# abb128/april-asr

Hardware: AMD Instinct MI355X
Metric: audio_seconds_per_second (concurrent 16 kHz sessions x 1/RTF), aprilv0_en-us-sized streaming RNN-T (higher is better)
Workload: dtype f32

## Files before the change

### april_asr_amd/_ffi.py

```python
import ctypes as C
import os

_HERE = os.path.dirname(os.path.abspath(__file__))
LIB_PATH = os.environ.get("APRIL_ASR_LIB") or os.path.join(_HERE, "libaprilasr.so")


class AprilSpeakerID(C.Structure):
    _fields_ = [("data", C.c_uint8 * 16)]


class AprilToken(C.Structure):
    _fields_ = [("token", C.c_char_p), ("logprob", C.c_float), ("flags", C.c_int),
                ("time_ms", C.c_size_t), ("reserved", C.c_void_p)]


HANDLER = C.CFUNCTYPE(None, C.c_void_p, C.c_int, C.c_size_t, C.POINTER(AprilToken))


class AprilConfig(C.Structure):
    _fields_ = [("speaker", AprilSpeakerID), ("handler", HANDLER), ("userdata", C.c_void_p), ("flags", C.c_int)]


class AprilxDims(C.Structure):
    _fields_ = [(n, C.c_int32) for n in ("n_layers", "d_model", "hidden", "ffn", "joiner", "vocab", "mel", "seg",
                                         "seg_step", "context", "fft_size", "frame_shift", "sample_rate", "blank_id",
                                         "n_devices", "precision", "d_model_file")] + [("param_count", C.c_int64)]


class AprilxStats(C.Structure):
    _fields_ = [(n, C.c_uint64) for n in ("ticks", "steps", "chunks", "rounds", "frames", "max_batch_seen")] + \
               [("kernel_ms", C.c_double * 6), ("kernel_launches", C.c_uint64 * 6), ("host_ms", C.c_double * 8),
                ("flights", C.c_uint64), ("replay_mismatch", C.c_uint64), ("kernels_per_step", C.c_uint64),
                ("lm_steps", C.c_uint64), ("lm_chunks", C.c_uint64),
                ("wave_steps", C.c_uint64), ("wave_chunks", C.c_uint64),
                ("gates_clock_ms", C.c_double), ("gates_clock_launches", C.c_uint64), ("gates_clock_rows", C.c_uint64),
                ("gates_clock_ms_by_n", C.c_double * 4), ("gates_clock_launches_by_n", C.c_uint64 * 4),
                ("resample_ms", C.c_double), ("resample_launches", C.c_uint64), ("confidence_records", C.c_uint64)]


class AprilxTokenInfo(C.Structure):
    _fields_ = [("size", C.c_uint32), ("n_alt", C.c_uint32), ("eval_index", C.c_uint64), ("lse", C.c_float),
                ("token_logprob", C.c_float), ("blank_logprob", C.c_float), ("reserved0", C.c_float),
                ("alt_id", C.c_int32 * 8), ("alt_logit", C.c_float * 8)]


class AprilxSearchOptions(C.Structure):
    _fields_ = [("size", C.c_uint32), ("endpoint_silence_ms", C.c_uint32), ("max_utterance_ms", C.c_uint32), ("blank_penalty", C.c_float)]


class AprilxLoadInfo(C.Structure):
    _fields_ = [("broadcast_ms", C.c_double), ("comm_init_ms", C.c_double), ("broadcast_bytes", C.c_uint64),
                ("ranks", C.c_int32), ("used_rccl", C.c_int32)]


class AprilxInputFormat(C.Structure):
    _fields_ = [("size", C.c_uint32), ("encoding", C.c_uint32), ("channels", C.c_uint32), ("channel", C.c_int32)]


EXPORTED_REFERENCE_SYMBOLS = [
    "aam_api_init", "aam_create_model", "aam_get_name", "aam_get_description", "aam_get_language",
    "aam_get_sample_rate", "aam_free", "aas_create_session", "aas_feed_pcm16", "aas_flush",
    "aas_realtime_get_speedup", "aas_free",
]
EXPORTED_ENGINE_SYMBOLS = [
    "aprilx_model_dims", "aprilx_model_token", "aprilx_model_blob_size", "aprilx_model_export_blob",
    "aprilx_model_from_blob", "aprilx_model_save_blob", "aprilx_model_save_blob_f16", "aprilx_model_load_blob",
    "aprilx_broadcast_get_id", "aprilx_model_broadcast", "aprilx_model_load_info", "aprilx_feed_many", "aprilx_flush_many", "aprilx_session_drain", "aprilx_feed_many_pipelined", "aprilx_drain_many",
    "aprilx_run_encoder", "aprilx_run_decoder", "aprilx_run_joiner", "aprilx_run_fbank", "aprilx_run_decide", "aprilx_plan_gemm", "aprilx_stream_form",
    "aprilx_session_trace_logits", "aprilx_session_chunks", "aprilx_session_read_frames", "aprilx_session_context", "aprilx_model_stats", "aprilx_model_profile", "aprilx_model_feed_latency",
    "aprilx_greedy_create", "aprilx_greedy_step", "aprilx_greedy_finish", "aprilx_greedy_free", "aprilx_probe_file", "aprilx_model_load_host", "aprilx_model_fbank_tables", "aprilx_counting_handler",
    "aprilx_session_set_input_rate", "aprilx_session_input_rate", "aprilx_resampler_taps", "aprilx_resample",
    "aprilx_session_set_confidence", "aprilx_session_confidence", "aprilx_run_confidence",
    "aprilx_bias_create", "aprilx_bias_free", "aprilx_bias_info", "aprilx_bias_edges", "aprilx_session_set_bias", "aprilx_session_bias_state",
    "aprilx_run_decide_biased", "aprilx_greedy_set_bias", "aprilx_greedy_bias_state",
    "aprilx_bias_create_ex", "aprilx_bias_flags", "aprilx_run_confidence_biased",
    "aprilx_session_set_search_options", "aprilx_session_search_options", "aprilx_run_decide_opts", "aprilx_greedy_set_search_options",
    "aprilx_ramp_window", "aprilx_model_ramp_stats",
    "aprilx_session_set_input_format", "aprilx_session_input_format", "aprilx_session_feed_bytes", "aprilx_feed_many_bytes",
    "aprilx_decode_host", "aprilx_decode", "aprilx_model_decode_stats",
]

_lib = None
_inited = False


def lib():
    global _lib
    if _lib is not None:
        return _lib
    if not os.path.exists(LIB_PATH):
        raise ImportError("libaprilasr.so is not built: run `python -c 'import __graft_entry__ as g; g.build()'` "
                          "or `make -C april_asr_amd/csrc` (hipcc, gfx950). There is no CPU fallback.")
    L = C.CDLL(LIB_PATH)
    vp, sz = C.c_void_p, C.c_size_t
    L.aam_api_init.argtypes = [C.c_int]; L.aam_api_init.restype = None
    L.aam_create_model.argtypes = [C.c_char_p]; L.aam_create_model.restype = vp
    for f in ("aam_get_name", "aam_get_description", "aam_get_language"):
        getattr(L, f).argtypes = [vp]; getattr(L, f).restype = C.c_char_p
    L.aam_get_sample_rate.argtypes = [vp]; L.aam_get_sample_rate.restype = sz
    L.aam_free.argtypes = [vp]; L.aam_free.restype = None
    L.aas_create_session.argtypes = [vp, AprilConfig]; L.aas_create_session.restype = vp
    L.aas_feed_pcm16.argtypes = [vp, vp, sz]; L.aas_feed_pcm16.restype = None
    L.aas_flush.argtypes = [vp]; L.aas_flush.restype = None
    L.aas_realtime_get_speedup.argtypes = [vp]; L.aas_realtime_get_speedup.restype = C.c_float
    L.aas_free.argtypes = [vp]; L.aas_free.restype = None
    L.aprilx_model_dims.argtypes = [vp, C.POINTER(AprilxDims)]; L.aprilx_model_dims.restype = C.c_int
    L.aprilx_model_token.argtypes = [vp, C.c_int32]; L.aprilx_model_token.restype = C.c_char_p
    L.aprilx_model_blob_size.argtypes = [vp]; L.aprilx_model_blob_size.restype = sz
    L.aprilx_model_export_blob.argtypes = [vp, vp, sz]; L.aprilx_model_export_blob.restype = C.c_int
    L.aprilx_model_from_blob.argtypes = [vp, sz, C.c_int]; L.aprilx_model_from_blob.restype = vp
    L.aprilx_model_save_blob.argtypes = [vp, C.c_char_p]; L.aprilx_model_save_blob.restype = C.c_int
    L.aprilx_model_save_blob_f16.argtypes = [vp, C.c_char_p]; L.aprilx_model_save_blob_f16.restype = C.c_int
    L.aprilx_model_load_blob.argtypes = [C.c_char_p]; L.aprilx_model_load_blob.restype = vp
    L.aprilx_broadcast_get_id.argtypes = [vp, sz]; L.aprilx_broadcast_get_id.restype = C.c_int
    L.aprilx_model_broadcast.argtypes = [vp, C.c_int, C.c_int, vp]; L.aprilx_model_broadcast.restype = vp
    L.aprilx_model_load_info.argtypes = [vp, C.POINTER(AprilxLoadInfo)]; L.aprilx_model_load_info.restype = C.c_int
    L.aprilx_feed_many.argtypes = [sz, C.POINTER(vp), C.POINTER(vp), C.POINTER(sz)]; L.aprilx_feed_many.restype = None
    L.aprilx_flush_many.argtypes = [sz, C.POINTER(vp)]; L.aprilx_flush_many.restype = None
    L.aprilx_session_drain.argtypes = [vp]; L.aprilx_session_drain.restype = None
    L.aprilx_feed_many_pipelined.argtypes = [sz, C.POINTER(vp), C.POINTER(vp), C.POINTER(sz), C.c_int]; L.aprilx_feed_many_pipelined.restype = None
    L.aprilx_drain_many.argtypes = [sz, C.POINTER(vp)]; L.aprilx_drain_many.restype = None
    L.aprilx_run_encoder.argtypes = [vp, C.c_int] + [vp] * 6; L.aprilx_run_encoder.restype = C.c_int
    L.aprilx_run_decoder.argtypes = [vp, C.c_int, vp, vp]; L.aprilx_run_decoder.restype = C.c_int
    L.aprilx_run_joiner.argtypes = [vp, C.c_int, vp, vp, vp]; L.aprilx_run_joiner.restype = C.c_int
    L.aprilx_run_fbank.argtypes = [vp, C.c_int, vp, vp]; L.aprilx_run_fbank.restype = C.c_int
    L.aprilx_plan_gemm.argtypes = [C.c_int] * 6 + [vp]; L.aprilx_plan_gemm.restype = C.c_int
    L.aprilx_ramp_window.argtypes = [C.c_int] * 3 + [vp, C.c_int]; L.aprilx_ramp_window.restype = C.c_int
    L.aprilx_model_ramp_stats.argtypes = [vp, C.c_int, C.POINTER(C.c_uint64), C.POINTER(C.c_uint64)]; L.aprilx_model_ramp_stats.restype = C.c_int
    L.aprilx_stream_form.argtypes = [C.c_int] * 6; L.aprilx_stream_form.restype = C.c_int
    L.aprilx_run_decide.argtypes = [vp, C.c_int, C.c_int, vp, C.c_float, vp, C.c_int, vp, vp]; L.aprilx_run_decide.restype = C.c_int
    L.aprilx_session_trace_logits.argtypes = [vp, vp, sz, C.POINTER(sz)]; L.aprilx_session_trace_logits.restype = None
    L.aprilx_session_chunks.argtypes = [vp]; L.aprilx_session_chunks.restype = C.c_uint64
    L.aprilx_session_read_frames.argtypes = [vp, C.c_uint64, C.c_int, C.c_void_p]; L.aprilx_session_read_frames.restype = C.c_uint64
    L.aprilx_session_context.argtypes = [vp, vp, vp]; L.aprilx_session_context.restype = None
    L.aprilx_model_stats.argtypes = [vp, C.c_int, C.POINTER(AprilxStats)]; L.aprilx_model_stats.restype = None
    L.aprilx_model_feed_latency.argtypes = [vp, C.c_int, vp, C.c_int, C.c_int]; L.aprilx_model_feed_latency.restype = C.c_int
    L.aprilx_model_profile.argtypes = [vp, C.c_int]; L.aprilx_model_profile.restype = None
    L.aprilx_greedy_create.argtypes = [vp, HANDLER, vp]; L.aprilx_greedy_create.restype = vp
    L.aprilx_greedy_step.argtypes = [vp, C.c_int32, C.c_float, C.c_float, C.c_float, sz, C.POINTER(C.c_int32)]
    L.aprilx_greedy_step.restype = C.c_int
    L.aprilx_greedy_finish.argtypes = [vp]; L.aprilx_greedy_finish.restype = None
    L.aprilx_greedy_free.argtypes = [vp]; L.aprilx_greedy_free.restype = None
    L.aprilx_model_load_host.argtypes = [C.c_char_p]; L.aprilx_model_load_host.restype = vp
    L.aprilx_model_fbank_tables.argtypes = [vp, vp, vp]; L.aprilx_model_fbank_tables.restype = C.c_int
    L.aprilx_probe_file.argtypes = [C.c_char_p, C.c_char_p, sz]; L.aprilx_probe_file.restype = C.c_int
    L.aprilx_session_set_input_rate.argtypes = [vp, C.c_uint32]; L.aprilx_session_set_input_rate.restype = C.c_int
    L.aprilx_session_input_rate.argtypes = [vp]; L.aprilx_session_input_rate.restype = C.c_uint32
    L.aprilx_resampler_taps.argtypes = [C.c_uint32, C.c_uint32, vp, vp, sz]; L.aprilx_resampler_taps.restype = C.c_int
    L.aprilx_resample.argtypes = [vp, C.c_uint32, vp, sz, vp, sz]; L.aprilx_resample.restype = C.c_int64
    L.aprilx_session_set_confidence.argtypes = [vp, C.c_int]; L.aprilx_session_set_confidence.restype = C.c_int
    L.aprilx_session_confidence.argtypes = [vp]; L.aprilx_session_confidence.restype = C.c_int
    L.aprilx_run_confidence.argtypes = [vp, C.c_int, vp, C.c_int, vp]; L.aprilx_run_confidence.restype = C.c_int
    L.aprilx_bias_create.argtypes = [vp, sz, C.POINTER(C.c_char_p), C.POINTER(C.c_float), C.c_char_p, sz]; L.aprilx_bias_create.restype = vp
    L.aprilx_bias_create_ex.argtypes = [vp, sz, C.POINTER(C.c_char_p), C.POINTER(C.c_float), C.c_uint32, C.c_char_p, sz]; L.aprilx_bias_create_ex.restype = vp
    L.aprilx_bias_flags.argtypes = [vp]; L.aprilx_bias_flags.restype = C.c_int
    L.aprilx_run_confidence_biased.argtypes = [vp, C.c_int, vp, C.c_int, vp, vp, vp]; L.aprilx_run_confidence_biased.restype = C.c_int
    L.aprilx_bias_free.argtypes = [vp]; L.aprilx_bias_free.restype = None
    L.aprilx_bias_info.argtypes = [vp, C.POINTER(C.c_int32), C.POINTER(C.c_int64)]; L.aprilx_bias_info.restype = C.c_int
    L.aprilx_bias_edges.argtypes = [vp, C.c_int32, vp, vp, vp, sz]; L.aprilx_bias_edges.restype = C.c_int
    L.aprilx_session_set_bias.argtypes = [vp, vp]; L.aprilx_session_set_bias.restype = C.c_int
    L.aprilx_session_bias_state.argtypes = [vp, C.POINTER(C.c_int32), C.POINTER(C.c_int32)]; L.aprilx_session_bias_state.restype = C.c_int
    L.aprilx_run_decide_biased.argtypes = [vp, C.c_int, C.c_int, vp, C.c_float, vp, C.c_int, vp, vp, vp, vp]; L.aprilx_run_decide_biased.restype = C.c_int
    L.aprilx_greedy_set_bias.argtypes = [vp, vp]; L.aprilx_greedy_set_bias.restype = C.c_int
    L.aprilx_greedy_bias_state.argtypes = [vp]; L.aprilx_greedy_bias_state.restype = C.c_int
    L.aprilx_session_set_search_options.argtypes = [vp, C.POINTER(AprilxSearchOptions)]; L.aprilx_session_set_search_options.restype = C.c_int
    L.aprilx_session_search_options.argtypes = [vp, C.POINTER(AprilxSearchOptions)]; L.aprilx_session_search_options.restype = C.c_int
    L.aprilx_run_decide_opts.argtypes = [vp, C.c_int, C.c_int, vp, C.c_float, vp, C.c_int, vp, vp, vp, vp, vp]; L.aprilx_run_decide_opts.restype = C.c_int
    L.aprilx_greedy_set_search_options.argtypes = [vp, C.POINTER(AprilxSearchOptions)]; L.aprilx_greedy_set_search_options.restype = C.c_int
    L.aprilx_session_set_input_format.argtypes = [vp, C.POINTER(AprilxInputFormat)]; L.aprilx_session_set_input_format.restype = C.c_int
    L.aprilx_session_input_format.argtypes = [vp, C.POINTER(AprilxInputFormat)]; L.aprilx_session_input_format.restype = C.c_int
    L.aprilx_session_feed_bytes.argtypes = [vp, vp, sz]; L.aprilx_session_feed_bytes.restype = C.c_int
    L.aprilx_feed_many_bytes.argtypes = [sz, C.POINTER(vp), C.POINTER(vp), C.POINTER(sz), C.c_int]; L.aprilx_feed_many_bytes.restype = C.c_int
    L.aprilx_decode_host.argtypes = [C.POINTER(AprilxInputFormat), vp, sz, vp, sz]; L.aprilx_decode_host.restype = C.c_int64
    L.aprilx_decode.argtypes = [vp, C.POINTER(AprilxInputFormat), vp, sz, vp, sz]; L.aprilx_decode.restype = C.c_int64
    L.aprilx_model_decode_stats.argtypes = [vp, C.c_int, C.POINTER(C.c_uint64), C.POINTER(C.c_uint64), C.POINTER(C.c_double)]; L.aprilx_model_decode_stats.restype = C.c_int
    _lib = L
    return L


def init():
    global _inited
    L = lib()
    if not _inited:
        L.aam_api_init(1)
        _inited = True
    return L
```

### april_asr_amd/csrc/engine.cc

```cpp
#include "engine.h"
#include <array>
#include <algorithm>
#include <cmath>
#include <chrono>
#include <cstdlib>
#include <cstring>
#include "common.h"
#include "env.h"

namespace aprilx {

static size_t align64(size_t x) { return (x + 63) & ~(size_t)63; }

void plan_layout(const NetDims &d, bool has_dec_conv_b, PackedLayout &L)
{
    L.dims = d;
    L.has_dec_conv_b = has_dec_conv_b;
    L.vocab_pad = (d.vocab + 31) & ~31;
    size_t off = 0;
    auto take = [&](size_t n) { size_t o = off; off = align64(off + n); return o; };
    L.k3 = (d.conv_ch[1] * 9 + 63) & ~63;
    L.conv_w[0] = take((size_t)d.conv_ch[0] * 9); L.conv_b[0] = take((size_t)d.conv_ch[0]);
    L.conv_w[1] = take((size_t)d.conv_ch[1] * d.conv_ch[0] * 9); L.conv_b[1] = take((size_t)d.conv_ch[1]);
    L.conv_w[2] = take((size_t)L.k3 * d.conv_ch[2]); L.conv_b[2] = take((size_t)d.conv_ch[2]);
// ... 49 lines not shown
    const NetDims &d = L.dims;
    blob.assign(L.total, 0.0f);
    float *B = blob.data();
    for (int i = 0; i < 3; ++i) {
        if (i < 2) memcpy(B + L.conv_w[i], m.conv_w[i].data(), m.conv_w[i].size() * 4);
        memcpy(B + L.conv_b[i], m.conv_b[i].data(), m.conv_b[i].size() * 4);
    }
    {
        const int kreal = d.conv_ch[1] * 9, c2 = d.conv_ch[2];
        std::vector<float> w3((size_t)L.k3 * c2, 0.0f);
        for (int o = 0; o < c2; ++o) for (int k = 0; k < kreal; ++k) w3[(size_t)k * c2 + o] = m.conv_w[2][(size_t)o * kreal + k];
        pack_mfma(w3.data(), L.k3, c2, c2, nullptr, B + L.conv_w[2]);
    }
    {
        const int c2 = d.conv_ch[2], F = d.f_out;
        std::vector<float> we((size_t)d.embed_in * d.d_model);
        for (int c = 0; c < c2; ++c) for (int f = 0; f < F; ++f)
            memcpy(&we[((size_t)f * c2 + c) * d.d_model], &m.w_embed[((size_t)c * F + f) * d.d_model], (size_t)d.d_model * 4);
        pack_mfma(we.data(), d.embed_in, d.d_model, d.d_model, nullptr, B + L.w_embed);
    }
    memcpy(B + L.b_embed, m.b_embed.data(), (size_t)d.d_model * 4);
    L.embed_eps = m.embed_norm_eps;
    L.norm_eps.resize((size_t)d.n_layers);
    std::vector<int> gmap((size_t)4 * d.hidden);
    for (int u = 0; u < d.hidden; ++u) for (int g = 0; g < 4; ++g) gmap[(size_t)u * 4 + g] = g * d.hidden + u;
    for (int l = 0; l < d.n_layers; ++l) {
        const LayerWeights &lw = m.layers[(size_t)l];
        const PackedLayout::Layer &o = L.layers[(size_t)l];
        pack_mfma(lw.w_gates.data(), 2 * d.d_model, 4 * d.hidden, 4 * d.hidden, &gmap, B + o.wg);
        for (int n = 0; n < 4 * d.hidden; ++n) B[o.bg + n] = lw.b_gates[(size_t)gmap[(size_t)n]];
        pack_mfma(lw.w_hr.data(), d.hidden, d.d_model, d.d_model, nullptr, B + o.whr);
        pack_mfma(lw.w_ff1.data(), d.d_model, d.ffn, d.ffn, nullptr, B + o.wff1);
        memcpy(B + o.bff1, lw.b_ff1.data(), (size_t)d.ffn * 4);
        pack_mfma(lw.w_ff2.data(), d.ffn, d.d_model, d.d_model, nullptr, B + o.wff2);
        memcpy(B + o.bff2, lw.b_ff2.data(), (size_t)d.d_model * 4);
        L.norm_eps[(size_t)l] = lw.norm_eps;
    }
    pack_mfma(m.w_encproj.data(), d.d_model, d.joiner, d.joiner, nullptr, B + L.w_encproj);
    memcpy(B + L.b_encproj, m.b_encproj.data(), (size_t)d.joiner * 4);
    memcpy(B + L.emb, m.emb.data(), m.emb.size() * 4);
    memcpy(B + L.dec_conv, m.dec_conv.data(), m.dec_conv.size() * 4);
    if (!m.dec_conv_b.empty()) memcpy(B + L.dec_conv_b, m.dec_conv_b.data(), m.dec_conv_b.size() * 4);
    pack_mfma(m.w_decproj.data(), d.d_model, d.joiner, d.joiner, nullptr, B + L.w_decproj);
    memcpy(B + L.b_decproj, m.b_decproj.data(), (size_t)d.joiner * 4);
    pack_mfma(m.w_out.data(), d.joiner, d.vocab, L.vocab_pad, nullptr, B + L.w_out);
    memcpy(B + L.b_out, m.b_out.data(), (size_t)d.vocab * 4);
}

template <typename T> static T *dmalloc(size_t n) { HipLegacyLock legacy; T *p = nullptr; HIP_CHECK(hipMalloc((void **)&p, std::max<size_t>(n, 1) * sizeof(T))); return p; }
template <typename T> static T *hmalloc(size_t n) { HipLegacyLock legacy; T *p = nullptr; HIP_CHECK(hipHostMalloc((void **)&p, std::max<size_t>(n, 1) * sizeof(T), hipHostMallocDefault)); return p; }

std::recursive_mutex &hip_legacy_mutex() { static std::recursive_mutex m; return m; }

static int pick_kz(int K, int N, int kblk = 16)
{
    int kz = 256 / std::max(1, N / 16);
    kz = std::max(1, std::min(kz, 8));
    while (kz > 1 && ((K / kblk) / kz < 4 || (K / kblk) % (4 * kz) != 0)) kz >>= 1;
    return kz;
}

Engine::Engine(const EngineConfig &cfg, const PackedLayout &layout, const float *blob_host, const float *blob_device,
               const ModelParams &params, const FbankHostTables &ft, const std::vector<uint8_t> &tok_class)
    : cfg_(cfg), L_(layout), P_(params)
{
    HipLegacyLock legacy;
    HIP_CHECK(hipSetDevice(cfg_.device));
    HIP_CHECK(hipStreamCreateWithFlags(&stream_, hipStreamNonBlocking));
    HIP_CHECK(hipStreamCreateWithFlags(&f_stream_, hipStreamNonBlocking));
    HIP_CHECK(hipStreamCreateWithFlags(&s_stream_, hipStreamNonBlocking));
    search_stream_ = stream_;
    for (int i = 0; i < 32; ++i) { hipEvent_t e; HIP_CHECK(hipEventCreateWithFlags(&e, hipEventDisableTiming)); join_ev_.push_back(e); }
    split_streams_ = std::max(0, std::min(2, env_int("APRIL_SPLIT_STREAMS", 2)));
    const NetDims &d = L_.dims;
    w_ = dmalloc<float>(L_.total);
    if (blob_device) HIP_CHECK(hipMemcpy(w_, blob_device, L_.total * 4, hipMemcpyDeviceToDevice));
    else if (blob_host) HIP_CHECK(hipMemcpy(w_, blob_host, L_.total * 4, hipMemcpyHostToDevice));

    const size_t S = (size_t)cfg_.max_slots, MB = (size_t)cfg_.max_batch;
    ring_frames_ = std::max(P_.segment_size * 32, env_int("APRIL_RING_FRAMES", 8192));
    h_ = dmalloc<float>((size_t)d.n_layers * S * d.d_model);
    c_ = dmalloc<float>((size_t)d.n_layers * S * d.hidden);
    if (!env_str("APRIL_RING_FRAMES")) {
        size_t free_b = 0, total_b = 0;
        if (hipMemGetInfo(&free_b, &total_b) == hipSuccess && free_b > 0) {
            const size_t per_frame = S * (size_t)d.mel * sizeof(float);
            const size_t fit = (free_b / 4) / per_frame;
            if (fit < (size_t)ring_frames_) {
                const int shrunk = std::max(P_.segment_size * 32, (int)std::min<size_t>(fit, 8192) / 64 * 64);
                LOGW("engine: %zu MB of feature rings (%d frames x %zu slots) exceed a quarter of the %zu MB free on device %d: %d frames per session",
                     per_frame * (size_t)ring_frames_ >> 20, ring_frames_, S, free_b >> 20, cfg_.device, shrunk);
                ring_frames_ = shrunk;
            }
        } else (void)hipGetLastError();
        float *p = nullptr;
        if (hipMalloc((void **)&p, S * ring_frames_ * d.mel * sizeof(float)) == hipSuccess) ring_ = p;
        else {
            (void)hipGetLastError();
            const size_t asked = S * (size_t)ring_frames_ * d.mel * sizeof(float);
            ring_frames_ = std::max(P_.segment_size * 32, 2048);
            LOGW("engine: no room for %zu MB of feature rings, falling back to %d frames per session", asked >> 20, ring_frames_);
        }
    }
    if (!ring_) ring_ = dmalloc<float>(S * ring_frames_ * d.mel);
    eout_ = dmalloc<float>(S * d.joiner);
    dout_ = dmalloc<float>(S * d.joiner);
    gstate_ = dmalloc<GreedyState>(S);
    HIP_CHECK(hipMemset(h_, 0, (size_t)d.n_layers * S * d.d_model * 4));
    HIP_CHECK(hipMemset(c_, 0, (size_t)d.n_layers * S * d.hidden * 4));
    HIP_CHECK(hipMemset(ring_, 0, S * ring_frames_ * d.mel * 4));
    HIP_CHECK(hipMemset(eout_, 0, S * d.joiner * 4));
    HIP_CHECK(hipMemset(dout_, 0, S * d.joiner * 4));
    {
        std::vector<GreedyState> init(S);
        for (auto &g : init) { g.ctx0 = P_.blank_id; g.ctx1 = P_.blank_id; g.last_tok = -1; g.last_emit_ms = 0; }
        HIP_CHECK(hipMemcpy(gstate_, init.data(), S * sizeof(GreedyState), hipMemcpyHostToDevice));
    }
    cls_ = dmalloc<uint8_t>((size_t)d.vocab);
    HIP_CHECK(hipMemcpy(cls_, tok_class.data(), (size_t)d.vocab, hipMemcpyHostToDevice));

    kz_embed_ = pick_kz(d.embed_in, d.d_model);
    kz_hr_ = pick_kz(d.hidden, d.d_model);
    kz_ff2_ = pick_kz(d.ffn, d.d_model);
    kz_proj_ = pick_kz(d.d_model, d.joiner);
    kz_out_ = pick_kz(d.joiner, L_.vocab_pad);
    {
        const bool want = cfg_.precision == 1 && env_int("APRIL_F16_TILE", 1) != 0;
        f16_tile_ = want && d.d_model % 128 == 0 && d.hidden % 128 == 0 && d.ffn % 128 == 0 && d.hidden % 16 == 0;
        if (f16_tile_) {
            kzx_hr_ = pick_kz(d.hidden, d.d_model, 32); kzx_ff2_ = pick_kz(d.ffn, d.d_model, 32);
            for (int p = 0; p < 2; ++p) y16_buf_[p] = dmalloc<uint16_t>(MB * d.d_model);
            y16_ = y16_buf_[0];
            for (int p = 0; p < 2; ++p) { xb16_buf_[p] = dmalloc<uint16_t>(MB * d.d_model); u16_buf_[p] = dmalloc<uint16_t>(MB * d.hidden); ff16_buf_[p] = dmalloc<uint16_t>(MB * d.ffn); }
            xb16_ = xb16_buf_[0]; u16_ = u16_buf_[0]; ff16_ = ff16_buf_[0];
            h16_ = dmalloc<uint16_t>((size_t)d.n_layers * S * d.d_model);
            HIP_CHECK(hipMemset(h16_, 0, (size_t)d.n_layers * S * d.d_model * 2));
        }
    }
    ws_mstride_ = cfg_.max_batch;
    const size_t ws_n = (size_t)std::max({kz_embed_ * d.d_model, kz_hr_ * d.d_model, kz_ff2_ * d.d_model, kz_proj_ * d.joiner, kz_out_ * L_.vocab_pad});
    ws_ = dmalloc<float>(ws_n * MB);
    ws_g_ = dmalloc<float>((size_t)std::max(kz_proj_ * d.joiner, kz_out_ * L_.vocab_pad) * MB);
    xin_ = dmalloc<float>(MB * d.embed_in);
    a3_ = dmalloc<float>(MB * d.f_out * L_.k3);
    HIP_CHECK(hipMemset(a3_, 0, MB * d.f_out * L_.k3 * 4));
    for (int p = 0; p < 2; ++p) { y_buf_[p] = dmalloc<float>(MB * d.d_model); ssq_buf_[p] = dmalloc<float>(MB * (d.d_model / SSQ_COLS)); }
    y_ = y_buf_[0]; ssq_ = ssq_buf_[0];
    ws_fe_ = dmalloc<float>((size_t)kz_embed_ * d.d_model * MB);
    ws_sr_ = dmalloc<float>((size_t)std::max(kz_proj_ * d.joiner, d.d_model) * MB);
    for (int p = 0; p < 2; ++p) { xb_buf_[p] = dmalloc<float>(MB * d.d_model); u_buf_[p] = dmalloc<float>(MB * d.hidden); ff_buf_[p] = dmalloc<float>(MB * d.ffn); }
    xb_ = xb_buf_[0]; u_ = u_buf_[0]; ff_ = ff_buf_[0];
    ramp_mode_ = env_int("APRIL_RAMP_MERGE", 1);
    if (ramp_mode_ < 0 || ramp_mode_ > 2) ramp_mode_ = 1;
    ramp_d_ = dmalloc<RampState>(1); HIP_CHECK(hipMemset(ramp_d_, 0, sizeof(RampState)));
    de_ = dmalloc<float>(MB * d.d_model);
    HIP_CHECK(hipMemset(de_, 0, MB * d.d_model * 4));
    logits_ = dmalloc<float>(3 * MB * d.vocab);
    logits_h_ = hmalloc<float>(3 * MB * d.vocab);
    ring_cap_ = std::max<size_t>((size_t)1 << 20, 3 * MB * 8 + 2 * S); ring_h_ = hmalloc<int>(2 * ring_cap_);
    step_cap_ = 1 << 14; step_off_h_ = hmalloc<int>((size_t)2 * step_cap_); rec_off_h_ = hmalloc<int>((size_t)2 * step_cap_);
    rec_cap_ = std::max<size_t>((size_t)1 << 20, 3 * MB * 8); rec_d_ = dmalloc<StepRecord>(2 * rec_cap_); rec_h_ = hmalloc<StepRecord>(2 * rec_cap_);
    for (int i = 0; i < 2; ++i) HIP_CHECK(hipEventCreateWithFlags(&flight_done_[i], hipEventDisableTiming));
    counter_d_ = dmalloc<int>(1);
    for (int p = 0; p < 2; ++p) {
        rec_off_buf_[p] = dmalloc<int>(1); flags_buf_[p] = dmalloc<int>(8); step_buf_[p] = dmalloc<int>(4 * MB);
        HIP_CHECK(hipMemset(rec_off_buf_[p], 0, 4)); HIP_CHECK(hipMemset(flags_buf_[p], 0, 32));
    }
    rec_off_d_ = rec_off_buf_[0]; flags_d_ = flags_buf_[0]; step_d_ = step_buf_[0];
    active_d_ = dmalloc<int>(MB); dirty_d_ = dmalloc<int>(MB);
    dec_slots_d_ = dmalloc<int>(std::max(S, MB));
    HIP_CHECK(hipMemset(counter_d_, 0, 4));

    upload_tables(ft);
    use_graphs_ = env_int("APRIL_NO_GRAPHS", 0) == 0;
    if (const int n = env_int("APRIL_GRAPH_CACHE_CAP", 0))
        step_graphs_.cap = lm_graphs_.cap = lm_search_graphs_.cap = sw_plan_cap_ = (size_t)std::max(n, 2), sw_graphs_.cap = 4 * sw_plan_cap_;
    free_.reserve(S);
    for (int i = cfg_.max_slots - 1; i >= 0; --i) free_.push_back(i);
    LOGI("engine: device %d, %d slots, max batch %d, weights %.1f MB, kz(embed,hr,ff2,proj,out)=%d,%d,%d,%d,%d",
         cfg_.device, cfg_.max_slots, cfg_.max_batch, L_.total * 4.0 / 1e6, kz_embed_, kz_hr_, kz_ff2_, kz_proj_, kz_out_);
}

void Engine::finish_weights()
{
    HipLegacyLock legacy;
    HIP_CHECK(hipSetDevice(cfg_.device));
    if (cfg_.precision == 1 && !wh_) {
        wh_ = dmalloc<uint16_t>(L_.total);
        for (const auto &sec : gemm_sections(L_)) launch_cvt_f16(w_ + sec.first, wh_ + sec.first, sec.second, nullptr);
        if (f16_tile_) {
            const NetDims &d = L_.dims;
            wx_ = dmalloc<uint16_t>(L_.total);
            for (const PackedLayout::Layer &o : L_.layers) {
                launch_repack_x32(w_ + o.wg, wx_ + o.wg, 2 * d.d_model, 4 * d.hidden, nullptr);
                launch_repack_x32(w_ + o.whr, wx_ + o.whr, d.hidden, d.d_model, nullptr);
                launch_repack_x32(w_ + o.wff1, wx_ + o.wff1, d.d_model, d.ffn, nullptr);
                launch_repack_x32(w_ + o.wff2, wx_ + o.wff2, d.ffn, d.d_model, nullptr);
            }
        }
        HIP_CHECK(hipDeviceSynchronize());
    }
    if (!conv_wt_) {
        const NetDims &d = L_.dims;
        conv_wt_ = dmalloc<float>((size_t)9 * d.conv_ch[0] + (size_t)9 * d.conv_ch[0] * d.conv_ch[1]);
        launch_conv_weight_transpose(w_ + L_.conv_w[0], w_ + L_.conv_w[1], d.conv_ch[0], d.conv_ch[1], conv_wt_, conv_wt_ + (size_t)9 * d.conv_ch[0], nullptr);
        HIP_CHECK(hipDeviceSynchronize());
    }
    build_dec_table();
}

void Engine::build_dec_table()
{
    if (dec_table_) return;
    const NetDims &d = L_.dims;
    const size_t limit_mb = (size_t)std::max(0, env_int("APRIL_DEC_TABLE_MB", 2048));
    const size_t rows = (size_t)d.vocab * (size_t)d.vocab;
    if (d.context != 2 || rows * (size_t)d.joiner * 4 > limit_mb * 1024 * 1024 || rows * (size_t)d.joiner * 4 >= ((size_t)1 << 32)) return;
    const int MB = cfg_.max_batch;
    float *table = dmalloc<float>(rows * (size_t)d.joiner);
    std::vector<int> iota((size_t)MB), ctx((size_t)MB * 2);
    for (int i = 0; i < MB; ++i) iota[(size_t)i] = i;
    int *ctx_d = dmalloc<int>((size_t)MB * 2);
    HIP_CHECK(hipMemcpy(dec_slots_d_, iota.data(), (size_t)MB * 4, hipMemcpyHostToDevice));
    for (size_t base = 0; base < rows; base += (size_t)MB) {
        const int n = (int)std::min<size_t>((size_t)MB, rows - base);
        for (int i = 0; i < n; ++i) { const size_t r = base + (size_t)i; ctx[(size_t)2 * i] = (int)(r / (size_t)d.vocab); ctx[(size_t)2 * i + 1] = (int)(r % (size_t)d.vocab); }
        HIP_CHECK(hipMemcpy(ctx_d, ctx.data(), (size_t)n * 8, hipMemcpyHostToDevice));
        DecEmbedArgs a; a.dec = dec_params(); a.ctx = ctx_d; a.M = n; a.out = de_; a.ldo = d.d_model;
        launch_dec_embed(a, stream_);
        run_decproj(n, dec_slots_d_, nullptr, nullptr, 1, table + base * (size_t)d.joiner);
        HIP_CHECK(hipStreamSynchronize(stream_));
    }
    (void)hipFree(ctx_d);
    dec_table_ = table;
    LOGI("engine: decoder table %zu rows x %d (%.0f MB)", rows, d.joiner, rows * (double)d.joiner * 4 / 1e6);
}

Engine::~Engine()
{
    HipLegacyLock legacy;
    (void)hipSetDevice(cfg_.device);
    (void)hipStreamSynchronize(f_stream_); (void)hipStreamSynchronize(stream_); (void)hipStreamSynchronize(s_stream_);
    dump_stream_trace();
    if (ramp_d_ && ramp_eligible_.load() > 0) {
        unsigned h = 0;
        if (hipMemcpy(&h, &ramp_d_->hosted, sizeof h, hipMemcpyDeviceToHost) == hipSuccess) LOGI("engine: ramp merge: %u of %llu hostable split feeds were hosted by their predecessor", h, (unsigned long long)ramp_eligible_.load());
    }
    for (StreamTrace &t : trace_) for (hipEvent_t e : t.ev) if (e) (void)hipEventDestroy(e);
    if (trace_base_) (void)hipEventDestroy(trace_base_);
    for (hipEvent_t e : join_ev_) (void)hipEventDestroy(e);
    for (auto &e : ev_pool_) { (void)hipEventDestroy(e.a); (void)hipEventDestroy(e.b); }
    drop_graphs(); free_sw_plans(); if (gclk_slots_) (void)hipFree(gclk_slots_);
    if (lm_stream_) { (void)hipStreamSynchronize(lm_stream_); (void)hipStreamDestroy(lm_stream_); }
    for (hipEvent_t e : lm_events_) (void)hipEventDestroy(e);
    if (zargs_h_) { (void)hipHostFree(zargs_h_); (void)hipFree(zargs_d_); }
    for (int i = 0; i < 3; ++i) if (zargs_done_[i]) (void)hipEventDestroy(zargs_done_[i]);
    for (void *p : {(void *)lm_now_d_, (void *)lm_rows_d_, (void *)lm_rec_off_d_}) if (p) (void)hipFree(p);
    if (conf_k_d_) (void)hipFree(conf_k_d_);
    if (conf_d_) (void)hipFree(conf_d_);
    if (conf_k_h_) (void)hipHostFree(conf_k_h_);
    if (conf_h_) (void)hipHostFree(conf_h_);
    for (auto &b : bias_sets_) if (b.dev) (void)hipFree(b.dev);
    for (void *p : {(void *)bias_set_d_, (void *)bias_state_d_, (void *)bias_desc_d_}) if (p) (void)hipFree(p);
    for (void *p : {(void *)bias_set_h_, (void *)bias_desc_h_}) if (p) (void)hipHostFree(p);
    if (opt_d_) (void)hipFree(opt_d_);
    if (opt_h_) (void)hipHostFree(opt_h_);
    if (ws_g_) (void)hipFree(ws_g_);
    if (conv_wt_) (void)hipFree(conv_wt_);
    if (dec_table_) (void)hipFree(dec_table_);
    if (p_lm_) (void)hipFree(p_lm_);
    for (int p = 0; p < 2; ++p)
        for (void *q : {(void *)eout_lm_buf_[p], (void *)y16_buf_[p], (void *)y_buf_[p], (void *)ssq_buf_[p], (void *)xb_buf_[p], (void *)u_buf_[p], (void *)ff_buf_[p],
                        (void *)xb16_buf_[p], (void *)u16_buf_[p], (void *)ff16_buf_[p], (void *)rec_off_buf_[p], (void *)flags_buf_[p], (void *)step_buf_[p]}) if (q) (void)hipFree(q);
    if (ws_fe_) (void)hipFree(ws_fe_);
    if (ws_sr_) (void)hipFree(ws_sr_);
    for (void *p : {(void *)wx_, (void *)h16_, (void *)ramp_d_}) if (p) (void)hipFree(p);
    for (void *p : {(void *)w_, (void *)wh_, (void *)h_, (void *)c_, (void *)ring_, (void *)eout_, (void *)dout_, (void *)gstate_, (void *)cls_, (void *)ws_, (void *)xin_,
                    (void *)a3_, (void *)de_, (void *)logits_, (void *)rec_d_, (void *)counter_d_,
                    (void *)active_d_, (void *)dirty_d_, (void *)dec_slots_d_,
                    (void *)ds_desc_[0], (void *)ds_desc_[1], (void *)ds_pcm_[0], (void *)ds_pcm_[1]})
        if (p) (void)hipFree(p);
    for (void *p : {(void *)ring_h_, (void *)step_off_h_, (void *)rec_off_h_, (void *)rec_h_, (void *)logits_h_, (void *)hs_desc_[0], (void *)hs_desc_[1], (void *)hs_pcm_[0], (void *)hs_pcm_[1]})
        if (p) (void)hipHostFree(p);
    for (int b = 0; b < 2; ++b) if (fb_done_[b]) (void)hipEventDestroy(fb_done_[b]);
    for (int b = 0; b < 2; ++b) if (flight_done_[b]) (void)hipEventDestroy(flight_done_[b]);
    for (void *p : table_allocs_) (void)hipFree(p);
    (void)hipStreamDestroy(stream_); (void)hipStreamDestroy(f_stream_); (void)hipStreamDestroy(s_stream_);
}

void Engine::upload_tables(const FbankHostTables &ft)
{
    auto up = [&](const void *src, size_t bytes) {
        void *p = nullptr;
        HIP_CHECK(hipMalloc(&p, std::max<size_t>(bytes, 16)));
        if (bytes) HIP_CHECK(hipMemcpy(p, src, bytes, hipMemcpyHostToDevice));
        table_allocs_.push_back(p);
        return p;
    };
    ft_.window = (const float *)up(ft.window.data(), ft.window.size() * 4);
    ft_.mel = (const float *)up(ft.mel.data(), ft.mel.size() * 4);
    ft_.mel_lo = (const int *)up(ft.mel_lo.data(), ft.mel_lo.size() * 4);
    ft_.mel_hi = (const int *)up(ft.mel_hi.data(), ft.mel_hi.size() * 4);
    ft_.nfct = (int)ft.factors.size();
    for (int k = 0; k < ft_.nfct; ++k) {
        ft_.fct[k] = ft.factors[(size_t)k];
        ft_.tw[k] = (const double *)up(ft.tw[(size_t)k].data(), ft.tw[(size_t)k].size() * 8);
        ft_.tws[k] = ft.tws[(size_t)k].empty() ? nullptr : (const double *)up(ft.tws[(size_t)k].data(), ft.tws[(size_t)k].size() * 8);
    }
    ft_.padded = ft.padded; ft_.nbins = ft.nbins;
    pad_value_ = ft.pad_value;
}

int Engine::alloc_slot()
{
    std::lock_guard<std::mutex> g(slot_mu_);
    if (free_.empty() && !zero_pending_.empty()) zero_pending_slots();
    if (free_.empty()) return -1;
    const int s = free_.back();
    free_.pop_back();
    ++live_;
    return s;
}

void Engine::zero_pending_slots()
{
    if (zero_pending_.empty()) return;
    if (hipSetDevice(cfg_.device) == hipSuccess) {
        std::lock_guard<std::mutex> cg(capture_mu_);
        m_touched();
        const NetDims &d = L_.dims;
        for (size_t o = 0; o < zero_pending_.size(); o += 64) {
            ZeroSlotArgs z;
            z.h = h_; z.c = c_; z.n_layers = d.n_layers; z.slots = (size_t)cfg_.max_slots; z.d_model = d.d_model; z.hidden = d.hidden;
            z.eout = eout_; z.dout = dout_; z.joiner = d.joiner; z.state = gstate_; z.blank = P_.blank_id; z.h16 = h16_;
            z.n_list = (int)std::min<size_t>(64, zero_pending_.size() - o);
            for (int i = 0; i < z.n_list; ++i) z.list[i] = zero_pending_[o + (size_t)i];
            launch_zero_slot(z, stream_);
        }
    }
    for (int s : zero_pending_) free_.push_back(s);
    zero_pending_.clear();
}

void Engine::free_slot(int slot)
{
    if (conf_ever_.load(std::memory_order_relaxed)) set_slot_confidence(slot, 0);
    if (bias_ever_.load(std::memory_order_relaxed)) set_slot_bias(slot, nullptr);
    if (opt_ever_.load(std::memory_order_relaxed)) set_slot_search_options(slot, SearchOpt{0u, 0.0f});
    std::lock_guard<std::mutex> g(slot_mu_);
    zero_pending_.push_back(slot);
    --live_;
    if (zero_pending_.size() >= 256) zero_pending_slots();
}

void Engine::sync_streams()
{
    HIP_CHECK(hipStreamSynchronize(f_stream_)); HIP_CHECK(hipStreamSynchronize(stream_)); HIP_CHECK(hipStreamSynchronize(s_stream_));
}

void Engine::sync()
{
    m_touched();
    sync_streams();
    f_unseen_by_m_ = s_unseen_by_m_ = m_unseen_by_f_ = m_unseen_by_s_ = false;
    if (profiling_) collect_timing();
}

template <typename Chain> static hipGraphExec_t capture_graph(hipStream_t st, Chain &&chain)
{
    hipGraph_t graph = nullptr;
    hipGraphExec_t exec = nullptr;
    HipLegacyLock capture_guard;
    HIP_CHECK(hipStreamBeginCapture(st, hipStreamCaptureModeRelaxed));
    chain();
    HIP_CHECK(hipStreamEndCapture(st, &graph));
    HIP_CHECK(hipGraphInstantiate(&exec, graph, nullptr, nullptr, 0));
    HIP_CHECK(hipGraphDestroy(graph));
    return exec;
}

void GraphCache::clear()
{
    if (!map_.empty()) LOGI("engine: %s graphs emptied (%zu entries)", name, map_.size());
    for (auto &g : map_) (void)hipGraphExecDestroy(g.second);
    map_.clear(); uses_.clear();
}

template <typename Chain> hipGraphExec_t Engine::cached_graph(GraphCache &cache, const GraphCache::Key &key, hipStream_t st, Chain &&chain)
{
    if (!cache.find(key)) cache.insert(key, capture_graph(st, chain));
    return cache.find(key);
}

template <typename Capture> void Engine::capture_both_parities(Capture &&capture)
{
    const int par = flight_parity_;
    m_touched();
    for (int q : {1 - par, par}) { select_parity(q); capture(); }
}

Engine::StreamTrace *Engine::trace_slot()
{
    static const char *path = env_str("APRIL_STREAM_TRACE");
    if (!path) return nullptr;
    if (!trace_base_) { HIP_CHECK(hipEventCreate(&trace_base_)); HIP_CHECK(hipEventRecord(trace_base_, stream_)); }
    if (trace_.size() >= 4096) return nullptr;
    trace_.emplace_back();
    StreamTrace &t = trace_.back();
    for (hipEvent_t &e : t.ev) HIP_CHECK(hipEventCreate(&e));
    return &t;
}

void Engine::dump_stream_trace()
{
    const char *path = env_str("APRIL_STREAM_TRACE");
    if (!path || trace_.empty()) return;
    FILE *f = fopen(path, "w");
    if (!f) return;
    fprintf(f, "# one line per split feed; times in us since the first split feed; FE = index fetch + conv + embed on stream F, LY = layer wavefront on M, SR = encoder_proj + search on S\n");
    fprintf(f, "# feed sessions chunks  FE_start FE_end  LY_start LY_end  SR_start SR_end   overlap: FE inside the previous feed's LY window? SR inside the next feed's LY window?\n");
    std::vector<std::array<float, 6>> ts;
    for (StreamTrace &t : trace_) {
        std::array<float, 6> a{};
        bool ok = t.used;
        for (int i = 0; i < 6 && ok; ++i) ok = hipEventElapsedTime(&a[(size_t)i], trace_base_, t.ev[i]) == hipSuccess;
        if (ok) ts.push_back(a); else (void)hipGetLastError();
    }
    for (size_t i = 0; i < ts.size(); ++i) {
        const auto &a = ts[i];
        const bool fe_in_prev = i > 0 && a[0] * 1e3f < ts[i - 1][3] * 1e3f && a[1] * 1e3f > ts[i - 1][2] * 1e3f;
        const bool sr_in_next = i + 1 < ts.size() && a[5] > ts[i + 1][2] && a[4] < ts[i + 1][3];
        fprintf(f, "%4zu %5d %2d  %10.1f %10.1f  %10.1f %10.1f  %10.1f %10.1f   %s %s\n", i, trace_[i].m, trace_[i].T, a[0] * 1e3, a[1] * 1e3, a[2] * 1e3, a[3] * 1e3, a[4] * 1e3, a[5] * 1e3,
                fe_in_prev ? "FE<prevLY" : "-", sr_in_next ? "SR<nextLY" : "-");
    }
    fclose(f);
}

void Engine::join(hipStream_t waiter, hipStream_t src)
{
    hipEvent_t e = join_ev_[join_pos_++ % join_ev_.size()];
    HIP_CHECK(hipEventRecord(e, src));
    HIP_CHECK(hipStreamWaitEvent(waiter, e, 0));
}

void Engine::general_prologue()
{
    m_touched();
    if (f_unseen_by_m_) { join(stream_, f_stream_); f_unseen_by_m_ = false; }
    if (s_unseen_by_m_) { join(stream_, s_stream_); s_unseen_by_m_ = false; }
    m_unseen_by_f_ = m_unseen_by_s_ = true;
    flight_tail_s_ = false;
}

void Engine::set_profiling(bool on) { std::lock_guard<std::mutex> cg(capture_mu_); sync(); profiling_ = on; }
void Engine::reset_timing() { for (auto &t : timing_) t = KernelTiming(); }
void Engine::set_gates_clock(bool on)
{
    std::lock_guard<std::mutex> cg(capture_mu_);
    HIP_CHECK(hipSetDevice(cfg_.device));
    sync();
    if (on) {
        if (!gclk_slots_) gclk_slots_ = dmalloc<unsigned long long>((size_t)GCLK_SLOTS * STAMP_WORDS);
        HIP_CHECK(hipMemsetAsync(gclk_slots_, 0, (size_t)GCLK_SLOTS * STAMP_WORDS * 8, stream_));
        HIP_CHECK(hipStreamSynchronize(stream_));
        gclk_ms_ = 0; gclk_launches_ = 0; gclk_rows_ = 0;
        for (int i = 0; i < 4; ++i) { gclk_ms_n_[i] = 0; gclk_launches_n_[i] = 0; }
        gclk_ = true;
        return;
    }
    collect_gates_clock(); gclk_ = false;
}
void Engine::collect_gates_clock()
{
    if (!gclk_ || !gclk_slots_) return;
    std::vector<unsigned long long> h((size_t)GCLK_SLOTS * STAMP_WORDS);
    HIP_CHECK(hipMemcpyAsync(h.data(), gclk_slots_, h.size() * 8, hipMemcpyDeviceToHost, stream_)); HIP_CHECK(hipStreamSynchronize(stream_));
    for (auto &kv : sw_plans_)
        for (size_t i = 0; i < kv.second.stamp_slots.size(); ++i) {
            const auto &sl = kv.second.stamp_slots[i];
            const unsigned long long ticks = h[(size_t)sl.first * STAMP_WORDS + 2], n = h[(size_t)sl.first * STAMP_WORDS + 3];
            gclk_ms_ += (double)ticks * 1e-5; gclk_launches_ += (long)n; gclk_rows_ += (long)n * sl.second;
            const int bn = std::min(std::max(kv.second.stamp_n[i], 1), 4) - 1;
            gclk_ms_n_[bn] += (double)ticks * 1e-5; gclk_launches_n_[bn] += (long)n;
        }
}
void Engine::timed_begin(int cls)
{
    ++launch_count_;
    if (!profiling_) return;
    if (ev_used_ == ev_pool_.size()) { Ev e; HIP_CHECK(hipEventCreate(&e.a)); HIP_CHECK(hipEventCreate(&e.b)); e.cls = cls; ev_pool_.push_back(e); }
    ev_pool_[ev_used_].cls = cls;
    if (cls == T_GATES) gemm_profile_next_launch(ev_pool_[ev_used_].a, ev_pool_[ev_used_].b);
    else HIP_CHECK(hipEventRecord(ev_pool_[ev_used_].a, stream_));
}
void Engine::timed_end(int cls)
{
    if (!profiling_) return;
    if (cls == T_GATES) {
        if (gemm_profile_pending()) { gemm_profile_next_launch(nullptr, nullptr); return; }
    } else HIP_CHECK(hipEventRecord(ev_pool_[ev_used_].b, stream_));
    ++ev_used_;
}
void Engine::collect_timing()
{
    for (size_t i = 0; i < ev_used_; ++i) {
        float ms = 0;
        if (hipEventElapsedTime(&ms, ev_pool_[i].a, ev_pool_[i].b) == hipSuccess) { timing_[ev_pool_[i].cls].ms += ms; timing_[ev_pool_[i].cls].launches++; }
    }
    ev_used_ = 0;
}

void Engine::fbank(int n_frames, const FbankFrameDesc *desc, const std::pair<const int16_t *, size_t> *parts, size_t n_parts, size_t n_pcm, HostPool *pool)
{
    const int n_rs = n_frames > 0 ? std::max(rs_n_, 0) : 0;
    ResampleDesc *rs = rs_desc_;
    const std::pair<const int16_t *, size_t> *in_parts = rs_in_parts_;
    const size_t n_in_parts = n_rs ? rs_n_in_parts_ : 0, n_in = n_rs ? rs_n_in_ : 0;
    rs_n_ = 0;
    const int n_dc = n_frames > 0 ? std::max(dc_n_, 0) : 0;
    const DecodeDesc *dc = dc_desc_;
    const std::pair<const uint8_t *, size_t> *raw_parts = dc_raw_parts_;
    const size_t n_raw_parts = n_dc ? dc_n_raw_parts_ : 0, n_raw = n_dc ? dc_n_raw_ : 0;
    const size_t raw_units = n_dc ? (n_raw + 1) / 2 + 8 : 0;
    dc_n_ = 0;
    if (n_frames <= 0) return;
    HIP_CHECK(hipSetDevice(cfg_.device));
    for (int i = 0; i < n_rs; ++i) rs[i].taps = resample_table(rs_specs_[i]);
    if (n_frames > desc_cap_ || n_pcm + n_in + raw_units > pcm_cap_ || (size_t)n_rs > rs_cap_ || (size_t)n_dc > dc_cap_) {
        sync();
        HipLegacyLock regrow_guard;
        for (int b = 0; b < 2; ++b) {
            if (hs_desc_[b]) { (void)hipHostFree(hs_desc_[b]); (void)hipFree(ds_desc_[b]); }
            if (hs_pcm_[b]) { (void)hipHostFree(hs_pcm_[b]); (void)hipFree(ds_pcm_[b]); }
        }
        desc_cap_ = std::max({n_frames * 2, desc_cap_, 1024});
        pcm_cap_ = std::max({(n_pcm + n_in + raw_units) * 2, pcm_cap_, (size_t)1 << 16});
        rs_cap_ = std::max({(size_t)n_rs * 2, rs_cap_, n_rs ? (size_t)256 : (size_t)0});
        dc_cap_ = std::max({(size_t)n_dc * 2, dc_cap_, n_dc ? (size_t)256 : (size_t)0});
        const size_t units = pcm_cap_ + 8 + ((size_t)desc_cap_ * sizeof(FbankFrameDesc) + 1) / 2 + 8 + rs_cap_ * sizeof(ResampleDesc) / 2
                             + 8 + dc_cap_ * sizeof(DecodeDesc) / 2;
        for (int b = 0; b < 2; ++b) {
            hs_pcm_[b] = hmalloc<int16_t>(units); ds_pcm_[b] = dmalloc<int16_t>(units);
            hs_desc_[b] = nullptr; ds_desc_[b] = nullptr;
            if (!fb_done_[b]) HIP_CHECK(hipEventCreateWithFlags(&fb_done_[b], hipEventDisableTiming));
        }
    }
    const int b = fb_flip_;
    fb_flip_ ^= 1;
    HIP_CHECK(hipEventSynchronize(fb_done_[b]));
    const size_t woff = ((n_pcm + n_in) * sizeof(int16_t) + 15) / 16 * 16;
    const size_t doff = (woff + n_raw + 15) / 16 * 16;
    const size_t roff = (doff + (size_t)n_frames * sizeof(FbankFrameDesc) + 15) / 16 * 16;
    const size_t coff = (roff + (size_t)n_rs * sizeof(ResampleDesc) + 15) / 16 * 16;
    const size_t bytes = n_dc ? coff + (size_t)n_dc * sizeof(DecodeDesc)
                              : (n_rs ? roff + (size_t)n_rs * sizeof(ResampleDesc) : doff + (size_t)n_frames * sizeof(FbankFrameDesc));
    char *hs = reinterpret_cast<char *>(hs_pcm_[b]);
    memcpy(hs + doff, desc, (size_t)n_frames * sizeof(FbankFrameDesc));
    ResampleArgs ra;
    if (n_rs) {
        ResampleDesc *hr = reinterpret_cast<ResampleDesc *>(hs + roff);
        int64_t blocks = 0, lds = 0;
        for (int i = 0; i < n_rs; ++i) {
            hr[i] = rs[i];
            hr[i].in_off += (int32_t)n_pcm;
            blocks = std::max<int64_t>(blocks, (rs[i].out_cnt + kResampleBlock - 1) / kResampleBlock);
            lds = std::max<int64_t>(lds, resample_lds_floats(rs[i].L, rs[i].M, rs[i].K));
        }
        ra.n_desc = n_rs; ra.max_blocks = (int)blocks; ra.lds_floats = (int)lds;
    }
    DecodeArgs da;
    if (n_dc) {
        DecodeDesc *hd = reinterpret_cast<DecodeDesc *>(hs + coff);
        int64_t blocks = 0; uint64_t frames = 0;
        for (int i = 0; i < n_dc; ++i) {
            hd[i] = dc[i];
            if (dc[i].dst_in) hd[i].dst += (int32_t)n_pcm;
            blocks = std::max<int64_t>(blocks, (dc[i].out_cnt + kDecodeBlock - 1) / kDecodeBlock);
            frames += (uint64_t)dc[i].n_src;
        }
        da.n_desc = n_dc; da.max_blocks = (int)blocks;
        dc_launches_.fetch_add(1, std::memory_order_relaxed); dc_frames_.fetch_add(frames, std::memory_order_relaxed);
    }
    auto stage = [&](const auto *pp, size_t np, size_t base) {
        const size_t el = sizeof(*pp[0].first);
        char *dst = hs;
        if (pool && np >= 256) {
            part_off_.resize(np);
            size_t off = base;
            for (size_t i = 0; i < np; ++i) { part_off_[i] = off; off += pp[i].second; }
            pool->run(np, 64, [&](size_t i) { if (pp[i].first) memcpy(dst + part_off_[i] * el, pp[i].first, pp[i].second * el); });
        } else {
            size_t off = base;
            for (size_t i = 0; i < np; ++i) { if (pp[i].first) memcpy(dst + off * el, pp[i].first, pp[i].second * el); off += pp[i].second; }
        }
    };
    stage(parts, n_parts, 0);
    if (n_in_parts) stage(in_parts, n_in_parts, n_pcm);
    if (n_raw_parts) stage(raw_parts, n_raw_parts, woff);
    std::lock_guard<std::mutex> cg(capture_mu_);
    if (m_unseen_by_f_) { join(f_stream_, stream_); m_unseen_by_f_ = false; }
    HIP_CHECK(hipMemcpyAsync(ds_pcm_[b], hs_pcm_[b], bytes, hipMemcpyHostToDevice, f_stream_));
    FbankArgs a;
    a.t = ft_; a.pcm = ds_pcm_[b]; a.desc = reinterpret_cast<const FbankFrameDesc *>(reinterpret_cast<const char *>(ds_pcm_[b]) + doff); a.n_frames = n_frames; a.ring = ring_; a.ring_frames = ring_frames_; a.pad_value = pad_value_;
    if (n_rs) { ra.in = ds_pcm_[b]; ra.out = ds_pcm_[b]; ra.desc = reinterpret_cast<const ResampleDesc *>(reinterpret_cast<const char *>(ds_pcm_[b]) + roff); }
    if (n_dc) {
        da.raw = reinterpret_cast<const uint8_t *>(ds_pcm_[b]) + woff; da.out = ds_pcm_[b];
        da.desc = reinterpret_cast<const DecodeDesc *>(reinterpret_cast<const char *>(ds_pcm_[b]) + coff);
    }
    if (profiling_) {
        m_touched();
        join(stream_, f_stream_);
        if (n_dc) { timed_begin(T_DECODE); launch_decode(da, stream_); timed_end(T_DECODE); }
        if (n_rs) { timed_begin(T_RESAMPLE); launch_resample(ra, stream_); timed_end(T_RESAMPLE); }
        timed_begin(T_FBANK); launch_fbank(a, stream_); timed_end(T_FBANK);
        join(f_stream_, stream_);
    } else {
        if (n_dc) launch_decode(da, f_stream_);
        if (n_rs) launch_resample(ra, f_stream_);
        launch_fbank(a, f_stream_);
    }
    HIP_CHECK(hipEventRecord(fb_done_[b], f_stream_));
    f_unseen_by_m_ = true;
}

const float *Engine::resample_table(const ResampleSpec *spec)
{
    std::lock_guard<std::mutex> g(rs_mu_);
    auto it = rs_tables_.find(spec);
    if (it != rs_tables_.end()) return it->second;
    HIP_CHECK(hipSetDevice(cfg_.device));
    float *d = dmalloc<float>(spec->taps.size());
    {
        HipLegacyLock legacy;
        if (!spec->taps.empty()) HIP_CHECK(hipMemcpy(d, spec->taps.data(), spec->taps.size() * sizeof(float), hipMemcpyHostToDevice));
        table_allocs_.push_back(d);
    }
    rs_tables_[spec] = d;
    return d;
}


RowScale Engine::in_scale(int l, size_t r0) const
{
    const NetDims &d = L_.dims;
    const int G = d.d_model / SSQ_COLS;
    RowScale r; r.ssq = ssq_ + r0 * G; r.groups = G; r.inv_n = 1.0f / (float)(d.d_norm ? d.d_norm : d.d_model); r.eps = l == 0 ? L_.embed_eps : L_.norm_eps[(size_t)l - 1];
    return r;
}

GemmArgs Engine::args_gates(int l, size_t r0, int rows, int waves) const
{
    const NetDims &d = L_.dims;
    const size_t S = (size_t)cfg_.max_slots;
    const PackedLayout::Layer &o = L_.layers[(size_t)l];
    GemmArgs g; g.a0 = y_ + r0 * d.d_model; g.lda0 = d.d_model; g.K0 = d.d_model; g.lda1 = d.d_model; g.K1 = d.d_model;
    lin(g, o.wg); g.M = rows; g.N = 4 * d.hidden; g.K = 2 * d.d_model; g.kz = 1; g.wave_mask = waves;
    if (f16_tile_) { g.a0 = reinterpret_cast<const float *>(y16_ + r0 * d.d_model); lin16(g, o.wg); }
    if (waves != GATES_H) g.x_scale = in_scale(l, r0);
    if (waves == GATES_X) {
        g.a1 = g.a0; g.epi = EPI_XPART; g.out = p_lm_ + r0 * 4 * d.hidden; g.ldo = 4 * d.hidden;
        return g;
    }
    g.a1 = h_ + (size_t)l * S * d.d_model; g.aidx1 = step_d_; g.epi = EPI_LSTM;
    g.out = u_ + r0 * d.hidden; g.ldo = d.hidden; g.bias = w_ + o.bg; g.c_state = c_ + (size_t)l * S * d.hidden; g.slot_idx = step_d_; g.hidden = d.hidden;
    if (waves == GATES_H) { g.p_add = p_lm_ + r0 * 4 * d.hidden; g.ldp = 4 * d.hidden; }
    else if (cfg_.precision == 0 && gates_tile_rows(rows)) g.tile_ok = 2;
    if (f16_tile_) {
        g.a1 = reinterpret_cast<const float *>(h16_ + (size_t)l * S * d.d_model); g.out = nullptr; g.out16 = u16_ + r0 * d.hidden;
    }
    return g;
}

constexpr long GATES_TILE_MIN_ROWS = 2048;
bool Engine::gates_tile_rows(long rows) const
{
    static const int mode = env_int("APRIL_GATES_TILE", 2);
    return mode == 1 || (mode == 2 && rows >= GATES_TILE_MIN_ROWS);
}

GemmArgs Engine::args_whr(int l, size_t r0, int rows) const
{
    const NetDims &d = L_.dims;
// ... 205 lines not shown

static int lm_block_steps(int T)
{
    const int b = (int)(0.75 * std::sqrt((double)std::max(1, T)) + 0.5);
    return std::max(6, std::min(32, b));
}
constexpr int LM_WAVEFRONT_MIN_CHUNKS = 10;

static bool lm_wavefront_on()
{
    static const bool on = env_int("APRIL_LM_WAVEFRONT", 1) != 0;
    return on;
}

void Engine::run_lm_chain(int m, int T, bool dump_logits)
{
    const NetDims &d = L_.dims;
    const int MB = cfg_.max_batch;
    const int L = d.n_layers;
    launch_advance(advance_args(m, T), stream_);
    encoder_front(0, m * T, step_d_ + 3 * MB, nullptr, stream_, ws_);
    for (int l = 0; l < L; ++l) lm_stage_layer(l, m, 0, T, stream_);
    lm_stage_proj(m, 0, T, stream_, ws_);
    for (int t = 0; t < T; ++t) run_greedy_rounds(m, dump_logits, t, eout_lm_ + (size_t)t * m * d.joiner);
}

void Engine::run_lm_wavefront(int m, int T, bool dump_logits)
{
    const NetDims &d = L_.dims;
    const int MB = cfg_.max_batch;
    const int L = d.n_layers;
    const int blk = lm_block_steps(T);
    const int NB = (T + blk - 1) / blk;
    launch_advance(advance_args(m, T), stream_);
    hipStream_t cs = lm_stream_;
    HIP_CHECK(hipEventRecord(lm_events_[0], stream_));
    HIP_CHECK(hipStreamWaitEvent(cs, lm_events_[0], 0));

    const size_t need = (size_t)(NB + L + 1) * (size_t)(2 * blk + 6) * (size_t)L;
    if (need > zargs_region_) {
        HIP_CHECK(hipStreamSynchronize(cs));
        HipLegacyLock regrow_guard;
        if (zargs_h_) { (void)hipHostFree(zargs_h_); (void)hipFree(zargs_d_); }
        zargs_region_ = need + need / 4;
        zargs_h_ = hmalloc<GemmArgs>(3 * zargs_region_); zargs_d_ = dmalloc<GemmArgs>(3 * zargs_region_);
        for (int i = 0; i < 3; ++i) zargs_busy_[i] = false;
    }
    const int zslot = zargs_next_;
    zargs_next_ = (zargs_next_ + 1) % 3;
    if (zargs_busy_[zslot]) HIP_CHECK(hipEventSynchronize(zargs_done_[zslot]));
    zargs_pos_ = (size_t)zslot * zargs_region_;

    static const bool timing = env_str("APRIL_LM_TIMING") != nullptr;
    double tacc[6] = {0, 0, 0, 0, 0, 0};
    auto now = [&]() { return timing ? std::chrono::duration<double, std::micro>(std::chrono::steady_clock::now().time_since_epoch()).count() : 0.0; };
    struct Batch { size_t off; int n; };
    std::vector<Batch> plan;
    std::vector<size_t> plan_end((size_t)(NB + L + 1), 0);
    std::vector<GemmArgs> items;
    struct Act { int l, t0, t1; };
    std::vector<Act> act;
    double tq = now();
    auto lap = [&](int i) { if (timing) { const double t = now(); tacc[i] += t - tq; tq = t; } };
    const size_t first = zargs_pos_;
    for (int W = 0; W <= NB + L; ++W) {
        act.clear();
        for (int l = 0; l < L; ++l) { const int b = W - 1 - l; if (b >= 0 && b < NB) act.push_back({l, b * blk, std::min(T, (b + 1) * blk)}); }
        auto flush = [&]() {
            if (items.empty()) return;
            stage_gemm_z(items.data(), (int)items.size(), zargs_h_ + zargs_pos_);
            plan.push_back({zargs_pos_, (int)items.size()});
            zargs_pos_ += items.size(); items.clear();
        };
        auto by_len = [&](auto make) {
            for (int pass = 0; pass < 2; ++pass) {
                for (const Act &x : act) if (((x.t1 - x.t0) == blk) == (pass == 0)) items.push_back(make(x));
                flush();
            }
        };
        by_len([&](const Act &x) { return args_gates(x.l, (size_t)x.t0 * m, (x.t1 - x.t0) * m, GATES_X); });
        for (int i = 0; i < blk; ++i) {
            for (const Act &x : act) if (x.t0 + i < x.t1) items.push_back(args_gates(x.l, (size_t)(x.t0 + i) * m, m, GATES_H));
            flush();
            for (const Act &x : act) if (x.t0 + i < x.t1) items.push_back(args_whr(x.l, (size_t)(x.t0 + i) * m, m));
            flush();
        }
        by_len([&](const Act &x) { return args_ff1(x.l, (size_t)x.t0 * m, (x.t1 - x.t0) * m); });
        by_len([&](const Act &x) { return args_ff2(x.l, (size_t)x.t0 * m, (x.t1 - x.t0) * m); });
        plan_end[(size_t)W] = plan.size();
    }
    lap(0);
    if (zargs_pos_ > first)
        HIP_CHECK(hipMemcpyAsync(zargs_d_ + first, zargs_h_ + first, (zargs_pos_ - first) * sizeof(GemmArgs), hipMemcpyHostToDevice, cs));
    lap(1);
    for (int W = 0; W <= NB + L; ++W) {
        if (W < NB) encoder_front((size_t)W * blk * m, (std::min(T, (W + 1) * blk) - W * blk) * m, step_d_ + 3 * MB, nullptr, cs, ws_);
        lap(2);
        for (size_t k = W ? plan_end[(size_t)W - 1] : 0; k < plan_end[(size_t)W]; ++k) launch_gemm_z(zargs_h_ + plan[k].off, plan[k].n, zargs_d_ + plan[k].off, cs);
        lap(3);
        const int bp = W - L - 1;
        if (bp >= 0) {
            const int t0 = bp * blk, t1 = std::min(T, t0 + blk), len = t1 - t0;
            lm_stage_proj(m, t0, t1, cs, ws_);
            hipEvent_t e = lm_events_[1 + (size_t)(bp % (int)(lm_events_.size() - 1))];
            HIP_CHECK(hipEventRecord(e, cs));
            HIP_CHECK(hipStreamWaitEvent(stream_, e, 0));
            BlockSetupArgs bs;
            bs.now_src = step_d_ + 2 * MB + (size_t)t0 * m; bs.now_dst = lm_now_d_; bs.rows_dst = lm_rows_d_; bs.row0 = t0 * m; bs.count = len * m;
            bs.rec_off_step = rec_off_d_; bs.rec_off_block = lm_rec_off_d_; bs.rec_add = t0 * 3 * m; bs.flags = flags_d_; bs.n_flags = 8;
            launch_block_setup(bs, stream_);
            lap(4);
            auto search = [&]() {
                for (int i = 0; i < len; ++i) {
                    GreedyIo io;
                    io.gen = i + 1; io.now = lm_now_d_ + (size_t)i * m; io.eout = eout_lm_; io.eout_rows = lm_rows_d_ + (size_t)i * m;
                    io.rec_off = lm_rec_off_d_; io.rec_slot0 = i * 3;
                    io.dump = dump_logits ? logits_ + (size_t)(t0 + i) * 3 * m * d.vocab : nullptr;
                    run_greedy_rounds(m, io);
                }
            };
            if (!use_graphs_ || dump_logits) { search(); continue; }
            const GraphCache::Key key = graph_key(m, len);
            if (!lm_search_graphs_.find(key) && lm_search_graphs_.full()) { HIP_CHECK(hipStreamSynchronize(stream_));  lm_search_graphs_.clear(); }
            HIP_CHECK(hipGraphLaunch(cached_graph(lm_search_graphs_, key, stream_, search), stream_));
            lap(5);
        }
    }
    HIP_CHECK(hipEventRecord(zargs_done_[zslot], cs));
    zargs_busy_[zslot] = true;
    if (timing) fprintf(stderr, "lm wavefront %d x %d: host us: args %.0f, arg copy %.0f, front end %.0f, layer launches %.0f, proj + events + setup %.0f, search graph %.0f\n",
                        m, T, tacc[0], tacc[1], tacc[2], tacc[3], tacc[4], tacc[5]);
}

static bool lm_gates_split_on()
{
    static const bool on = env_int("APRIL_GATES_SPLIT", 1) != 0;
    return on;
}

Engine::SwPlan &Engine::sw_plan(int m, int T)
{
    const GraphCache::Key key = sw_key(m, T);
    auto it = sw_plans_.find(key);
    if (it != sw_plans_.end()) return it->second;
    if (sw_plans_.size() >= sw_plan_cap_) {
        sync();
        HipLegacyLock evict_guard;
        collect_gates_clock(); free_sw_plans();
        if (gclk_slots_) { HIP_CHECK(hipMemsetAsync(gclk_slots_, 0, (size_t)GCLK_SLOTS * STAMP_WORDS * 8, stream_)); HIP_CHECK(hipStreamSynchronize(stream_)); }
        gclk_used_ = 0;
    }
    SwPlan &p = sw_plans_[key];
    build_sw_chain(p, p.one, m, T, false);
    if (ramp_mode_ != 0 && !gclk_) build_sw_chain(p, p.split, m, T, true);
    return p;
}

std::vector<RampStep> ramp_window(int L, int T, int R, int max_problems)
{
    std::vector<RampStep> w;
    if (L <= 2 * R || T < 1 || R < 1) return w;
    for (int j = 1; j <= R; ++j) {
        RampStep s; s.macro = L + T - 1 - R + j;
        for (int l = 0; l < L; ++l) { const int t = s.macro - 1 - l; if (t >= 0 && t < T) ++s.own; }
        for (int t = 0; t < j; ++t) s.guests.push_back(std::make_pair(j - 1 - t, t));
        if (s.own + (int)s.guests.size() > max_problems) return std::vector<RampStep>();
        w.push_back(s);
    }
    return w;
}

void Engine::ramp_counts(uint64_t *hosted, uint64_t *eligible)
{
    unsigned h = 0;
    {
        HipLegacyLock legacy;
        if (hipSetDevice(cfg_.device) == hipSuccess) HIP_CHECK(hipMemcpy(&h, &ramp_d_->hosted, sizeof h, hipMemcpyDeviceToHost));
    }
    *hosted = h; *eligible = ramp_eligible_.load(std::memory_order_relaxed);
}

void Engine::build_sw_chain(SwPlan &p, SwPlan::Chain &c, int m, int T, bool ramp)
{
    const NetDims &d = L_.dims;
    const int L = d.n_layers;
    const int par = flight_parity_;
    const int tk = f16_tile_ ? 2 : tile_ok();
    auto needs_rows = [&](int kind, int n) {
        const int kz = kind == 1 ? kz_hr() : kz_ff2();
        return (kind == 1 || kind == 3) && tk && (tk == 2 || gemm_tile_planned(m, d.d_model, kz, n)) && !gemm_fullk(m, d.d_model, kz, false, n, tk);
    };
    std::vector<RampStep> window;
    if (ramp && m <= RAMP_MAX_M && T <= RAMP_MAX_T) {
        window = ramp_window(L, T, RAMP_R);
        for (const RampStep &s : window) if (needs_rows(1, s.own + (int)s.guests.size()) || needs_rows(3, s.own + (int)s.guests.size())) { window.clear(); break; }
    }
    if (ramp) p.hosts = !window.empty();
    std::vector<GemmArgs> items;
    std::vector<RowArgs> rows;
    for (int W = 0; W <= T + L; ++W) {
        const RampStep *host = nullptr; int wj = 0;
        for (size_t j = 0; j < window.size(); ++j) if (window[j].macro == W) { host = &window[j]; wj = (int)j; }
        if (host && wj == 0) { SwPlan::Batch b; b.off = c.host.size(); b.n = 0; b.macro = W; b.kind = 4; b.roff = c.rhost.size(); b.rn = 0; c.batches.push_back(b); }
        for (int kind = 0; kind < 4; ++kind) {
            items.clear(); rows.clear();
            int n_act = 0;
            for (int l = 0; l < L; ++l) { const int t = W - 1 - l; if (t >= 0 && t < T) ++n_act; }
            if (n_act == 0) continue;
            if (host) n_act += (int)host->guests.size();
            const int kz = kind == 1 ? kz_hr() : kz_ff2();
            const bool split = needs_rows(kind, n_act);
            auto problem = [&](int l, int t, const int *run_flag) {
                const size_t r0 = (size_t)t * m;
                GemmArgs g = kind == 0 ? args_gates(l, r0, m, GATES_ALL) : kind == 1 ? args_whr(l, r0, m) : kind == 2 ? args_ff1(l, r0, m) : args_ff2(l, r0, m);
                if (kind == 0 && cfg_.precision == 0) g.tile_ok = gates_tile_rows((long)m * n_act) ? 2 : 0;
                if (run_flag) { g.run_flag = run_flag; g.run_gen = 1; }
                if (split) {
                    float *ws = ws_ + r0 * d.d_model;
                    rows.push_back(row_form(g, ws, ws_mstride_, gemm_partials(m, d.d_model, kz, n_act, tk)));
                    g = partial_form(g, ws, ws_mstride_);
                } else if (tk == 2) g.force_fullk = 0;
                items.push_back(g);
            };
            for (int l = 0; l < L; ++l) {
                const int t = W - 1 - l;
                if (t < 0 || t >= T) continue;
                problem(l, t, ramp && W <= RAMP_R ? &ramp_d_->head_live[par] : nullptr);
            }
            if (host) {
                select_parity(1 - par);
                for (const auto &lt : host->guests) problem(lt.first, lt.second, &ramp_d_->guest_live[par][wj][lt.second]);
                select_parity(par);
            }
            std::vector<int> groups;
            {
                int left = (int)items.size();
                const bool cut = kind == 0 && cfg_.precision == 0 && left >= 4 && !gates_tile_rows((long)m * n_act) && lm_gates_split_on();
                while (cut && left > 0) { const int take = (left == 4 || left == 2) ? 2 : (left >= 3 ? 3 : left); groups.push_back(take); left -= take; }
                if (groups.empty()) groups.push_back((int)items.size());
            }
            size_t first = 0;
            for (size_t gi = 0; gi < groups.size(); ++gi) {
                const int gn = groups[gi];
                if (kind == 0 && !ramp && gclk_ && gclk_slots_ && gclk_used_ < GCLK_SLOTS) {
                    p.stamp_slots.push_back(std::make_pair(gclk_used_, (long)m * gn)); p.stamp_n.push_back(gn);
                    for (int i = 0; i < gn; ++i) items[first + (size_t)i].stamp = gclk_slots_ + (size_t)gclk_used_ * STAMP_WORDS;
                    ++gclk_used_;
                } else if (kind == 0 && !ramp && gclk_ && gclk_slots_ && !gclk_warned_) {
                    gclk_warned_ = true; LOGW("engine: the gates clock is out of stamp slots (%d): the gates launches of further plans are not timed", GCLK_SLOTS);
                }
                SwPlan::Batch b; b.off = c.host.size(); b.n = gn; b.macro = W; b.kind = kind; b.roff = c.rhost.size(); b.rn = gi == 0 ? (int)rows.size() : 0;
                c.host.resize(c.host.size() + (size_t)gn);
                stage_gemm_z(items.data() + first, gn, c.host.data() + b.off);
                if (gi == 0) c.rhost.insert(c.rhost.end(), rows.begin(), rows.end());
                c.batches.push_back(b);
                first += (size_t)gn;
            }
        }
    }
    m_touched();
    c.dev = dmalloc<GemmArgs>(c.host.size());
    HIP_CHECK(hipMemcpyAsync(c.dev, c.host.data(), c.host.size() * sizeof(GemmArgs), hipMemcpyHostToDevice, stream_));
    if (!c.rhost.empty()) {
        c.rdev = dmalloc<RowArgs>(c.rhost.size());
        HIP_CHECK(hipMemcpyAsync(c.rdev, c.rhost.data(), c.rhost.size() * sizeof(RowArgs), hipMemcpyHostToDevice, stream_));
    }
}

void Engine::free_sw_plans()
{
    if (!sw_plans_.empty()) LOGI("engine: feed wavefront plans emptied (%zu plans)", sw_plans_.size());
    for (auto &p : sw_plans_) for (SwPlan::Chain *c : {&p.second.one, &p.second.split}) { if (c->dev) (void)hipFree(c->dev); if (c->rdev) (void)hipFree(c->rdev); }
    sw_graphs_.clear(); sw_plans_.clear();
}

void Engine::run_sw_chain(int m, int T, bool dump_logits, const SwPlan &p, int part, hipStream_t st)
{
    const NetDims &d = L_.dims;
    const int MB = cfg_.max_batch;
    if (part < 0 || part == 0) {
        launch_advance(advance_args(m, T), st);
        encoder_front(0, m * T, step_d_ + 3 * MB, nullptr, st, part == 0 ? ws_fe_ : ws_);
    }
    if (part < 0 || part == 1) {
        static const int cls_of[4] = {T_GATES, T_GEMM_OTHER, T_GEMM_OTHER, T_GEMM_OTHER};
        const SwPlan::Chain &c = p.layers(part == 1);
        for (size_t bi = 0; bi < c.batches.size(); ++bi) {
            const SwPlan::Batch &b = c.batches[bi];
            if (b.kind == 4) { launch_ramp_latch(ramp_d_, flight_parity_, m, st); continue; }
            timed_begin(cls_of[b.kind]); launch_gemm_z(c.host.data() + b.off, b.n, c.dev + b.off, st); timed_end(cls_of[b.kind]);
            if (b.rn > 0) { timed_begin(T_ROW); launch_row_z(c.rhost.data() + b.roff, b.rn, c.rdev + b.roff, st); timed_end(T_ROW); }
        }
        if (part < 0) lm_stage_proj(m, 0, T, st, ws_);
    }
    if (part < 0 || part == 2) {
        if (part == 2) lm_stage_proj(m, 0, T, st, ws_sr_);
        hipStream_t keep = search_stream_;
        search_stream_ = st;
        for (int t = 0; t < T; ++t) run_greedy_rounds(m, dump_logits, t, eout_lm_ + (size_t)t * m * d.joiner);
        search_stream_ = keep;
    }
}

int Engine::lm_step(int m, int T, const int *slots, const int *ring_tails, const int *now_ms, float *logits_out, int mode)
{
    const int rows = m * T;
    if (m <= 0 || T <= 0 || rows > cfg_.max_batch || !flight_has_room(rows + m, 1)) { LOGE("engine: layer-major step %d x %d does not fit (max batch %d)", m, T, cfg_.max_batch); abort(); }
    HIP_CHECK(hipSetDevice(cfg_.device));
    const NetDims &d = L_.dims;
    if (!p_lm_) {
        p_lm_ = dmalloc<float>((size_t)cfg_.max_batch * 4 * d.hidden);
        for (int p = 0; p < 2; ++p) eout_lm_buf_[p] = dmalloc<float>((size_t)cfg_.max_batch * d.joiner);
        eout_lm_ = eout_lm_buf_[flight_parity_];
    }
    if (!lm_stream_) {
        HIP_CHECK(hipStreamCreateWithFlags(&lm_stream_, hipStreamNonBlocking));
        for (int i = 0; i < 9; ++i) { hipEvent_t e; HIP_CHECK(hipEventCreateWithFlags(&e, hipEventDisableTiming)); lm_events_.push_back(e); }
        for (int i = 0; i < 3; ++i) HIP_CHECK(hipEventCreateWithFlags(&zargs_done_[i], hipEventDisableTiming));
        lm_now_d_ = dmalloc<int>((size_t)cfg_.max_batch); lm_rows_d_ = dmalloc<int>((size_t)cfg_.max_batch); lm_rec_off_d_ = dmalloc<int>(1);
    }
    const int k = stage_step(m, T, slots, ring_tails, now_ms);
    std::lock_guard<std::mutex> cg(capture_mu_);
    mode == 1 ? run_feed_wavefront(m, T, logits_out != nullptr) : run_layer_major(m, T, logits_out != nullptr);
    if (logits_out) read_back_logits(k, rows, logits_out);
    return k;
}

void Engine::run_feed_wavefront(int m, int T, bool dump_logits)
{
    sw_plan(m, T);
    const bool graphs = use_graphs_ && !profiling_ && !dump_logits && (sw_graphs_.find(sw_key(m, T)) || sw_graphs_.find(sw_key(m, T, 1)) || sw_graphs_.use(m, T) >= 2);
    const bool split = graphs && split_streams_ > 0 && overlap_hint_ && flight_steps_ == 1 && !gclk_;
    const hipStream_t on[3] = {split_streams_ >= 2 ? f_stream_ : stream_, stream_, s_stream_};
    if (graphs && !sw_graphs_.find(sw_key(m, T, split ? 1 : 0)))
        capture_both_parities([&]() {
            const SwPlan &pl = sw_plan(m, T);
            if (split) for (int part = 0; part < 3; ++part) cached_graph(sw_graphs_, sw_key(m, T, 1 + part), on[part], [&]() { run_sw_chain(m, T, false, pl, part, on[part]); });
            else cached_graph(sw_graphs_, sw_key(m, T), stream_, [&]() { run_sw_chain(m, T, false, pl, -1, stream_); });
        });
    if (split) { launch_split_feed(m, T, on[0]); return; }
    general_prologue();
    if (graphs) { HIP_CHECK(hipGraphLaunch(sw_graphs_.find(sw_key(m, T)), stream_)); return; }
    launch_count_ = 0; run_sw_chain(m, T, dump_logits, sw_plan(m, T), -1, stream_); kernels_per_step_ = (launch_count_ + 1 + T - 1) / T;
}

void Engine::launch_split_feed(int m, int T, hipStream_t fe)
{
    if (fe == f_stream_) {
        if (m_unseen_by_f_) { join(f_stream_, stream_); m_unseen_by_f_ = false; }
    } else if (f_unseen_by_m_) { join(stream_, f_stream_); f_unseen_by_m_ = false; }
    if (m_unseen_by_s_) { join(s_stream_, stream_); m_unseen_by_s_ = false; }
    StreamTrace *tr = trace_slot();
    auto part = [&](int i, hipStream_t st) {
        if (tr) HIP_CHECK(hipEventRecord(tr->ev[2 * i], st));
        HIP_CHECK(hipGraphLaunch(sw_graphs_.find(sw_key(m, T, 1 + i)), st));
        if (tr) HIP_CHECK(hipEventRecord(tr->ev[2 * i + 1], st));
    };
    part(0, fe);
    if (ramp_mode_ != 0) {
        const bool hostable = ramp_mode_ == 1 && fe == f_stream_ && m_quiet_.load(std::memory_order_acquire);
        if (hostable) ramp_eligible_.fetch_add(1, std::memory_order_relaxed);
        launch_ramp_ready(ramp_d_, flight_parity_, m, T, hostable ? 1 : 0, fe);
    }
    if (fe == f_stream_) { join(stream_, f_stream_); f_unseen_by_m_ = false; }
    part(1, stream_);
    if (ramp_mode_ != 0) m_quiet_.store(true, std::memory_order_release);
    join(s_stream_, stream_); part(2, s_stream_);
    if (tr) { tr->m = m; tr->T = T; tr->used = true; }
    s_unseen_by_m_ = true; flight_tail_s_ = true;
    if (fe != f_stream_) m_unseen_by_f_ = true;
}

void Engine::run_layer_major(int m, int T, bool dump_logits)
{
    general_prologue();
    const NetDims &d = L_.dims; const int tk = f16_tile_ ? 2 : tile_ok();
    const bool wavefront = lm_wavefront_on() && !profiling_ && T > LM_WAVEFRONT_MIN_CHUNKS &&
                           gemm_fullk(m, d.d_model, kz_hr(), true, 1, tk) && gemm_fullk(m, d.d_model, kz_ff2(), true, 1, tk);
    if (wavefront) { run_lm_wavefront(m, T, dump_logits); return; }
    if (!use_graphs_ || profiling_ || dump_logits) { launch_count_ = 0; run_lm_chain(m, T, dump_logits); kernels_per_step_ = launch_count_ + 1; return; }
    const GraphCache::Key key = graph_key(m, T);
    if (!lm_graphs_.find(key) && lm_graphs_.full()) { sync(); lm_graphs_.clear(); }
    HIP_CHECK(hipGraphLaunch(cached_graph(lm_graphs_, key, stream_, [&]() { run_lm_chain(m, T, false); }), stream_));
}

int Engine::stage_step(int m, int T, const int *slots, const int *ring_tails, const int *now_ms)
{
    const size_t rows = (size_t)m * (size_t)std::max(T, 1);
    const int k = next_step_index(); int *blk = ring_h_ + ring_pos_;
    memcpy(blk, slots, (size_t)m * 4); memcpy(blk + m, ring_tails, rows * 4); memcpy(blk + m + rows, now_ms, rows * 4);
    for (int t = 0; t < T; ++t) memcpy(blk + m + 2 * rows + (size_t)t * m, slots, (size_t)m * 4);
    step_off_h_[k] = (int)ring_pos_; rec_off_h_[k] = (int)rec_pos_;
    ring_pos_ += (size_t)m + (T ? 3 : 2) * rows; rec_pos_ += 3 * rows;
    if (conf_k_h_) note_conf_step(k, slots, m, 3 * rows);
    return k;
}

void Engine::read_back_logits(int k, int rows, float *out)
{
    const size_t n = (size_t)3 * rows * L_.dims.vocab;
    HIP_CHECK(hipMemcpyAsync(logits_h_, logits_, n * 4, hipMemcpyDeviceToHost, stream_));
    HIP_CHECK(hipMemcpyAsync(rec_h_ + rec_off_h_[k], rec_d_ + rec_off_h_[k], (size_t)3 * rows * sizeof(StepRecord), hipMemcpyDeviceToHost, stream_));
    sync();
    memcpy(out, logits_h_, n * 4);
}

void Engine::apply_confidence_pending()
{
    std::vector<std::pair<int, int>> todo;
    { std::lock_guard<std::mutex> g(conf_mu_); todo.swap(conf_pending_); conf_has_pending_.store(false, std::memory_order_release); }
    if (!conf_k_h_) {
        bool any = false;
        for (const auto &t : todo) any = any || t.second > 0;
        if (!any) return;
        std::lock_guard<std::mutex> cg(capture_mu_);
        HipLegacyLock legacy;
        sync();
        drop_graphs();
        const size_t S = (size_t)cfg_.max_slots;
        conf_k_d_ = dmalloc<uint8_t>(S); conf_k_h_ = hmalloc<uint8_t>(S);
        memset(conf_k_h_, 0, S);
        conf_d_ = dmalloc<ConfRecord>(2 * rec_cap_); conf_h_ = hmalloc<ConfRecord>(2 * rec_cap_);
        LOGI("engine: confidences on (side ring %.0f MB on the device and pinned)", 2.0 * rec_cap_ * sizeof(ConfRecord) / 1e6);
    }
    for (const auto &t : todo) if (t.first >= 0 && t.first < cfg_.max_slots) conf_k_h_[t.first] = (uint8_t)t.second;
    std::lock_guard<std::mutex> cg(capture_mu_);
    m_touched();
    HIP_CHECK(hipMemcpyAsync(conf_k_d_, conf_k_h_, (size_t)cfg_.max_slots, hipMemcpyHostToDevice, stream_));
}

void Engine::drop_graphs()
{
    for (GraphCache *c : {&step_graphs_, &lm_graphs_, &lm_search_graphs_, &sw_graphs_}) c->clear();
}

BiasDesc Engine::upload_bias(const BiasSet &set, void **dev, hipStream_t st)
{
    auto pad = [](size_t b) { return (b + 15) & ~(size_t)15; };
    const size_t ns = set.state_off.size() * 4, ne = std::max<size_t>(set.edge_tok.size(), 1) * 4;
    char *p = nullptr;
    HIP_CHECK(hipMalloc((void **)&p, pad(ns) + 3 * pad(ne)));
    BiasDesc d;
    d.state_off = (const int32_t *)p; d.edge_tok = (const int32_t *)(p + pad(ns)); d.edge_next = (const int32_t *)(p + pad(ns) + pad(ne));
    d.edge_bonus = (const float *)(p + pad(ns) + 2 * pad(ne)); d.n_states = set.states(); d.flags = (int32_t)set.flags;
    HIP_CHECK(hipMemcpyAsync((void *)d.state_off, set.state_off.data(), ns, hipMemcpyHostToDevice, st));
    if (!set.edge_tok.empty()) {
        const size_t b = set.edge_tok.size() * 4;
        HIP_CHECK(hipMemcpyAsync((void *)d.edge_tok, set.edge_tok.data(), b, hipMemcpyHostToDevice, st));
        HIP_CHECK(hipMemcpyAsync((void *)d.edge_next, set.edge_next.data(), b, hipMemcpyHostToDevice, st));
        HIP_CHECK(hipMemcpyAsync((void *)d.edge_bonus, set.edge_bonus.data(), b, hipMemcpyHostToDevice, st));
    }
    *dev = p;
    return d;
}

void Engine::apply_bias_pending()
{
    std::lock_guard<std::mutex> bg(bias_mu_);
    std::vector<std::pair<int, int>> todo;
    todo.swap(bias_pending_);
    bias_has_pending_.store(false, std::memory_order_release);
    std::lock_guard<std::mutex> cg(capture_mu_);
    m_touched();
    if (!bias_set_h_) {
        bool any = false;
        for (const auto &t : todo) any = any || t.second >= 0;
        if (!any) return;
        HipLegacyLock legacy;
        sync();
        drop_graphs();
        const size_t S = (size_t)cfg_.max_slots;
        bias_set_d_ = dmalloc<int32_t>(S); bias_set_h_ = hmalloc<int32_t>(S); bias_state_d_ = dmalloc<int32_t>(S);
        bias_desc_d_ = dmalloc<BiasDesc>(kBiasSets); bias_desc_h_ = hmalloc<BiasDesc>(kBiasSets);
        for (size_t i = 0; i < S; ++i) bias_set_h_[i] = -1;
        for (int i = 0; i < kBiasSets; ++i) bias_desc_h_[i] = BiasDesc();
        HIP_CHECK(hipMemsetAsync(bias_state_d_, 0, S * 4, stream_));
        LOGI("engine: phrase boosting on");
    }
    bool tables = false;
    for (int i = 0; i < kBiasSets; ++i) {
        BiasEntry &b = bias_sets_[(size_t)i];
        if (b.set && b.users > 0 && !b.dev) {
            HipLegacyLock legacy;
            bias_desc_h_[i] = upload_bias(*b.set, &b.dev, stream_);
            HIP_CHECK(hipStreamSynchronize(stream_));
            tables = true;
        } else if (b.set && b.users == 0) {
            if (b.dev) { HipLegacyLock legacy; sync_streams(); (void)hipFree(b.dev); b.dev = nullptr; }
            bias_desc_h_[i] = BiasDesc();
            b.set.reset();
            tables = true;
        }
    }
    for (const auto &t : todo) {
        bias_set_h_[t.first] = t.second;
        HIP_CHECK(hipMemsetAsync(bias_state_d_ + t.first, 0, 4, stream_));
    }
    if (tables) HIP_CHECK(hipMemcpyAsync(bias_desc_d_, bias_desc_h_, sizeof(BiasDesc) * kBiasSets, hipMemcpyHostToDevice, stream_));
    HIP_CHECK(hipMemcpyAsync(bias_set_d_, bias_set_h_, (size_t)cfg_.max_slots * 4, hipMemcpyHostToDevice, stream_));
}

void Engine::apply_search_options_pending()
{
    std::vector<std::pair<int, SearchOpt>> todo;
    { std::lock_guard<std::mutex> g(opt_mu_); todo.swap(opt_pending_); opt_has_pending_.store(false, std::memory_order_release); }
    if (!opt_h_) {
        bool any = false;
        for (const auto &t : todo) any = any || t.second.endpoint_ms != 0;
        if (!any) return;
        std::lock_guard<std::mutex> cg(capture_mu_);
        HipLegacyLock legacy;
        sync();
        drop_graphs();
        const size_t S = (size_t)cfg_.max_slots;
        opt_d_ = dmalloc<SearchOpt>(S); opt_h_ = hmalloc<SearchOpt>(S);
        memset(opt_h_, 0, S * sizeof(SearchOpt));
        LOGI("engine: search options on");
    }
    for (const auto &t : todo) if (t.first >= 0 && t.first < cfg_.max_slots) opt_h_[t.first] = t.second;
    std::lock_guard<std::mutex> cg(capture_mu_);
    m_touched();
    HIP_CHECK(hipMemcpyAsync(opt_d_, opt_h_, (size_t)cfg_.max_slots * sizeof(SearchOpt), hipMemcpyHostToDevice, stream_));
}

int Engine::read_bias_state(int slot)
{
    if (!bias_ever_.load(std::memory_order_relaxed)) return 0;
    std::lock_guard<std::mutex> bg(bias_mu_);
    for (const auto &t : bias_pending_) if (t.first == slot) return 0;
    HipLegacyLock legacy;
    HIP_CHECK(hipSetDevice(cfg_.device));
    sync_streams();
    int v = 0;
    if (bias_state_d_) HIP_CHECK(hipMemcpy(&v, bias_state_d_ + slot, 4, hipMemcpyDeviceToHost));
    return v;
}

void Engine::note_conf_step(int k, const int *slots, int m, size_t records)
{
    bool any = false;
    for (int i = 0; i < m && !any; ++i) any = conf_k_h_[slots[i]] != 0;
    if (!any) return;
    const size_t first = (size_t)rec_off_h_[k];
    if (!conf_spans_.empty() && conf_spans_.back().first + conf_spans_.back().second == first) conf_spans_.back().second += records;
    else conf_spans_.push_back(std::make_pair(first, records));
}

void Engine::select_parity(int p)
{
    flight_parity_ = p;
    xb_ = xb_buf_[p]; u_ = u_buf_[p]; ff_ = ff_buf_[p]; xb16_ = xb16_buf_[p]; u16_ = u16_buf_[p]; ff16_ = ff16_buf_[p];
    y_ = y_buf_[p]; ssq_ = ssq_buf_[p]; y16_ = y16_buf_[p]; step_d_ = step_buf_[p]; flags_d_ = flags_buf_[p]; rec_off_d_ = rec_off_buf_[p]; eout_lm_ = eout_lm_buf_[p];
}

void Engine::begin_flight()
{
    HIP_CHECK(hipSetDevice(cfg_.device));
    const int p = flight_parity_ = next_parity_; next_parity_ ^= 1;
    if (flight_open_[p]) { HIP_CHECK(hipEventSynchronize(flight_done_[p])); flight_open_[p] = false; }
    if (conf_has_pending_.load(std::memory_order_acquire)) apply_confidence_pending();
    if (bias_has_pending_.load(std::memory_order_acquire)) apply_bias_pending();
    if (opt_has_pending_.load(std::memory_order_acquire)) apply_search_options_pending();
    conf_spans_.clear();
    ring_base_ = (size_t)p * ring_cap_; rec_base_ = (size_t)p * rec_cap_;
    ring_pos_ = ring_base_; rec_pos_ = rec_base_; flight_steps_ = 0;
    select_parity(p);
    flight_tail_s_ = false;
    { std::lock_guard<std::mutex> g(slot_mu_); zero_pending_slots(); }
}

bool Engine::flight_has_room(int rows, int nsteps) const
{
    return flight_steps_ + nsteps <= step_cap_ && ring_pos_ + (size_t)3 * rows + (size_t)cfg_.max_slots <= ring_base_ + ring_cap_ && rec_pos_ + (size_t)3 * rows <= rec_base_ + rec_cap_;
}

int Engine::step(int m, const int *slots, const int *ring_tails, const int *now_ms, float *logits_out)
{
    if (m <= 0 || m > cfg_.max_batch || !flight_has_room(m, 1)) { LOGE("engine: step of %d rows does not fit (max batch %d)", m, cfg_.max_batch); abort(); }
    const int k = stage_step(m, 0, slots, ring_tails, now_ms);
    std::lock_guard<std::mutex> cg(capture_mu_);
    general_prologue();
    const GraphCache::Key key = graph_key(m);
    if (use_graphs_ && !profiling_ && !logits_out && (step_graphs_.find(key) || step_graphs_.use(m) >= 2)) {
        if (!step_graphs_.find(key)) {
            if (step_graphs_.full()) { sync(); step_graphs_.clear(); }
            capture_both_parities([&]() { cached_graph(step_graphs_, graph_key(m), stream_, [&]() { run_chain(m, false); }); });
        }
        HIP_CHECK(hipGraphLaunch(step_graphs_.find(key), stream_));
        return k;
    }
    launch_count_ = 0; run_chain(m, logits_out != nullptr); kernels_per_step_ = launch_count_ + 1;
    if (logits_out) read_back_logits(k, m, logits_out);
    return k;
}

void Engine::decode_rows(int n, const int *slots, int op)
{
    if (n <= 0) return;
    if (dec_table_ && op == 0) return;
    HIP_CHECK(hipSetDevice(cfg_.device));
    const NetDims &d = L_.dims;
    const int MB = cfg_.max_batch;
    std::lock_guard<std::mutex> cg(capture_mu_);
    general_prologue();
    for (int o = 0; o < n; o += MB) {
        const int m = std::min(MB, n - o);
        if (ring_pos_ + (size_t)m > ring_base_ + ring_cap_) { LOGE("engine: index ring exhausted"); abort(); }
        int *blk = ring_h_ + ring_pos_;
        memcpy(blk, slots + o, (size_t)m * 4);
        ring_pos_ += (size_t)m;
        HIP_CHECK(hipMemcpyAsync(dec_slots_d_, blk, (size_t)m * 4, hipMemcpyHostToDevice, stream_));
        DecRowsArgs a; a.slot_idx = dec_slots_d_; a.M = m; a.op = op; a.blank = P_.blank_id; a.state = gstate_; a.dec = dec_params(); a.de_out = dec_table_ ? nullptr : de_; a.ld_de = d.d_model;
        a.bias_state = bias_state_d_;
        timed_begin(T_DEC); launch_dec_rows(a, stream_); timed_end(T_DEC);
        if (!dec_table_) run_decproj(m, dec_slots_d_, nullptr, nullptr, 1);
    }
}

int Engine::close_flight()
{
    HIP_CHECK(hipSetDevice(cfg_.device));
    std::lock_guard<std::mutex> cg(capture_mu_);
    hipStream_t tail = s_stream_;
    if (!(flight_tail_s_ && s_unseen_by_m_)) {
        tail = stream_;
        if (f_unseen_by_m_) { join(stream_, f_stream_); f_unseen_by_m_ = false; }
        if (s_unseen_by_m_) { join(stream_, s_stream_); s_unseen_by_m_ = false; }
    }
    if (rec_pos_ > rec_base_) HIP_CHECK(hipMemcpyAsync(rec_h_ + rec_base_, rec_d_ + rec_base_, (rec_pos_ - rec_base_) * sizeof(StepRecord), hipMemcpyDeviceToHost, tail));
    for (const auto &sp : conf_spans_) {
        HIP_CHECK(hipMemcpyAsync(conf_h_ + sp.first, conf_d_ + sp.first, sp.second * sizeof(ConfRecord), hipMemcpyDeviceToHost, tail));
        conf_copied_.fetch_add(sp.second, std::memory_order_relaxed);
    }
    conf_spans_.clear();
    HIP_CHECK(hipEventRecord(flight_done_[flight_parity_], tail));
    flight_open_[flight_parity_] = true;
    return flight_parity_;
}

bool Engine::flight_done(int parity)
{
    const hipError_t e = hipEventQuery(flight_done_[parity]);
    if (e == hipSuccess) return true;
    if (e != hipErrorNotReady) HIP_CHECK(e);
    (void)hipGetLastError();
    return false;
}

void Engine::wait_flight(int parity)
{
    HIP_CHECK(hipSetDevice(cfg_.device));
    HIP_CHECK(hipEventSynchronize(flight_done_[parity]));
    if (profiling_) sync();
}

void Engine::end_flight() { wait_flight(close_flight()); }

void Engine::zero_slots(int n)
{
    const NetDims &d = L_.dims;
    for (int i = 0; i < n; ++i) {
        ZeroSlotArgs z;
        z.h = h_; z.c = c_; z.n_layers = d.n_layers; z.slots = (size_t)cfg_.max_slots; z.d_model = d.d_model; z.hidden = d.hidden;
        z.eout = eout_; z.dout = dout_; z.joiner = d.joiner; z.state = gstate_; z.blank = P_.blank_id; z.slot = i; z.h16 = h16_;
        launch_zero_slot(z, stream_);
    }
    HIP_CHECK(hipStreamSynchronize(stream_));
}

void Engine::debug_encoder(int n, const float *x, const float *h, const float *c, float *eout, float *h2, float *c2)
{
    std::lock_guard<std::mutex> cg(capture_mu_);
    HipLegacyLock legacy;
    HIP_CHECK(hipSetDevice(cfg_.device));
    const NetDims &d = L_.dims;
    const size_t S = (size_t)cfg_.max_slots;
    if (n > cfg_.max_batch || n > cfg_.max_slots) { LOGE("debug_encoder: n too large"); abort(); }
    std::vector<int> slots((size_t)n);
    for (int i = 0; i < n; ++i) slots[(size_t)i] = i;
    float *xd = dmalloc<float>((size_t)n * d.seg * d.mel);
    HIP_CHECK(hipMemcpy(xd, x, (size_t)n * d.seg * d.mel * 4, hipMemcpyHostToDevice));
    for (int i = 0; i < n; ++i)
        for (int l = 0; l < d.n_layers; ++l) {
            HIP_CHECK(hipMemcpy(h_ + ((size_t)l * S + i) * d.d_model, h + ((size_t)i * d.n_layers + l) * d.d_model, (size_t)d.d_model * 4, hipMemcpyHostToDevice));
            HIP_CHECK(hipMemcpy(c_ + ((size_t)l * S + i) * d.hidden, c + ((size_t)i * d.n_layers + l) * d.hidden, (size_t)d.hidden * 4, hipMemcpyHostToDevice));
        }
    HIP_CHECK(hipMemcpy(step_d_, slots.data(), (size_t)n * 4, hipMemcpyHostToDevice));
    if (f16_tile_)
        for (int l = 0; l < d.n_layers; ++l) launch_cvt_f16(h_ + (size_t)l * S * d.d_model, h16_ + (size_t)l * S * d.d_model, (size_t)n * d.d_model, stream_);
    run_encoder_rows(n, xd);
    sync();
    for (int i = 0; i < n; ++i) {
        HIP_CHECK(hipMemcpy(eout + (size_t)i * d.joiner, eout_ + (size_t)i * d.joiner, (size_t)d.joiner * 4, hipMemcpyDeviceToHost));
        for (int l = 0; l < d.n_layers; ++l) {
            HIP_CHECK(hipMemcpy(h2 + ((size_t)i * d.n_layers + l) * d.d_model, h_ + ((size_t)l * S + i) * d.d_model, (size_t)d.d_model * 4, hipMemcpyDeviceToHost));
            HIP_CHECK(hipMemcpy(c2 + ((size_t)i * d.n_layers + l) * d.hidden, c_ + ((size_t)l * S + i) * d.hidden, (size_t)d.hidden * 4, hipMemcpyDeviceToHost));
        }
    }
    (void)hipFree(xd);
    zero_slots(n);
}

void Engine::debug_decoder(int n, const int64_t *ctx, float *dout)
{
    std::lock_guard<std::mutex> cg(capture_mu_);
    HipLegacyLock legacy;
    HIP_CHECK(hipSetDevice(cfg_.device));
    const NetDims &d = L_.dims;
    if (n > cfg_.max_batch) { LOGE("debug_decoder: n too large"); abort(); }
    if (dec_table_) {
        bool in_range = true;
        for (int i = 0; i < n * 2; ++i) if (ctx[i] < 0 || ctx[i] >= d.vocab) in_range = false;
        if (in_range) {
            sync();
            for (int i = 0; i < n; ++i)
                HIP_CHECK(hipMemcpy(dout + (size_t)i * d.joiner, dec_table_ + ((size_t)ctx[2 * i] * d.vocab + (size_t)ctx[2 * i + 1]) * d.joiner, (size_t)d.joiner * 4, hipMemcpyDeviceToHost));
            return;
        }
    }
    std::vector<int> slots((size_t)n), c32((size_t)n * d.context);
    for (int i = 0; i < n; ++i) { slots[(size_t)i] = i; for (int t = 0; t < d.context; ++t) c32[(size_t)i * d.context + t] = (int)ctx[(size_t)i * d.context + t]; }
    int *ctx_d = dmalloc<int>(c32.size());
    HIP_CHECK(hipMemcpy(ctx_d, c32.data(), c32.size() * 4, hipMemcpyHostToDevice));
    HIP_CHECK(hipMemcpy(dec_slots_d_, slots.data(), (size_t)n * 4, hipMemcpyHostToDevice));
    DecEmbedArgs a; a.dec = dec_params(); a.ctx = ctx_d; a.M = n; a.out = de_; a.ldo = d.d_model;
    launch_dec_embed(a, stream_);
    run_decproj(n, dec_slots_d_, nullptr, nullptr, 1);
    sync();
    HIP_CHECK(hipMemcpy(dout, dout_, (size_t)n * d.joiner * 4, hipMemcpyDeviceToHost));
    (void)hipFree(ctx_d);
    zero_slots(n);
}

void Engine::debug_joiner(int n, const float *eout, const float *dout, float *logits)
{
    std::lock_guard<std::mutex> cg(capture_mu_);
    HipLegacyLock legacy;
    const NetDims &d = L_.dims;
    HIP_CHECK(hipSetDevice(cfg_.device));
    if (n > cfg_.max_batch) { LOGE("debug_joiner: n too large"); abort(); }
    HIP_CHECK(hipMemcpy(eout_, eout, (size_t)n * d.joiner * 4, hipMemcpyHostToDevice));
    HIP_CHECK(hipMemcpy(dout_, dout, (size_t)n * d.joiner * 4, hipMemcpyHostToDevice));
    std::vector<int> slots((size_t)n);
    for (int i = 0; i < n; ++i) slots[(size_t)i] = i;
    HIP_CHECK(hipMemcpy(step_d_, slots.data(), (size_t)n * 4, hipMemcpyHostToDevice));
    GemmArgs g; g.a0 = eout_; g.a0b = dout_; g.lda0 = d.joiner; g.aidx0 = step_d_; g.K0 = d.joiner; g.a_op = AOP_TANH_ADD;
    lin(g, L_.w_out); g.M = n; g.N = L_.vocab_pad; g.K = d.joiner; g.kz = kz_out_; g.epi = EPI_PARTIAL; g.out = ws_; g.m_stride = ws_mstride_;
    launch_gemm(g, stream_);
    float *lg = dmalloc<float>((size_t)n * L_.vocab_pad);
    RowArgs r; r.mode = ROW_SLOT_STORE; r.ws = ws_; r.parts = gemm_partials(n, L_.vocab_pad, kz_out_); r.m_stride = ws_mstride_; r.N = L_.vocab_pad; r.M = n;
    r.bias = w_ + L_.b_out; r.out = lg; r.ldo = L_.vocab_pad;
    launch_row(r, stream_);
    sync();
    std::vector<float> host((size_t)n * L_.vocab_pad);
    HIP_CHECK(hipMemcpy(host.data(), lg, host.size() * 4, hipMemcpyDeviceToHost));
    for (int i = 0; i < n; ++i) memcpy(logits + (size_t)i * d.vocab, host.data() + (size_t)i * L_.vocab_pad, (size_t)d.vocab * 4);
    (void)hipFree(lg);
    zero_slots(n);
}

void Engine::debug_decide(int n, int op, const float *logits, float early_emit, const int *now_ms, int round, int32_t *state_io, StepRecord *rec_out)
{
    debug_decide_impl(n, op, logits, early_emit, now_ms, round, state_io, rec_out, nullptr, nullptr);
}

void Engine::debug_decide_biased(int n, int op, const float *logits, float early_emit, const int *now_ms, int round, int32_t *state_io, StepRecord *rec_out,
                                 const BiasSet &set, int32_t *bias_state_io)
{
    debug_decide_impl(n, op, logits, early_emit, now_ms, round, state_io, rec_out, &set, bias_state_io);
}

void Engine::debug_decide_opts(int n, int op, const float *logits, float early_emit, const int *now_ms, int round, int32_t *state_io, StepRecord *rec_out,
                               const BiasSet *set, int32_t *bias_state_io, const SearchOpt *opts)
{
    debug_decide_impl(n, op, logits, early_emit, now_ms, round, state_io, rec_out, set, bias_state_io, opts);
}

void Engine::debug_decide_impl(int n, int op, const float *logits, float early_emit, const int *now_ms, int round, int32_t *state_io, StepRecord *rec_out,
                               const BiasSet *set, int32_t *bias_state_io, const SearchOpt *opts)
{
    std::lock_guard<std::mutex> cg(capture_mu_);
    HipLegacyLock legacy;
    const NetDims &d = L_.dims;
    HIP_CHECK(hipSetDevice(cfg_.device));
    if (n > cfg_.max_batch || n > cfg_.max_slots) { LOGE("debug_decide: n too large"); abort(); }
    static_assert(sizeof(GreedyState) == 16, "GreedyState is 4 x int32 in the ABI");
    std::vector<int> slots((size_t)n);
    for (int i = 0; i < n; ++i) slots[(size_t)i] = i;
    int *slots_d = dmalloc<int>((size_t)n), *now_d = dmalloc<int>((size_t)n), *active_d = dmalloc<int>((size_t)n), *dirty_d = dmalloc<int>((size_t)n);
    StepRecord *rec_d = dmalloc<StepRecord>((size_t)n);
    HIP_CHECK(hipMemcpy(slots_d, slots.data(), (size_t)n * 4, hipMemcpyHostToDevice));
    HIP_CHECK(hipMemcpy(gstate_, state_io, (size_t)n * sizeof(GreedyState), hipMemcpyHostToDevice));
    int32_t *bset_d = nullptr, *bstate_d = nullptr; BiasDesc *bdesc_d = nullptr; void *barrays_d = nullptr;
    if (set) {
        std::vector<int32_t> bset((size_t)n), bstate((size_t)n);
        for (int i = 0; i < n; ++i) { bset[(size_t)i] = bias_state_io[i] < 0 ? -1 : 0; bstate[(size_t)i] = std::max(0, bias_state_io[i]); }
        bset_d = dmalloc<int32_t>((size_t)n); bstate_d = dmalloc<int32_t>((size_t)n); bdesc_d = dmalloc<BiasDesc>(1);
        const BiasDesc desc = upload_bias(*set, &barrays_d, stream_);
        HIP_CHECK(hipStreamSynchronize(stream_));
        HIP_CHECK(hipMemcpy(bset_d, bset.data(), (size_t)n * 4, hipMemcpyHostToDevice));
        HIP_CHECK(hipMemcpy(bstate_d, bstate.data(), (size_t)n * 4, hipMemcpyHostToDevice));
        HIP_CHECK(hipMemcpy(bdesc_d, &desc, sizeof desc, hipMemcpyHostToDevice));
    }
    SearchOpt *opt_d = nullptr;
// ... 174 lines not shown
```

### april_asr_amd/csrc/engine.h

```cpp
#pragma once
#include <hip/hip_runtime.h>
#include <atomic>
#include <cstdint>
#include <deque>
#include <array>
#include <functional>
#include <map>
#include <memory>
#include <mutex>
#include <string>
#include <utility>
#include <vector>
#include "bias.h"
#include "fbank_tables.h"
#include "resample.h"
#include "input_format.h"
#include "kernels.h"
#include "host_pool.h"
#include "model_loader.h"

namespace aprilx {

struct PackedLayout {
    NetDims dims;
    size_t conv_w[3], conv_b[3];
    int k3 = 0;
    size_t w_embed, b_embed;
    struct Layer { size_t wg, bg, whr, wff1, bff1, wff2, bff2; };
    std::vector<Layer> layers;
    size_t w_encproj, b_encproj, emb, dec_conv, dec_conv_b, w_decproj, b_decproj, w_out, b_out;
    size_t total = 0;
    int vocab_pad = 0;
    bool has_dec_conv_b = false;
    std::vector<float> norm_eps;
    float embed_eps = 0;
};
void plan_layout(const NetDims &d, bool has_dec_conv_b, PackedLayout &L);
std::vector<std::pair<size_t, size_t>> gemm_sections(const PackedLayout &L);
void pack_weights(const HostModel &m, PackedLayout &L, std::vector<float> &blob);

std::recursive_mutex &hip_legacy_mutex();
struct HipLegacyLock { std::lock_guard<std::recursive_mutex> g; HipLegacyLock() : g(hip_legacy_mutex()) {} };

struct EngineConfig {
    int device = 0;
    int max_slots = 4096;
    int max_batch = 2048;
    int precision = 0;
};

struct KernelTiming { double ms = 0; long launches = 0; };

struct GraphCache {
    using Key = std::array<int, 3>;
    const char *name; size_t cap;
    bool full() const { return map_.size() >= cap; }
    hipGraphExec_t find(const Key &k) const { auto it = map_.find(k); return it == map_.end() ? nullptr : it->second; }
    void insert(const Key &k, hipGraphExec_t g) { map_[k] = g; }
    int use(int m, int T = 0) { return ++uses_[std::make_pair(m, T)]; }
    void clear();
    std::map<Key, hipGraphExec_t> map_; std::map<std::pair<int, int>, int> uses_;
};

struct RampStep { int macro = 0, own = 0; std::vector<std::pair<int, int>> guests; };
std::vector<RampStep> ramp_window(int L, int T, int R, int max_problems = 3);

class Engine {
public:
    Engine(const EngineConfig &cfg, const PackedLayout &layout, const float *blob_host, const float *blob_device,
           const ModelParams &params, const FbankHostTables &ft, const std::vector<uint8_t> &tok_class);
    ~Engine();

    int device() const { return cfg_.device; }
    int max_batch() const { return cfg_.max_batch; }
    int max_slots() const { return cfg_.max_slots; }
    int ring_frames() const { return ring_frames_; }
    const NetDims &dims() const { return L_.dims; }
    hipStream_t stream() const { return stream_; }
    const float *weights_device() const { return w_; }
    float *weights_mut() { return w_; }
    void finish_weights();
    int precision() const { return cfg_.precision; }
    int tile_ok() const { return cfg_.precision == 0 ? 1 : 0; }
    bool f16_tile() const { return f16_tile_; }
    const PackedLayout &layout() const { return L_; }

    int alloc_slot();
    void free_slot(int slot);
    int live_slots() const { return live_.load(std::memory_order_relaxed); }

    void fbank(int n_frames, const FbankFrameDesc *desc, const std::pair<const int16_t *, size_t> *parts, size_t n_parts, size_t n_pcm,
               HostPool *pool = nullptr);
    void set_resample_pass(int n, ResampleDesc *rs, const ResampleSpec *const *specs, const std::pair<const int16_t *, size_t> *in_parts,
                           size_t n_in_parts, size_t n_in)
    {
        rs_n_ = n; rs_desc_ = rs; rs_specs_ = specs; rs_in_parts_ = in_parts; rs_n_in_parts_ = n_in_parts; rs_n_in_ = n_in;
    }
    void set_decode_pass(int n, const DecodeDesc *dc, const std::pair<const uint8_t *, size_t> *raw_parts, size_t n_raw_parts, size_t n_raw)
    {
        dc_n_ = n; dc_desc_ = dc; dc_raw_parts_ = raw_parts; dc_n_raw_parts_ = n_raw_parts; dc_n_raw_ = n_raw;
    }
    void decode_counts(uint64_t *launches, uint64_t *frames) const
    {
        *launches = dc_launches_.load(std::memory_order_relaxed); *frames = dc_frames_.load(std::memory_order_relaxed);
    }
    void begin_flight();
    bool flight_has_room(int rows, int nsteps = 1) const;
    int step(int m, const int *slots, const int *ring_tails, const int *now_ms, float *logits_out = nullptr);
    int lm_step(int m, int T, const int *slots, const int *ring_tails, const int *now_ms, float *logits_out = nullptr, int mode = 0);
    int lm_max_rows() const { return cfg_.max_batch; }
    void decode_rows(int n, const int *slots, int op);
    int close_flight();
    bool flight_done(int parity);
    void wait_flight(int parity);
    void end_flight();
    bool profiling() const { return profiling_; }
    void set_overlap_hint(bool on) { overlap_hint_ = on; }
    const StepRecord *records(int step_index) const { return rec_h_ + rec_off_h_[step_index]; }
    void set_slot_confidence(int slot, int k)
    {
        std::lock_guard<std::mutex> g(conf_mu_);
        conf_pending_.push_back(std::make_pair(slot, k));
        if (k > 0) conf_ever_.store(true, std::memory_order_relaxed);
        conf_has_pending_.store(true, std::memory_order_release);
    }
    const ConfRecord *conf_records(int step_index) const { return conf_h_ ? conf_h_ + rec_off_h_[step_index] : nullptr; }
    uint64_t confidence_records() const { return conf_copied_.load(std::memory_order_relaxed); }
    static constexpr int kBiasSets = 64;
    bool set_slot_bias(int slot, const std::shared_ptr<const BiasSet> &set)
    {
        std::lock_guard<std::mutex> g(bias_mu_);
        if (slot < 0 || slot >= cfg_.max_slots) return false;
        if (bias_slot_set_.empty()) {
            if (!set) return true;
            bias_slot_set_.assign((size_t)cfg_.max_slots, -1); bias_sets_.resize(kBiasSets);
        }
        int idx = -1;
        if (set) {
            if (set->vocab != L_.dims.vocab || set->vocab > kBiasMaxVocab) return false;
            for (int i = 0; i < kBiasSets && idx < 0; ++i) if (bias_sets_[(size_t)i].set == set) idx = i;
            for (int i = 0; i < kBiasSets && idx < 0; ++i) if (!bias_sets_[(size_t)i].set) idx = i;
            if (idx < 0) return false;
            bias_sets_[(size_t)idx].set = set;
            ++bias_sets_[(size_t)idx].users;
        }
        const int old = bias_slot_set_[(size_t)slot];
        if (old < 0 && idx < 0) return true;
        if (old >= 0) --bias_sets_[(size_t)old].users;
        bias_slot_set_[(size_t)slot] = idx;
        bias_pending_.push_back(std::make_pair(slot, idx));
        if (set) bias_ever_.store(true, std::memory_order_relaxed);
        bias_has_pending_.store(true, std::memory_order_release);
        return true;
    }
    int read_bias_state(int slot);
    void debug_decide_biased(int n, int op, const float *logits, float early_emit, const int *now_ms, int round, int32_t *state_io, StepRecord *rec_out,
                             const BiasSet &set, int32_t *bias_state_io);
    void set_slot_search_options(int slot, SearchOpt o)
    {
        std::lock_guard<std::mutex> g(opt_mu_);
        if (o.endpoint_ms == 0 && !opt_ever_.load(std::memory_order_relaxed)) return;
        opt_pending_.push_back(std::make_pair(slot, o));
        if (o.endpoint_ms) opt_ever_.store(true, std::memory_order_relaxed);
        opt_has_pending_.store(true, std::memory_order_release);
    }
    void debug_decide_opts(int n, int op, const float *logits, float early_emit, const int *now_ms, int round, int32_t *state_io, StepRecord *rec_out,
                           const BiasSet *set, int32_t *bias_state_io, const SearchOpt *opts);
    void sync();
    void sync_streams();

    void debug_encoder(int n, const float *x, const float *h, const float *c, float *eout, float *h2, float *c2);
    void debug_decoder(int n, const int64_t *ctx, float *dout);
    void debug_joiner(int n, const float *eout, const float *dout, float *logits);
    void debug_decide(int n, int op, const float *logits, float early_emit, const int *now_ms, int round, int32_t *state_io, StepRecord *rec_out);
    void debug_confidence(int n, const float *logits, int k, ConfRecord *out, const BiasSet *set = nullptr, const int32_t *bias_state = nullptr);
    void debug_fbank(int n_frames, const int16_t *pcm_frames , float *out );
    void debug_resample(const ResampleSpec *spec, const int16_t *pcm, size_t n, int16_t *out);
    void debug_decode(uint32_t encoding, uint32_t channels, int32_t channel, const void *data, size_t n_frames, int16_t *out);
    void read_ring(int slot, int row, int n_rows, float *out);
    void read_greedy_state(int slot, GreedyState *out);

    void set_profiling(bool on);
    void set_gates_clock(bool on);
    void gates_clock(double *ms, long *launches, long *rows) const { *ms = gclk_ms_; *launches = gclk_launches_; *rows = gclk_rows_; }
    void gates_clock_by_n(double *ms4, long *launches4) const { for (int i = 0; i < 4; ++i) { ms4[i] = gclk_ms_n_[i]; launches4[i] = gclk_launches_n_[i]; } }
    KernelTiming timing(int cls) const { return timing_[cls]; }
    void ramp_counts(uint64_t *hosted, uint64_t *eligible);
    void reset_timing();
    enum { T_GATES = 0, T_GEMM_OTHER = 1, T_ROW = 2, T_CONV = 3, T_FBANK = 4, T_DEC = 5, T_RESAMPLE = 6, T_DECODE = 7, T_COUNT = 8 };
    long kernels_per_step() const { return kernels_per_step_.load(std::memory_order_relaxed); }

private:
    void upload_tables(const FbankHostTables &ft);
    void zero_slots(int n);
    void run_encoder_rows(int n, const float *x_direct);
    void encoder_front(size_t r0, int rows, const int *row_slots, const float *x_direct, hipStream_t st, float *ws);
    void lm_stage_layer(int l, int m, int t0, int t1, hipStream_t st);
    void lm_stage_proj(int m, int t0, int t1, hipStream_t st, float *ws);
    enum { GATES_ALL = 0xF, GATES_X = 0x3, GATES_H = 0xC };
    RowScale in_scale(int l, size_t r0) const;
    GemmArgs args_gates(int l, size_t r0, int rows, int waves) const;
    GemmArgs args_whr(int l, size_t r0, int rows) const;
    GemmArgs args_ff1(int l, size_t r0, int rows) const;
    GemmArgs args_ff2(int l, size_t r0, int rows) const;
    GemmArgs args_encproj(size_t r0, int rows, const int *slot_idx, float *out) const;
    AdvanceArgs advance_args(int m, int T) const;
    struct GreedyIo {
        int gen = 1;
        const int *now = nullptr;
        const float *eout = nullptr;
        const int *eout_rows = nullptr;
        const int *rec_off = nullptr; int rec_slot0 = 0;
        float *dump = nullptr;
    };
    void run_greedy_rounds(int n, bool dump_logits, int chunk = 0, const float *eout_rows = nullptr);
    void run_greedy_rounds(int n, const GreedyIo &io);
    void run_lm_chain(int m, int T, bool dump_logits);
    void run_lm_wavefront(int m, int T, bool dump_logits);
    struct SwPlan {
        struct Batch { size_t off; int n, macro, kind; size_t roff; int rn; };
        struct Chain { std::vector<GemmArgs> host; GemmArgs *dev = nullptr; std::vector<Batch> batches; std::vector<RowArgs> rhost; RowArgs *rdev = nullptr; };
        Chain one;
        Chain split;
        bool hosts = false;
        const Chain &layers(bool split_feed) const { return split_feed && !split.batches.empty() ? split : one; }
        std::vector<std::pair<int, long>> stamp_slots; std::vector<int> stamp_n;
    };
    GraphCache::Key graph_key(int m, int T = 0, int part = 0) const { return {m, T, flight_parity_ * 4 + part}; }
    GraphCache::Key sw_key(int m, int T, int part = 0) const { return graph_key(gclk_ ? -m : m, T, part); }
    SwPlan &sw_plan(int m, int T);
    void build_sw_chain(SwPlan &p, SwPlan::Chain &c, int m, int T, bool ramp);
    void free_sw_plans();
    void run_sw_chain(int m, int T, bool dump_logits, const SwPlan &p, int part, hipStream_t st);
    int stage_step(int m, int T, const int *slots, const int *ring_tails, const int *now_ms); void read_back_logits(int k, int rows, float *out);
    template <typename Chain> hipGraphExec_t cached_graph(GraphCache &cache, const GraphCache::Key &key, hipStream_t st, Chain &&chain);
    template <typename Capture> void capture_both_parities(Capture &&capture);
    void run_feed_wavefront(int m, int T, bool dump_logits); void run_layer_major(int m, int T, bool dump_logits); void launch_split_feed(int m, int T, hipStream_t fe);
    struct StreamTrace { hipEvent_t ev[6] = {nullptr, nullptr, nullptr, nullptr, nullptr, nullptr}; int m = 0, T = 0; bool used = false; };
    std::deque<StreamTrace> trace_; hipEvent_t trace_base_ = nullptr;
    StreamTrace *trace_slot();
    void dump_stream_trace();
    void select_parity(int p);
    void join(hipStream_t waiter, hipStream_t src);
    void general_prologue();
    int next_step_index() { ++flight_steps_; return (int)(step_seq_++ & (uint64_t)(2 * step_cap_ - 1)); }
    void launch_rowepi(GemmArgs fused_form, float *ws, hipStream_t st, bool force = false, int cls = T_GEMM_OTHER);
    bool gates_tile_rows(long rows) const;
    void run_decproj(int n, const int *d_slots, const int *row_mask, const int *run_flag, int run_gen, float *out = nullptr);
    void build_dec_table();
    void run_chain(int m, bool dump_logits);
    void collect_gates_clock();
    void timed_begin(int cls);
    void timed_end(int cls);
    void collect_timing();
    DecEmbedParams dec_params() const;

    EngineConfig cfg_;
    PackedLayout L_;
    ModelParams P_;
    hipStream_t stream_ = nullptr;
    float *w_ = nullptr;
    uint16_t *wh_ = nullptr;
    void lin(GemmArgs &g, size_t off) const { if (wh_) { g.wp = wh_ + off; g.wt = 1; } else { g.wp = w_ + off; g.wt = 0; } }
    bool f16_tile_ = false;
    uint16_t *wx_ = nullptr;
    uint16_t *y16_ = nullptr, *xb16_ = nullptr, *u16_ = nullptr, *ff16_ = nullptr;
    uint16_t *h16_ = nullptr;
    int kzx_hr_ = 1, kzx_ff2_ = 1;
    void lin16(GemmArgs &g, size_t off) const { g.wp = wx_ + off; g.wt = 1; g.tile_ok = 2; }
    int kz_hr() const { return f16_tile_ ? kzx_hr_ : kz_hr_; }
    int kz_ff2() const { return f16_tile_ ? kzx_ff2_ : kz_ff2_; }
    float *h_ = nullptr, *c_ = nullptr, *ring_ = nullptr, *eout_ = nullptr, *dout_ = nullptr;
    GreedyState *gstate_ = nullptr;
    float *dec_table_ = nullptr;
    uint8_t *cls_ = nullptr;
    int ring_frames_ = 0;
    float *xin_ = nullptr, *a3_ = nullptr, *y_ = nullptr, *ssq_ = nullptr, *xb_ = nullptr, *u_ = nullptr, *ff_ = nullptr, *ws_ = nullptr, *ws_g_ = nullptr, *de_ = nullptr;
    float *logits_ = nullptr;
    float *p_lm_ = nullptr, *eout_lm_ = nullptr;
    int *ring_h_ = nullptr; size_t ring_cap_ = 0, ring_pos_ = 0;
    int *step_off_h_ = nullptr, *rec_off_h_ = nullptr; int step_cap_ = 0;
    StepRecord *rec_d_ = nullptr, *rec_h_ = nullptr; size_t rec_cap_ = 0, rec_pos_ = 0;
    int flight_parity_ = 0, next_parity_ = 0; size_t ring_base_ = 0, rec_base_ = 0; int flight_steps_ = 0;
    uint64_t step_seq_ = 0;
    hipEvent_t flight_done_[2] = {nullptr, nullptr};
    std::mutex conf_mu_;
    std::vector<std::pair<int, int>> conf_pending_;
    std::atomic<bool> conf_has_pending_{false}, conf_ever_{false};
    uint8_t *conf_k_d_ = nullptr, *conf_k_h_ = nullptr;
    ConfRecord *conf_d_ = nullptr, *conf_h_ = nullptr;
    std::vector<std::pair<size_t, size_t>> conf_spans_;
    std::atomic<uint64_t> conf_copied_{0};
    void apply_confidence_pending();
    void drop_graphs();
    struct BiasEntry { std::shared_ptr<const BiasSet> set; int users = 0; void *dev = nullptr; };
    std::mutex bias_mu_;
    std::vector<BiasEntry> bias_sets_;
    std::vector<int> bias_slot_set_;
    std::vector<std::pair<int, int>> bias_pending_;
    std::atomic<bool> bias_has_pending_{false}, bias_ever_{false};
    int32_t *bias_set_d_ = nullptr, *bias_set_h_ = nullptr, *bias_state_d_ = nullptr;
    BiasDesc *bias_desc_d_ = nullptr, *bias_desc_h_ = nullptr;
    void apply_bias_pending();
    std::mutex opt_mu_;
    std::vector<std::pair<int, SearchOpt>> opt_pending_;
    std::atomic<bool> opt_has_pending_{false}, opt_ever_{false};
    SearchOpt *opt_d_ = nullptr, *opt_h_ = nullptr;
    void apply_search_options_pending();
    BiasDesc upload_bias(const BiasSet &set, void **dev, hipStream_t st);
    void debug_decide_impl(int n, int op, const float *logits, float early_emit, const int *now_ms, int round, int32_t *state_io, StepRecord *rec_out,
                           const BiasSet *set, int32_t *bias_state_io, const SearchOpt *opts = nullptr);
    void note_conf_step(int k, const int *slots, int m, size_t records);
    bool flight_open_[2] = {false, false};
    hipStream_t f_stream_ = nullptr, s_stream_ = nullptr, search_stream_ = nullptr;
    std::vector<hipEvent_t> join_ev_; size_t join_pos_ = 0;
    bool f_unseen_by_m_ = false, s_unseen_by_m_ = false, m_unseen_by_f_ = false, m_unseen_by_s_ = false, flight_tail_s_ = false;
    bool overlap_hint_ = false;
    int split_streams_ = 2;
    int ramp_mode_ = 1;
    RampState *ramp_d_ = nullptr;
    std::atomic<bool> m_quiet_{false};
    void m_touched() { m_quiet_.store(false, std::memory_order_release); }
    std::atomic<uint64_t> ramp_eligible_{0};
    float *xb_buf_[2] = {nullptr, nullptr}, *u_buf_[2] = {nullptr, nullptr}, *ff_buf_[2] = {nullptr, nullptr};
    uint16_t *xb16_buf_[2] = {nullptr, nullptr}, *u16_buf_[2] = {nullptr, nullptr}, *ff16_buf_[2] = {nullptr, nullptr};
    float *y_buf_[2] = {nullptr, nullptr}, *ssq_buf_[2] = {nullptr, nullptr}, *eout_lm_buf_[2] = {nullptr, nullptr}, *ws_fe_ = nullptr, *ws_sr_ = nullptr;
    uint16_t *y16_buf_[2] = {nullptr, nullptr};
    int *step_buf_[2] = {nullptr, nullptr}, *flags_buf_[2] = {nullptr, nullptr}, *rec_off_buf_[2] = {nullptr, nullptr};
    int *counter_d_ = nullptr, *step_d_ = nullptr, *active_d_ = nullptr, *dirty_d_ = nullptr, *rec_off_d_ = nullptr, *flags_d_ = nullptr;
    int *dec_slots_d_ = nullptr;
    float *logits_h_ = nullptr;
    FbankFrameDesc *hs_desc_[2] = {nullptr, nullptr}, *ds_desc_[2] = {nullptr, nullptr}; int desc_cap_ = 0;
    int16_t *hs_pcm_[2] = {nullptr, nullptr}, *ds_pcm_[2] = {nullptr, nullptr}; size_t pcm_cap_ = 0;
    int fb_flip_ = 0;
    hipEvent_t fb_done_[2] = {nullptr, nullptr};
    std::vector<size_t> part_off_;
    size_t rs_cap_ = 0;
    int rs_n_ = 0;
    ResampleDesc *rs_desc_ = nullptr;
    const ResampleSpec *const *rs_specs_ = nullptr;
    const std::pair<const int16_t *, size_t> *rs_in_parts_ = nullptr;
    size_t rs_n_in_parts_ = 0, rs_n_in_ = 0;
    size_t dc_cap_ = 0;
    int dc_n_ = 0;
    const DecodeDesc *dc_desc_ = nullptr;
    const std::pair<const uint8_t *, size_t> *dc_raw_parts_ = nullptr;
    size_t dc_n_raw_parts_ = 0, dc_n_raw_ = 0;
    std::atomic<uint64_t> dc_launches_{0}, dc_frames_{0};
    std::mutex rs_mu_;
    std::map<const ResampleSpec *, const float *> rs_tables_;
    const float *resample_table(const ResampleSpec *spec);
    FbankTables ft_;
    std::vector<void *> table_allocs_;
    float pad_value_ = 0;
    std::vector<int> free_, zero_pending_;
    void zero_pending_slots();
    std::atomic<int> live_{0};
    std::mutex slot_mu_;
    std::mutex capture_mu_;
    int kz_embed_ = 1, kz_hr_ = 1, kz_ff2_ = 1, kz_proj_ = 1, kz_out_ = 1;
    int ws_mstride_ = 0;
    float *conv_wt_ = nullptr;
    bool use_graphs_ = true;
    GraphCache step_graphs_{"chunk step", 256};
    GraphCache lm_graphs_{"layer-major chain", 32};
    GraphCache lm_search_graphs_{"long-feed search", 64};
    GraphCache sw_graphs_{"feed wavefront", 4 * 64};
    size_t sw_plan_cap_ = 64;
    std::map<GraphCache::Key, SwPlan> sw_plans_;
    hipStream_t lm_stream_ = nullptr;
    std::vector<hipEvent_t> lm_events_;
    GemmArgs *zargs_h_ = nullptr, *zargs_d_ = nullptr; size_t zargs_region_ = 0, zargs_pos_ = 0;
    hipEvent_t zargs_done_[3] = {nullptr, nullptr, nullptr}; bool zargs_busy_[3] = {false, false, false}; int zargs_next_ = 0;
    int *lm_now_d_ = nullptr, *lm_rows_d_ = nullptr, *lm_rec_off_d_ = nullptr;
    std::atomic<long> kernels_per_step_{0};
    long launch_count_ = 0;
    bool profiling_ = false;
    bool gclk_ = false, gclk_warned_ = false; unsigned long long *gclk_slots_ = nullptr; int gclk_used_ = 0;
    static constexpr int GCLK_SLOTS = 2048;
    double gclk_ms_ = 0; long gclk_launches_ = 0, gclk_rows_ = 0; double gclk_ms_n_[4] = {0, 0, 0, 0}; long gclk_launches_n_[4] = {0, 0, 0, 0};
    struct Ev { hipEvent_t a, b; int cls; };
    std::vector<Ev> ev_pool_; size_t ev_used_ = 0;
    KernelTiming timing_[T_COUNT];
};

}
```

### april_asr_amd/csrc/kernels.h

```cpp
#pragma once
#include <hip/hip_runtime.h>
#include <cstdint>

namespace aprilx {

enum GemmEpilogue {
    EPI_PARTIAL = 0,
    EPI_LSTM = 1,
    EPI_BIAS_DSWISH = 2,
    EPI_HR = 3,
    EPI_RESID_SSQ = 4,
    EPI_SLOT_STORE = 5,
    EPI_XPART = 6
};
enum GemmAOp { AOP_NONE = 0, AOP_TANH_ADD = 1 };
enum GemmMode { GM_SLAB = 0, GM_FULLK = 1, GM_TILE = 2, GM_KW = 3, GM_PP = 4 };


constexpr int SSQ_COLS = 32;

struct RowScale {
    const float *ssq = nullptr;
    int groups = 0;
    float inv_n = 0.0f;
    float eps = 0.0f;
};

struct GreedyState { int32_t ctx0, ctx1; int32_t last_tok; uint32_t last_emit_ms; };

constexpr int STAMP_WORDS = 144, STAMP_ENDS = 8, STAMP_NENDS = 64, STAMP_SUBS = 72;

struct GemmArgs {
    const float *a0 = nullptr; int lda0 = 0; const int *aidx0 = nullptr; int K0 = 0;
    const float *a1 = nullptr; int lda1 = 0; const int *aidx1 = nullptr; int K1 = 0;
    const float *a0b = nullptr;
    const int *aidx0b = nullptr; int same_idx_b = 1;
    const GreedyState *ctx_state = nullptr; int ctx_vocab = 0;
    int a_op = AOP_NONE;
    RowScale x_scale;
    const void *wp = nullptr;
    int wt = 0;
    int M = 0, N = 0, K = 0;
    int kz = 1;
    int zs = 1;
    int mode = GM_SLAB;
    int epi = EPI_PARTIAL;
    float *out = nullptr; int ldo = 0;
    void *out16 = nullptr;
    void *state16 = nullptr;
    int m_stride = 0;
    const float *bias = nullptr;
    float *c_state = nullptr;
    const int *slot_idx = nullptr;
    int hidden = 0;
    float *state = nullptr; int ld_state = 0;
    const float *resid = nullptr; int ldr = 0;
    RowScale r_scale;
    float *ssq_out = nullptr;
    const int *row_mask = nullptr;
    const int *run_flag = nullptr;
    int run_gen = 1;
    int wave_mask = 0xF;
    const float *p_add = nullptr; int ldp = 0;
    int force_fullk = 0;
    int zcount = 1;
    int tile_ok = 0;
    int asm_loop = 0;
    unsigned long long *trace = nullptr;
    unsigned long long *stamp = nullptr;
    int debug = 0;
};
void launch_gemm(const GemmArgs &g, hipStream_t s);
void gemm_profile_next_launch(hipEvent_t start, hipEvent_t stop);
bool gemm_profile_pending();
void launch_gemm_tile(const GemmArgs &g, int mt, int nt, const GemmArgs *dev_args, int n, hipStream_t s);
int gemm_kw_waves(const GemmArgs &g);
bool gemm_pp_ok(const GemmArgs &g, int mt);
void launch_gemm_pp(const GemmArgs &g, int mt, const GemmArgs *dev_args, int n, hipStream_t s);
bool gemm_pw_ok(const GemmArgs &g);
void launch_gemm_pw(const GemmArgs &g, const GemmArgs *dev_args, int n, hipStream_t s);
void gemm_pp_pin(int enable, int mt);
bool gemm_kw_has_kernel(const GemmArgs &g, int mt, int nt);
void launch_gemm_kw(const GemmArgs &g, int mt, int nt, const GemmArgs *dev_args, int n, hipStream_t s);
void gemm_kw_pin(int enable, int mt);
int recur_form(const GemmArgs &g);
void launch_recur(const GemmArgs &g, int form, const GemmArgs *dev_args, int n, hipStream_t s);
void stage_gemm_z(const GemmArgs *items, int n, GemmArgs *staged);
void launch_gemm_z(const GemmArgs *staged, int n, const GemmArgs *dev_args, hipStream_t s);
int gemm_partials(int M, int N, int kz, int zcount = 1, int tile_ok = 0);
bool gemm_fullk(int M, int N, int kz, bool force = false, int zcount = 1, int tile_ok = 0);
bool gemm_tile_planned(int M, int N, int kz, int zcount = 1);
void gemm_tile_pin(int enable, int mt, int zs);

enum RowMode {
    ROW_HR = 0,
    ROW_RESID_SSQ = 1,
    ROW_SLOT_STORE = 2
};
struct RowArgs {
    int mode = ROW_HR;
    const float *ws = nullptr; int parts = 1; int m_stride = 0; int N = 0; int M = 0;
    const float *bias = nullptr;
    const float *resid = nullptr; int ldr = 0;
    RowScale r_scale;
    float *out = nullptr; int ldo = 0;
    const int *slot_idx = nullptr;
    float *state = nullptr; int ld_state = 0;
    float *ssq_out = nullptr;
    void *out16 = nullptr, *state16 = nullptr;
    const int *row_mask = nullptr;
    const int *run_flag = nullptr;
    int run_gen = 1;
};
void launch_row(const RowArgs &r, hipStream_t s);
void launch_row_z(const RowArgs *host_args, int n, const RowArgs *dev_args, hipStream_t s);

constexpr int RAMP_R = 2;
struct RampState {
    unsigned long long ready[2];
    int head_live[2];
    int guest_live[2][RAMP_R][RAMP_R];
    unsigned generation;
    unsigned hosted;
};
constexpr int RAMP_MAX_M = 0xFFFFF, RAMP_MAX_T = 0xFF;
void launch_ramp_ready(RampState *rs, int q, int m, int T, int hostable, hipStream_t s);
void launch_ramp_latch(RampState *rs, int p, int m, hipStream_t s);

struct StepRecord { int32_t idx; float max_val; float blank_val; uint32_t flags; };
constexpr int kConfMaxAlt = 8;
struct ConfRecord { float lse; float blank_val; int32_t n_alt; uint32_t reserved; int32_t alt_id[kConfMaxAlt]; float alt_logit[kConfMaxAlt]; };
static_assert(sizeof(ConfRecord) == 80, "ConfRecord is 20 x 32 bit");
enum { REC_VALID = 1, REC_BLANK = 2, REC_CTX = 4 };
enum TokClassBits { TKC_WORD_START = 1, TKC_SENT_END = 2, TKC_COMMA = 4, TKC_DOT = 8, TKC_DIGIT_START = 16 };

struct BiasDesc { const int32_t *state_off = nullptr, *edge_tok = nullptr, *edge_next = nullptr; const float *edge_bonus = nullptr; int32_t n_states = 0, flags = 0; };

struct SearchOpt { uint32_t endpoint_ms; float blank_penalty; };
static_assert(sizeof(SearchOpt) == 8, "SearchOpt is 2 x 32 bit");

struct DecEmbedParams {
    const float *emb = nullptr;
    const float *conv_w = nullptr;
    const float *conv_b = nullptr;
    int d = 0, groups = 0, context = 0, vocab = 0;
};

struct DecideArgs {
    const float *ws = nullptr; int parts = 1; int m_stride = 0; int N = 0; int M = 0;
    int n_valid = 0;
    const float *bias = nullptr;
    int blank = 0;
    float early_emit = 0.0f;
    const int *slot_idx = nullptr;
    const int *now_ms = nullptr;
    int *active = nullptr;
    int gen = 1;
    int rec_slot = 0;
    int *dirty = nullptr;
    const uint8_t *tok_class = nullptr;
    GreedyState *state = nullptr;
    StepRecord *rec = nullptr;
    StepRecord *rec_ring = nullptr;
    const int *rec_off = nullptr; int round = 0;
    float *logits_dump = nullptr;
    DecEmbedParams dec;
    float *de_out = nullptr; int ld_de = 0;
    int *run_flags = nullptr;
    int *rerun_flags = nullptr;
    const uint8_t *conf_k = nullptr;
    ConfRecord *conf_ring = nullptr;
    ConfRecord *conf = nullptr; int conf_k_all = 0;
    const int32_t *bias_set = nullptr;
    int32_t *bias_state = nullptr;
    const BiasDesc *bias_desc = nullptr;
    const SearchOpt *opt = nullptr;
};
void launch_decide(const DecideArgs &a, hipStream_t s);

struct DecRowsArgs {
    const int *slot_idx = nullptr; int M = 0;
    int op = 0; int blank = 0;
    GreedyState *state = nullptr;
    DecEmbedParams dec;
    float *de_out = nullptr; int ld_de = 0;
    int32_t *bias_state = nullptr;
};
void launch_dec_rows(const DecRowsArgs &a, hipStream_t s);

struct DecEmbedArgs {
    DecEmbedParams dec;
    const int *ctx = nullptr;
    int M = 0;
    float *out = nullptr; int ldo = 0;
};
void launch_dec_embed(const DecEmbedArgs &a, hipStream_t s);

struct AdvanceArgs {
    const int *host_ring = nullptr;
    const int *host_step_off = nullptr;
    const int *host_rec_off = nullptr;
    int *counter = nullptr;
    int index_mask = 0x7fffffff;
    int *dst = nullptr; int dst_stride = 0;
    int n_arrays = 3; int len[4] = {0, 0, 0, 0};
    int *rec_off = nullptr;
    int *flags = nullptr; int n_flags = 0;
};
void launch_advance(const AdvanceArgs &a, hipStream_t s);

struct ZeroSlotArgs {
    float *h = nullptr, *c = nullptr; int n_layers = 0; size_t slots = 0; int d_model = 0, hidden = 0;
    float *eout = nullptr, *dout = nullptr; int joiner = 0;
    GreedyState *state = nullptr; int blank = 0;
    int slot = 0;
    void *h16 = nullptr;
    int n_list = 0; int list[64] = {0};
};
void launch_zero_slot(const ZeroSlotArgs &a, hipStream_t s);

struct BlockSetupArgs {
    const int *now_src = nullptr; int *now_dst = nullptr;
    int *rows_dst = nullptr; int row0 = 0; int count = 0;
    const int *rec_off_step = nullptr; int *rec_off_block = nullptr; int rec_add = 0;
    int *flags = nullptr; int n_flags = 0;
};
void launch_block_setup(const BlockSetupArgs &a, hipStream_t s);

struct ConvEmbedArgs {
    const float *ring = nullptr;
    int ring_frames = 0, mel = 0, seg = 0;
    const int *slot_idx = nullptr;
    const int *ring_tail = nullptr;
    const float *w[3] = {nullptr, nullptr, nullptr};
    const float *b[3] = {nullptr, nullptr, nullptr};
    int ch[3] = {0, 0, 0};
    int ch1_per_group = 0;
    int stride[3] = {1, 2, 2};
    float *out = nullptr; int ldo = 0;
    int M = 0;
    const float *x_direct = nullptr;
    const float *w0t = nullptr, *w1t = nullptr;
};
void launch_conv_embed(const ConvEmbedArgs &a, hipStream_t s);
void launch_conv_weight_transpose(const float *w0, const float *w1, int c0, int c1, float *w0t, float *w1t, hipStream_t s);

void launch_cvt_f16(const float *src, void *dst, size_t n, hipStream_t s);

void launch_repack_x32(const float *src_packed, void *dst, int K, int N, hipStream_t s);

struct FbankTables {
    const float *window = nullptr;
    const double *tw[16] = {nullptr};
    const double *tws[16] = {nullptr};
    int fct[16] = {0}; int nfct = 0;
    const float *mel = nullptr;
    const int *mel_lo = nullptr;
    const int *mel_hi = nullptr;
    int padded = 0, nbins = 0;
};
struct FbankFrameDesc { int32_t slot; int32_t ring_row; int32_t pcm_off; };
struct FbankArgs {
    FbankTables t;
    const int16_t *pcm = nullptr;
    const FbankFrameDesc *desc = nullptr;
    int n_frames = 0;
    float *ring = nullptr; int ring_frames = 0;
    float pad_value = 0.0f;
};
void launch_fbank(const FbankArgs &a, hipStream_t s);

struct ResampleDesc {
    const float *taps = nullptr;
    int64_t in_base = 0;
    int64_t out_first = 0;
    int64_t out_end = 0;
    int32_t in_off = 0, in_n = 0;
    int32_t out_dst = 0, out_cnt = 0;
    int32_t L = 1, M = 1, K = 0, ldt = 0;
};
// ... 29 lines not shown
```

### april_asr_amd/csrc/kernels_misc.hip

```cpp
#include "kernels.h"
#include "device_utils.h"
#include "env.h"
#include <algorithm>
#include <cstdio>
#include <cstdlib>

namespace aprilx {

template <int MODE>
__device__ __forceinline__ void row_body(const RowArgs &r)
{
    if (r.run_flag && *r.run_flag != r.run_gen) return;
    const int m = blockIdx.x;
    const int tid = threadIdx.x;
    const int slot = r.slot_idx ? r.slot_idx[m] : m;
    if (MODE == ROW_SLOT_STORE) { if (r.row_mask && !r.row_mask[m]) return; }
    float rs = 1.0f;
    const bool scaled = MODE == ROW_HR || (MODE == ROW_SLOT_STORE && r.r_scale.ssq != nullptr);
    if (scaled) rs = row_scale(r.r_scale, m);
    const int nq = r.N >> 2;
    for (int q0 = 0; q0 < nq; q0 += 256) {
        const int q = q0 + tid;
        const bool ok = q < nq;
        const int n = q * 4;
        f32x4 s = f32x4{0.f, 0.f, 0.f, 0.f};
        if (ok) s = tree_sum4(r.ws, r.parts, r.m_stride, r.N, m, n);
        if (MODE == ROW_HR) {
            if (ok) {
                const HrTail t = hr_tail(s, *reinterpret_cast<const f32x4 *>(r.resid + (size_t)m * r.ldr + n), rs);
                *reinterpret_cast<f32x4 *>(r.state + (size_t)slot * r.ld_state + n) = t.state;
                *reinterpret_cast<f32x4 *>(r.out + (size_t)m * r.ldo + n) = t.out;
                if (r.state16) *reinterpret_cast<h4 *>(reinterpret_cast<_Float16 *>(r.state16) + (size_t)slot * r.ld_state + n) = to_h4(t.state);
                if (r.out16) *reinterpret_cast<h4 *>(reinterpret_cast<_Float16 *>(r.out16) + (size_t)m * r.ldo + n) = to_h4(t.out);
            }
        } else if (MODE == ROW_RESID_SSQ) {
            f32x4 y = f32x4{0.f, 0.f, 0.f, 0.f};
            if (ok) {
                const f32x4 res = r.resid ? *reinterpret_cast<const f32x4 *>(r.resid + (size_t)m * r.ldr + n) : f32x4{0.f, 0.f, 0.f, 0.f};
                y = resid_tail(s, *reinterpret_cast<const f32x4 *>(r.bias + n), res, r.resid != nullptr);
                *reinterpret_cast<f32x4 *>(r.out + (size_t)m * r.ldo + n) = y;
                if (r.out16) *reinterpret_cast<h4 *>(reinterpret_cast<_Float16 *>(r.out16) + (size_t)m * r.ldo + n) = to_h4(y);
            }
            float ss;
            if (granule_ssq_store(y, ok, q, ss)) r.ssq_out[(size_t)m * (r.N / SSQ_COLS) + n / SSQ_COLS] = ss;
        } else {
            if (ok) {
                const f32x4 b = *reinterpret_cast<const f32x4 *>(r.bias + n);
                *reinterpret_cast<f32x4 *>(r.out + (size_t)slot * r.ldo + n) = scaled ? slot_value(s, rs, b) : slot_value(s, b);
            }
        }
    }
}

template <int MODE>
__global__ __launch_bounds__(256) void row_kernel(RowArgs r) { row_body<MODE>(r); }

template <int MODE>
__global__ __launch_bounds__(256) void row_zkernel(const RowArgs *__restrict__ zargs)
{
    const RowArgs r = zargs[blockIdx.y];
    row_body<MODE>(r);
}

void launch_row(const RowArgs &r, hipStream_t s)
{
    dim3 grid((unsigned)r.M), block(256);
    switch (r.mode) {
    case ROW_HR: hipLaunchKernelGGL(row_kernel<ROW_HR>, grid, block, 0, s, r); break;
    case ROW_RESID_SSQ: hipLaunchKernelGGL(row_kernel<ROW_RESID_SSQ>, grid, block, 0, s, r); break;
    default: hipLaunchKernelGGL(row_kernel<ROW_SLOT_STORE>, grid, block, 0, s, r); break;
    }
}

void launch_row_z(const RowArgs *host_args, int n, const RowArgs *dev_args, hipStream_t s)
{
    if (n <= 0) return;
    const RowArgs &r = host_args[0];
    for (int i = 1; i < n; ++i)
        if (host_args[i].mode != r.mode || host_args[i].M != r.M || host_args[i].N != r.N || host_args[i].parts != r.parts) {
            fprintf(stderr, "libapril(mi355x): launch_row_z: the problems of one launch must have one shape\n"); abort();
        }
    dim3 grid((unsigned)r.M, (unsigned)n), block(256);
    switch (r.mode) {
    case ROW_HR: hipLaunchKernelGGL(row_zkernel<ROW_HR>, grid, block, 0, s, dev_args); break;
    case ROW_RESID_SSQ: hipLaunchKernelGGL(row_zkernel<ROW_RESID_SSQ>, grid, block, 0, s, dev_args); break;
    default: hipLaunchKernelGGL(row_zkernel<ROW_SLOT_STORE>, grid, block, 0, s, dev_args); break;
    }
}

__global__ __launch_bounds__(64) void ramp_ready_kernel(RampState *rs, int q, int m, int T, int hostable)
{
    if (threadIdx.x != 0) return;
    __hip_atomic_store(&rs->head_live[q], 1, __ATOMIC_RELAXED, __HIP_MEMORY_SCOPE_AGENT);
    const unsigned g = __hip_atomic_load(&rs->generation, __ATOMIC_RELAXED, __HIP_MEMORY_SCOPE_AGENT) + 1u;
    __hip_atomic_store(&rs->generation, g, __ATOMIC_RELAXED, __HIP_MEMORY_SCOPE_AGENT);
    __builtin_amdgcn_fence(__ATOMIC_RELEASE, "agent");
    asm volatile("s_waitcnt vmcnt(0)" ::: "memory");
    const unsigned long long rec = ((unsigned long long)g << 32) | ((unsigned long long)(unsigned)m << 12) | ((unsigned long long)(unsigned)T << 4) | (unsigned long long)(hostable & 1);
    __hip_atomic_store(&rs->ready[q], rec, __ATOMIC_RELAXED, __HIP_MEMORY_SCOPE_AGENT);
}

__global__ __launch_bounds__(64) void ramp_latch_kernel(RampState *rs, int p, int m)
{
    if (threadIdx.x != 0) return;
    const unsigned long long mine = __hip_atomic_load(&rs->ready[p], __ATOMIC_RELAXED, __HIP_MEMORY_SCOPE_AGENT);
    const unsigned long long next = __hip_atomic_load(&rs->ready[1 - p], __ATOMIC_RELAXED, __HIP_MEMORY_SCOPE_AGENT);
    const unsigned g = (unsigned)(mine >> 32);
    const int next_m = (int)((next >> 12) & RAMP_MAX_M), next_T = (int)((next >> 4) & RAMP_MAX_T);
    const bool host = (unsigned)(next >> 32) == g + 1u && next_m == m && (int)((mine >> 12) & RAMP_MAX_M) == m && (next & 1ull) != 0;
    if (host) {
        __builtin_amdgcn_fence(__ATOMIC_ACQUIRE, "agent");
        __hip_atomic_store(&rs->head_live[1 - p], 0, __ATOMIC_RELAXED, __HIP_MEMORY_SCOPE_AGENT);
        rs->hosted += 1u;
    }
    for (int j = 1; j <= RAMP_R; ++j)
        for (int t = 0; t < RAMP_R; ++t) rs->guest_live[p][j - 1][t] = (host && t < j && t < next_T) ? 1 : 0;
}

void launch_ramp_ready(RampState *rs, int q, int m, int T, int hostable, hipStream_t s)
{
    hipLaunchKernelGGL(ramp_ready_kernel, dim3(1), dim3(64), 0, s, rs, q, m, T, hostable);
}
void launch_ramp_latch(RampState *rs, int p, int m, hipStream_t s)
{
    hipLaunchKernelGGL(ramp_latch_kernel, dim3(1), dim3(64), 0, s, rs, p, m);
}

__device__ __forceinline__ void dec_embed_row(const DecEmbedParams &p, int tok0, int tok1, float *out)
{
    const int cg = p.d / p.groups;
    for (int o = threadIdx.x; o < p.d; o += 256) {
        const int g0 = (o / cg) * cg;
        const float *w = p.conv_w + (size_t)o * cg * p.context;
        float acc = 0.0f;
        for (int ci = 0; ci < cg; ++ci) {
            acc += p.emb[(size_t)tok0 * p.d + g0 + ci] * w[ci * p.context + 0];
            acc += p.emb[(size_t)tok1 * p.d + g0 + ci] * w[ci * p.context + 1];
        }
        if (p.conv_b) acc += p.conv_b[o];
        out[o] = acc > 0.0f ? acc : 0.0f;
    }
}

#include "kernels_bias.inc"
#include "kernels_confidence.inc"

template <bool CONF, bool BIAS, bool OPT>
__device__ __forceinline__ void decide_body(const DecideArgs &a)
{
    extern __shared__ __attribute__((aligned(16))) unsigned char bias_lds[];
    __shared__ float s_best[4], s_blank[4];
    __shared__ int s_idx[4];
    __shared__ int s_ctx[3];
    if (a.round > 0 && a.run_flags && a.run_flags[a.round] != a.gen) return;
    const int m = blockIdx.x;
    const int tid = threadIdx.x;
    StepRecord *rec = a.rec ? a.rec + m : a.rec_ring + (size_t)a.rec_off[0] + (size_t)a.rec_slot * a.M + m;
    if (a.round > 0 && a.active[m] != a.gen) {
        if (tid == 0) { rec->idx = -1; rec->max_val = 0.0f; rec->blank_val = 0.0f; rec->flags = 0; a.dirty[m] = 0; }
        return;
    }
    float best = -9999999999.0f;
    int best_i = -1;
    float blank_v = 0.0f;
    BiasRow br;
    if (BIAS) bias_row_begin(a, m, bias_lds, br);
    if (BIAS && br.bonus) bias_scan(a, m, br, best, best_i, blank_v);
    else
    for (int n = tid; n < a.n_valid; n += 256) {
        const float v = tree_sum(a.ws, a.parts, a.m_stride, a.N, m, n) + a.bias[n];
        if (a.logits_dump) a.logits_dump[(size_t)m * a.n_valid + n] = v;
        if (n == a.blank) blank_v = v;
        else if (v > best) { best = v; best_i = n; }
    }
#pragma unroll
    for (int off = 32; off > 0; off >>= 1) {
        const float ov = __shfl_xor(best, off);
        const int oi = __shfl_xor(best_i, off);
        const bool take = (oi >= 0) && (best_i < 0 || ov > best || (ov == best && oi < best_i));
        if (take) { best = ov; best_i = oi; }
        blank_v += __shfl_xor(blank_v, off);
    }
    const int wave = tid >> 6;
    if ((tid & 63) == 0) { s_best[wave] = best; s_idx[wave] = best_i; s_blank[wave] = blank_v; }
    __syncthreads();
    if (tid == 0) {
        float b = s_best[0]; int bi = s_idx[0];
        for (int w = 1; w < 4; ++w) {
            const float ov = s_best[w]; const int oi = s_idx[w];
            if (oi >= 0 && (bi < 0 || ov > b || (ov == b && oi < bi))) { b = ov; bi = oi; }
        }
        float bl = s_blank[(a.blank & 255) >> 6];
        rec->idx = bi; rec->max_val = b; rec->blank_val = bl;

        const int slot = a.slot_idx[m];
        GreedyState st = a.state[slot];
        SearchOpt so; so.endpoint_ms = 0u; so.blank_penalty = 0.0f;
        if (OPT) { so = a.opt[slot]; if (so.endpoint_ms) bl = bl - so.blank_penalty; }
        int tok = bi; float tv = b;
        if (tok < 0) { tok = a.blank == 0 ? 1 : 0; tv = -9999999999.0f; }
        const bool cleared = st.ctx1 == a.blank;
        const bool same = st.ctx1 == tok;
        const float ee = same ? 0.0f : a.early_emit;
        bool is_blank = (bl - ee) > tv;
        const unsigned tc = a.tok_class[tok];
        bool punct = (tc & (TKC_SENT_END | TKC_COMMA)) != 0;
        if (punct && st.last_tok >= 0 && (a.tok_class[st.last_tok] & TKC_DIGIT_START) && (tc & TKC_DOT)) punct = false;
        if (!cleared && punct && !same && tv > (bl - 3.5f)) is_blank = false;
        const unsigned now = (unsigned)a.now_ms[m];
        unsigned flags = REC_VALID;
        bool rerun = false, silence = false;
        if (!is_blank) {
            st.last_emit_ms = now;
            st.ctx0 = st.ctx1; st.ctx1 = tok;
            st.last_tok = tok;
            rerun = true;
        } else {
            flags |= REC_BLANK;
            if (OPT && so.endpoint_ms) silence = now - st.last_emit_ms >= so.endpoint_ms;
            else if (now - st.last_emit_ms >= 2200u) { silence = true; }
            if (silence) {
                st.last_tok = -1;
                if (st.ctx0 != a.blank) { st.ctx0 = a.blank; st.ctx1 = a.blank; rerun = true; }
            }
        }
        a.active[m] = is_blank ? 0 : a.gen;
        if (rerun) flags |= REC_CTX;
        rec->flags = flags;
        a.state[slot] = st;
        if (BIAS && br.bonus) bias_row_end(a, br, slot, is_blank, tok, OPT ? silence : is_blank && now - st.last_emit_ms >= 2200u);
        a.dirty[m] = rerun ? 1 : 0;
        if (a.run_flags) {
            if (!is_blank && a.round < 2) a.run_flags[a.round + 1] = a.gen;
            if (rerun) a.rerun_flags[a.round] = a.gen;
        }
        s_ctx[0] = st.ctx0; s_ctx[1] = st.ctx1; s_ctx[2] = rerun ? 1 : 0;
    }
    __syncthreads();
    if (s_ctx[2] && a.de_out) dec_embed_row(a.dec, s_ctx[0], s_ctx[1], a.de_out + (size_t)m * a.ld_de);
    if (CONF) {
        if (a.conf) confidence_row(a, m, a.conf_k_all, a.conf + m, BIAS ? br.bonus : nullptr);
        else {
            const int k = a.conf_k[a.slot_idx[m]];
            if (k) confidence_row(a, m, k, a.conf_ring + (rec - a.rec_ring), BIAS ? br.bonus : nullptr);
        }
    }
}

__global__ __launch_bounds__(256) void decide_kernel(DecideArgs a) { decide_body<false, false, false>(a); }
__global__ __launch_bounds__(256) void decide_conf_kernel(DecideArgs a) { decide_body<true, false, false>(a); }
__global__ __launch_bounds__(256) void decide_bias_kernel(DecideArgs a) { decide_body<false, true, false>(a); }
__global__ __launch_bounds__(256) void decide_conf_bias_kernel(DecideArgs a) { decide_body<true, true, false>(a); }
__global__ __launch_bounds__(256) void decide_opt_kernel(DecideArgs a) { decide_body<false, false, true>(a); }
__global__ __launch_bounds__(256) void decide_conf_opt_kernel(DecideArgs a) { decide_body<true, false, true>(a); }
__global__ __launch_bounds__(256) void decide_bias_opt_kernel(DecideArgs a) { decide_body<false, true, true>(a); }
__global__ __launch_bounds__(256) void decide_conf_bias_opt_kernel(DecideArgs a) { decide_body<true, true, true>(a); }

void launch_decide(const DecideArgs &a, hipStream_t s)
{
    const bool conf = a.conf || a.conf_k;
    if (a.bias_set) {
        if (a.n_valid > 8192 || !a.bias_state || !a.bias_desc) { fprintf(stderr, "libapril(mi355x): launch_decide: phrase boosting needs a vocabulary of at most 8192 tokens and all three tables\n"); abort(); }
        const size_t lds = bias_lds_bytes(a.n_valid);
        if (a.opt) {
            if (conf) hipLaunchKernelGGL(decide_conf_bias_opt_kernel, dim3((unsigned)a.M), dim3(256), lds, s, a);
            else hipLaunchKernelGGL(decide_bias_opt_kernel, dim3((unsigned)a.M), dim3(256), lds, s, a);
        }
        else if (conf) hipLaunchKernelGGL(decide_conf_bias_kernel, dim3((unsigned)a.M), dim3(256), lds, s, a);
        else hipLaunchKernelGGL(decide_bias_kernel, dim3((unsigned)a.M), dim3(256), lds, s, a);
    }
    else if (a.opt) {
        if (conf) hipLaunchKernelGGL(decide_conf_opt_kernel, dim3((unsigned)a.M), dim3(256), 0, s, a);
        else hipLaunchKernelGGL(decide_opt_kernel, dim3((unsigned)a.M), dim3(256), 0, s, a);
    }
    else if (conf) hipLaunchKernelGGL(decide_conf_kernel, dim3((unsigned)a.M), dim3(256), 0, s, a);
    else hipLaunchKernelGGL(decide_kernel, dim3((unsigned)a.M), dim3(256), 0, s, a);
}

// ... 356 lines not shown
```

### april_asr_amd/csrc/ramp_api.cc

```cpp
#include <vector>
#include "../../include/april_api.h"
#include "../../include/aprilx_engine.h"
#include "common.h"
#include "session.h"

using namespace aprilx;

struct AprilASRModel_i { Model m; };

extern "C" {

int aprilx_ramp_window(int L, int T, int R, int32_t *out, int cap)
{
    if (L <= 0 || T <= 0 || R <= 0 || !out) return -1;
    const std::vector<RampStep> w = ramp_window(L, T, R);
    const int stride = 3 + 2 * R;
    if ((int)w.size() * stride > cap) return -1;
    for (size_t i = 0; i < w.size(); ++i) {
        int32_t *o = out + i * (size_t)stride;
        for (int k = 0; k < stride; ++k) o[k] = -1;
        o[0] = w[i].macro; o[1] = w[i].own; o[2] = (int32_t)w[i].guests.size();
        for (size_t g = 0; g < w[i].guests.size() && (int)g < R; ++g) { o[3 + 2 * g] = w[i].guests[g].first; o[4 + 2 * g] = w[i].guests[g].second; }
    }
    return (int)w.size();
}
int aprilx_model_ramp_stats(AprilASRModel model, int device_index, uint64_t *ramp_hosted, uint64_t *ramp_eligible)
{
    if (!model || device_index < 0 || device_index >= (int)model->m.engines.size() || !ramp_hosted || !ramp_eligible) return -1;
    model->m.engines[(size_t)device_index]->ramp_counts(ramp_hosted, ramp_eligible);
    return 0;
}

}
```

### include/aprilx_engine.h

```cpp
#ifndef APRILX_ENGINE_H
#define APRILX_ENGINE_H
#include "april_api.h"

#ifdef __cplusplus
extern "C" {
#endif

typedef struct AprilxDims {
    int32_t n_layers, d_model, hidden, ffn, joiner, vocab, mel, seg, seg_step, context;
    int32_t fft_size, frame_shift, sample_rate, blank_id, n_devices;
    int32_t precision;
    int32_t d_model_file;
    int64_t param_count;
} AprilxDims;
APRIL_EXPORT int aprilx_model_dims(AprilASRModel model, AprilxDims *out);
APRIL_EXPORT const char *aprilx_model_token(AprilASRModel model, int32_t id);

typedef struct AprilxLoadInfo {
    double broadcast_ms;
    double comm_init_ms;
    uint64_t broadcast_bytes;
    int32_t ranks;
    int32_t used_rccl;
} AprilxLoadInfo;
APRIL_EXPORT int aprilx_broadcast_get_id(void *id_out, size_t cap);
APRIL_EXPORT AprilASRModel aprilx_model_broadcast(AprilASRModel root_model, int rank, int world, const void *id_bytes);
APRIL_EXPORT int aprilx_model_load_info(AprilASRModel model, AprilxLoadInfo *out);
APRIL_EXPORT size_t aprilx_model_blob_size(AprilASRModel model);
APRIL_EXPORT int aprilx_model_export_blob(AprilASRModel model, void *dst, size_t dst_size);
APRIL_EXPORT AprilASRModel aprilx_model_from_blob(const void *blob, size_t size, int blob_is_device_ptr);
APRIL_EXPORT int aprilx_model_save_blob(AprilASRModel model, const char *path);
APRIL_EXPORT int aprilx_model_save_blob_f16(AprilASRModel model, const char *path);
APRIL_EXPORT AprilASRModel aprilx_model_load_blob(const char *path);

APRIL_EXPORT void aprilx_feed_many(size_t n, AprilASRSession *sessions, const short *const *pcm16, const size_t *short_counts);
APRIL_EXPORT void aprilx_flush_many(size_t n, AprilASRSession *sessions);
APRIL_EXPORT void aprilx_session_drain(AprilASRSession session);
APRIL_EXPORT void aprilx_feed_many_pipelined(size_t n, AprilASRSession *sessions, const short *const *pcm16, const size_t *short_counts, int depth);
APRIL_EXPORT void aprilx_drain_many(size_t n, AprilASRSession *sessions);

APRIL_EXPORT int aprilx_run_encoder(AprilASRModel model, int n, const float *x, const float *h, const float *c,
                                    float *eout, float *h2, float *c2);
APRIL_EXPORT int aprilx_run_decoder(AprilASRModel model, int n, const int64_t *context, float *dout);
APRIL_EXPORT int aprilx_run_joiner(AprilASRModel model, int n, const float *eout, const float *dout, float *logits);
APRIL_EXPORT int aprilx_run_fbank(AprilASRModel model, int n_frames, const int16_t *pcm_frames, float *out);
APRIL_EXPORT int aprilx_run_decide(AprilASRModel model, int n, int op, const float *logits, float early_emit, const int32_t *now_ms,
                                   int round, int32_t *state_io, void *records_out);

APRIL_EXPORT int aprilx_plan_gemm(int M, int N, int kz, int zcount, int tile_ok, int force, int32_t *out);

APRIL_EXPORT int aprilx_ramp_window(int L, int T, int R, int32_t *out, int cap);

APRIL_EXPORT int aprilx_stream_form(int kind, int M, int N, int K, int kz, int groups);

APRIL_EXPORT int aprilx_session_set_input_rate(AprilASRSession session, uint32_t rate_hz);
APRIL_EXPORT uint32_t aprilx_session_input_rate(AprilASRSession session);
APRIL_EXPORT int aprilx_resampler_taps(uint32_t in_rate, uint32_t out_rate, int32_t *lmk_out, float *taps, size_t cap);
APRIL_EXPORT int64_t aprilx_resample(AprilASRModel model, uint32_t in_rate, const int16_t *pcm, size_t n, int16_t *out, size_t cap);

enum { APRILX_ENC_S16 = 0, APRILX_ENC_MULAW = 1, APRILX_ENC_ALAW = 2, APRILX_ENC_F32 = 3 };
typedef struct AprilxInputFormat {
    uint32_t size;
    uint32_t encoding;
    uint32_t channels;
    int32_t channel;
} AprilxInputFormat;
APRIL_EXPORT int aprilx_session_set_input_format(AprilASRSession session, const AprilxInputFormat *format);
APRIL_EXPORT int aprilx_session_input_format(AprilASRSession session, AprilxInputFormat *out);
APRIL_EXPORT int aprilx_session_feed_bytes(AprilASRSession session, const void *data, size_t bytes);
APRIL_EXPORT int aprilx_feed_many_bytes(size_t n, AprilASRSession *sessions, const void *const *data, const size_t *byte_counts, int depth);
APRIL_EXPORT int64_t aprilx_decode_host(const AprilxInputFormat *format, const void *data, size_t bytes, int16_t *out, size_t cap);
APRIL_EXPORT int64_t aprilx_decode(AprilASRModel model, const AprilxInputFormat *format, const void *data, size_t bytes, int16_t *out, size_t cap);
APRIL_EXPORT int aprilx_model_decode_stats(AprilASRModel model, int device_index, uint64_t *launches, uint64_t *frames, double *ms);

typedef struct AprilxTokenInfo {
    uint32_t size;
    uint32_t n_alt;
    uint64_t eval_index;
    float lse;
    float token_logprob;
    float blank_logprob;
    float reserved0;
    int32_t alt_id[8];
    float alt_logit[8];
} AprilxTokenInfo;
APRIL_EXPORT int aprilx_session_set_confidence(AprilASRSession session, int n_alternatives);
APRIL_EXPORT int aprilx_session_confidence(AprilASRSession session);
APRIL_EXPORT int aprilx_run_confidence(AprilASRModel model, int n, const float *logits, int k, AprilxTokenInfo *out);

typedef struct AprilxBias_i *AprilxBias;
APRIL_EXPORT AprilxBias aprilx_bias_create(AprilASRModel model, size_t n, const char *const *phrases, const float *boosts, char *err, size_t err_cap);
#define APRILX_BIAS_STRICT 1u
APRIL_EXPORT AprilxBias aprilx_bias_create_ex(AprilASRModel model, size_t n, const char *const *phrases, const float *boosts, uint32_t flags, char *err,
                                              size_t err_cap);
APRIL_EXPORT int aprilx_bias_flags(AprilxBias bias);
APRIL_EXPORT void aprilx_bias_free(AprilxBias bias);
APRIL_EXPORT int aprilx_bias_info(AprilxBias bias, int32_t *states, int64_t *edges);
APRIL_EXPORT int aprilx_bias_edges(AprilxBias bias, int32_t state, int32_t *tok, int32_t *next, float *bonus, size_t cap);
APRIL_EXPORT int aprilx_session_set_bias(AprilASRSession session, AprilxBias bias);
APRIL_EXPORT int aprilx_session_bias_state(AprilASRSession session, int32_t *host_state, int32_t *device_state);
APRIL_EXPORT int aprilx_run_decide_biased(AprilASRModel model, int n, int op, const float *logits, float early_emit, const int32_t *now_ms, int round,
                                          int32_t *state_io, void *records_out, AprilxBias bias, int32_t *bias_state_io);
APRIL_EXPORT int aprilx_run_confidence_biased(AprilASRModel model, int n, const float *logits, int k, AprilxBias bias, const int32_t *bias_state,
                                              AprilxTokenInfo *out);

typedef struct AprilxSearchOptions {
    uint32_t size;
    uint32_t endpoint_silence_ms;
    uint32_t max_utterance_ms;
    float blank_penalty;
} AprilxSearchOptions;
APRIL_EXPORT int aprilx_session_set_search_options(AprilASRSession session, const AprilxSearchOptions *options);
APRIL_EXPORT int aprilx_session_search_options(AprilASRSession session, AprilxSearchOptions *out);
APRIL_EXPORT int aprilx_run_decide_opts(AprilASRModel model, int n, int op, const float *logits, float early_emit, const int32_t *now_ms, int round,
                                        int32_t *state_io, void *records_out, AprilxBias bias, int32_t *bias_state_io, const AprilxSearchOptions *opts);

APRIL_EXPORT void aprilx_session_trace_logits(AprilASRSession session, float *buf, size_t cap_floats, size_t *used_floats);
APRIL_EXPORT uint64_t aprilx_session_chunks(AprilASRSession session);
APRIL_EXPORT uint64_t aprilx_session_read_frames(AprilASRSession session, uint64_t first, int n, float *out);
APRIL_EXPORT void aprilx_session_context(AprilASRSession session, int32_t *host_ctx, int32_t *device_state);

typedef struct AprilxStats {
    uint64_t ticks, steps, chunks, rounds, frames, max_batch_seen;
    double kernel_ms[6];
    uint64_t kernel_launches[6];
    double host_ms[8];
    uint64_t flights;
    uint64_t replay_mismatch;
    uint64_t kernels_per_step;
    uint64_t lm_steps, lm_chunks;
    uint64_t wave_steps, wave_chunks;
    double gates_clock_ms; uint64_t gates_clock_launches, gates_clock_rows;
    double gates_clock_ms_by_n[4]; uint64_t gates_clock_launches_by_n[4];
    double resample_ms; uint64_t resample_launches;
    uint64_t confidence_records;
} AprilxStats;
APRIL_EXPORT void aprilx_model_stats(AprilASRModel model, int device_index, AprilxStats *out);
APRIL_EXPORT int aprilx_model_ramp_stats(AprilASRModel model, int device_index, uint64_t *ramp_hosted, uint64_t *ramp_eligible);
APRIL_EXPORT int aprilx_model_feed_latency(AprilASRModel model, int device_index, double *out_ms, int cap, int reset);
APRIL_EXPORT void aprilx_model_profile(AprilASRModel model, int enable);

typedef struct AprilxGreedy_i *AprilxGreedy;
APRIL_EXPORT AprilxGreedy aprilx_greedy_create(AprilASRModel model, AprilRecognitionResultHandler handler, void *userdata);
APRIL_EXPORT int aprilx_greedy_step(AprilxGreedy g, int32_t idx, float max_val, float blank_val, float early_emit,
                                    size_t now_ms, int32_t *ctx_out);
APRIL_EXPORT void aprilx_greedy_finish(AprilxGreedy g);
APRIL_EXPORT void aprilx_greedy_free(AprilxGreedy g);
APRIL_EXPORT int aprilx_greedy_set_bias(AprilxGreedy g, AprilxBias bias);
APRIL_EXPORT int aprilx_greedy_bias_state(AprilxGreedy g);
APRIL_EXPORT int aprilx_greedy_set_search_options(AprilxGreedy g, const AprilxSearchOptions *options);

APRIL_EXPORT void aprilx_counting_handler(void *userdata, AprilResultType type, size_t count, const AprilToken *tokens);

APRIL_EXPORT AprilASRModel aprilx_model_load_host(const char *model_path);
APRIL_EXPORT int aprilx_model_fbank_tables(AprilASRModel model, float *window, float *mel);

APRIL_EXPORT int aprilx_probe_file(const char *path, char *err, size_t err_cap);

#ifdef __cplusplus
}
#endif
#endif
```

Measured before the change: 20090.

## Replace device-side ramp latch with host-scheduled head/body/tail graph pieces

Removes the device RampState flags and the ready/latch kernels that decided at runtime whether the next feed's head layers would run inside the predecessor's tail. The layer wavefront is now cut into head, body and tail graphs. The host defers the tail and, when the next split feed is compatible, launches a merged tail that also carries the successor's head, so the successor skips its own head graph. This drops the per-feed flag kernels and predicated GEMMs, but adds host-side pending-tail state, a host callback per feed and more cached graphs.

Result: no change. 20200 (median of 6 runs) (+0.6%).

```diff
diff --git a/april_asr_amd/_ffi.py b/april_asr_amd/_ffi.py
--- a/april_asr_amd/_ffi.py
+++ b/april_asr_amd/_ffi.py
@@ -75,7 +75,7 @@
     "aprilx_run_decide_biased", "aprilx_greedy_set_bias", "aprilx_greedy_bias_state",
     "aprilx_bias_create_ex", "aprilx_bias_flags", "aprilx_run_confidence_biased",
     "aprilx_session_set_search_options", "aprilx_session_search_options", "aprilx_run_decide_opts", "aprilx_greedy_set_search_options",
-    "aprilx_ramp_window", "aprilx_model_ramp_stats",
+    "aprilx_ramp_window", "aprilx_ramp_pieces", "aprilx_model_ramp_stats",
     "aprilx_session_set_input_format", "aprilx_session_input_format", "aprilx_session_feed_bytes", "aprilx_feed_many_bytes",
     "aprilx_decode_host", "aprilx_decode", "aprilx_model_decode_stats",
 ]
@@ -126,6 +126,7 @@
     L.aprilx_run_fbank.argtypes = [vp, C.c_int, vp, vp]; L.aprilx_run_fbank.restype = C.c_int
     L.aprilx_plan_gemm.argtypes = [C.c_int] * 6 + [vp]; L.aprilx_plan_gemm.restype = C.c_int
     L.aprilx_ramp_window.argtypes = [C.c_int] * 3 + [vp, C.c_int]; L.aprilx_ramp_window.restype = C.c_int
+    L.aprilx_ramp_pieces.argtypes = [C.c_int] * 3 + [vp, C.c_int]; L.aprilx_ramp_pieces.restype = C.c_int
     L.aprilx_model_ramp_stats.argtypes = [vp, C.c_int, C.POINTER(C.c_uint64), C.POINTER(C.c_uint64)]; L.aprilx_model_ramp_stats.restype = C.c_int
     L.aprilx_stream_form.argtypes = [C.c_int] * 6; L.aprilx_stream_form.restype = C.c_int
     L.aprilx_run_decide.argtypes = [vp, C.c_int, C.c_int, vp, C.c_float, vp, C.c_int, vp, vp]; L.aprilx_run_decide.restype = C.c_int
diff --git a/april_asr_amd/csrc/engine.cc b/april_asr_amd/csrc/engine.cc
--- a/april_asr_amd/csrc/engine.cc
+++ b/april_asr_amd/csrc/engine.cc
@@ -225,7 +225,7 @@
     xb_ = xb_buf_[0]; u_ = u_buf_[0]; ff_ = ff_buf_[0];
     ramp_mode_ = env_int("APRIL_RAMP_MERGE", 1);
     if (ramp_mode_ < 0 || ramp_mode_ > 2) ramp_mode_ = 1;
-    ramp_d_ = dmalloc<RampState>(1); HIP_CHECK(hipMemset(ramp_d_, 0, sizeof(RampState)));
+    for (int i = 0; i < 2; ++i) HIP_CHECK(hipEventCreateWithFlags(&body_ev_[i], hipEventDisableTiming));
     de_ = dmalloc<float>(MB * d.d_model);
     HIP_CHECK(hipMemset(de_, 0, MB * d.d_model * 4));
     logits_ = dmalloc<float>(3 * MB * d.vocab);
@@ -313,12 +313,10 @@
 {
     HipLegacyLock legacy;
     (void)hipSetDevice(cfg_.device);
+    if (pend_.active) finish_tail(false);
     (void)hipStreamSynchronize(f_stream_); (void)hipStreamSynchronize(stream_); (void)hipStreamSynchronize(s_stream_);
     dump_stream_trace();
-    if (ramp_d_ && ramp_eligible_.load() > 0) {
-        unsigned h = 0;
-        if (hipMemcpy(&h, &ramp_d_->hosted, sizeof h, hipMemcpyDeviceToHost) == hipSuccess) LOGI("engine: ramp merge: %u of %llu hostable split feeds were hosted by their predecessor", h, (unsigned long long)ramp_eligible_.load());
-    }
+    if (ramp_eligible_.load() > 0) LOGI("engine: ramp merge: %llu split feeds ran their head in the predecessor's tail", (unsigned long long)ramp_hosted_.load());
     for (StreamTrace &t : trace_) for (hipEvent_t e : t.ev) if (e) (void)hipEventDestroy(e);
     if (trace_base_) (void)hipEventDestroy(trace_base_);
     for (hipEvent_t e : join_ev_) (void)hipEventDestroy(e);
@@ -347,7 +345,7 @@
                         (void *)xb16_buf_[p], (void *)u16_buf_[p], (void *)ff16_buf_[p], (void *)rec_off_buf_[p], (void *)flags_buf_[p], (void *)step_buf_[p]}) if (q) (void)hipFree(q);
     if (ws_fe_) (void)hipFree(ws_fe_);
     if (ws_sr_) (void)hipFree(ws_sr_);
-    for (void *p : {(void *)wx_, (void *)h16_, (void *)ramp_d_}) if (p) (void)hipFree(p);
+    for (void *p : {(void *)wx_, (void *)h16_}) if (p) (void)hipFree(p);
     for (void *p : {(void *)w_, (void *)wh_, (void *)h_, (void *)c_, (void *)ring_, (void *)eout_, (void *)dout_, (void *)gstate_, (void *)cls_, (void *)ws_, (void *)xin_,
                     (void *)a3_, (void *)de_, (void *)logits_, (void *)rec_d_, (void *)counter_d_,
                     (void *)active_d_, (void *)dirty_d_, (void *)dec_slots_d_,
@@ -357,6 +355,7 @@
         if (p) (void)hipHostFree(p);
     for (int b = 0; b < 2; ++b) if (fb_done_[b]) (void)hipEventDestroy(fb_done_[b]);
     for (int b = 0; b < 2; ++b) if (flight_done_[b]) (void)hipEventDestroy(flight_done_[b]);
+    for (int b = 0; b < 2; ++b) if (body_ev_[b]) (void)hipEventDestroy(body_ev_[b]);
     for (void *p : table_allocs_) (void)hipFree(p);
     (void)hipStreamDestroy(stream_); (void)hipStreamDestroy(f_stream_); (void)hipStreamDestroy(s_stream_);
 }
@@ -492,19 +491,22 @@
     if (!f) return;
     fprintf(f, "# one line per split feed; times in us since the first split feed; FE = index fetch + conv + embed on stream F, LY = layer wavefront on M, SR = encoder_proj + search on S\n");
     fprintf(f, "# feed sessions chunks  FE_start FE_end  LY_start LY_end  SR_start SR_end   overlap: FE inside the previous feed's LY window? SR inside the next feed's LY window?\n");
-    std::vector<std::array<float, 6>> ts;
+    fprintf(f, "# a cut layer chain adds: tail=plain|merged body_end tail_start (LY_end is the tail's end; a hosted feed's LY starts at its body, its head ran in the previous line's merged tail)\n");
+    std::vector<std::array<float, 8>> ts; std::vector<const StreamTrace *> of;
     for (StreamTrace &t : trace_) {
-        std::array<float, 6> a{};
+        std::array<float, 8> a{};
         bool ok = t.used;
-        for (int i = 0; i < 6 && ok; ++i) ok = hipEventElapsedTime(&a[(size_t)i], trace_base_, t.ev[i]) == hipSuccess;
-        if (ok) ts.push_back(a); else (void)hipGetLastError();
+        for (int i = 0; i < (t.tail ? 8 : 6) && ok; ++i) ok = hipEventElapsedTime(&a[(size_t)i], trace_base_, t.ev[i]) == hipSuccess;
+        if (ok) { ts.push_back(a); of.push_back(&t); } else (void)hipGetLastError();
     }
     for (size_t i = 0; i < ts.size(); ++i) {
         const auto &a = ts[i];
         const bool fe_in_prev = i > 0 && a[0] * 1e3f < ts[i - 1][3] * 1e3f && a[1] * 1e3f > ts[i - 1][2] * 1e3f;
         const bool sr_in_next = i + 1 < ts.size() && a[5] > ts[i + 1][2] && a[4] < ts[i + 1][3];
-        fprintf(f, "%4zu %5d %2d  %10.1f %10.1f  %10.1f %10.1f  %10.1f %10.1f   %s %s\n", i, trace_[i].m, trace_[i].T, a[0] * 1e3, a[1] * 1e3, a[2] * 1e3, a[3] * 1e3, a[4] * 1e3, a[5] * 1e3,
+        fprintf(f, "%4zu %5d %2d  %10.1f %10.1f  %10.1f %10.1f  %10.1f %10.1f   %s %s", i, of[i]->m, of[i]->T, a[0] * 1e3, a[1] * 1e3, a[2] * 1e3, a[3] * 1e3, a[4] * 1e3, a[5] * 1e3,
                 fe_in_prev ? "FE<prevLY" : "-", sr_in_next ? "SR<nextLY" : "-");
+        if (of[i]->tail) fprintf(f, "   tail=%s %10.1f %10.1f", of[i]->tail == 2 ? "merged" : "plain", a[6] * 1e3, a[7] * 1e3);
+        fprintf(f, "\n");
     }
     fclose(f);
 }
@@ -600,7 +602,7 @@
     HIP_CHECK(hipSetDevice(cfg_.device));
     for (int i = 0; i < n_rs; ++i) rs[i].taps = resample_table(rs_specs_[i]);
     if (n_frames > desc_cap_ || n_pcm + n_in + raw_units > pcm_cap_ || (size_t)n_rs > rs_cap_ || (size_t)n_dc > dc_cap_) {
-        sync();
+        { std::lock_guard<std::mutex> cg(capture_mu_); sync(); }
         HipLegacyLock regrow_guard;
         for (int b = 0; b < 2; ++b) {
             if (hs_desc_[b]) { (void)hipHostFree(hs_desc_[b]); (void)hipFree(ds_desc_[b]); }
@@ -1112,7 +1114,7 @@
     }
     SwPlan &p = sw_plans_[key];
     build_sw_chain(p, p.one, m, T, false);
-    if (ramp_mode_ != 0 && !gclk_) build_sw_chain(p, p.split, m, T, true);
+    if (ramp_mode_ != 0 && !gclk_) build_sw_chain(p, p.merged, m, T, true);
     return p;
 }
 
@@ -1130,14 +1132,27 @@
     return w;
 }
 
+RampPieces ramp_pieces(int L, int T, int R)
+{
+    RampPieces p;
+    const std::vector<RampStep> w = ramp_window(L, T, R);
+    if (w.empty()) return p;
+    p.ok = true;
+    p.head[0] = 1; p.head[1] = R;
+    p.body[0] = R + 1; p.body[1] = w.front().macro - 1;
+    p.tail[0] = w.front().macro; p.tail[1] = w.back().macro;
+    return p;
+}
+
 void Engine::ramp_counts(uint64_t *hosted, uint64_t *eligible)
 {
-    unsigned h = 0;
-    {
-        HipLegacyLock legacy;
-        if (hipSetDevice(cfg_.device) == hipSuccess) HIP_CHECK(hipMemcpy(&h, &ramp_d_->hosted, sizeof h, hipMemcpyDeviceToHost));
-    }
-    *hosted = h; *eligible = ramp_eligible_.load(std::memory_order_relaxed);
+    *hosted = ramp_hosted_.load(std::memory_order_relaxed); *eligible = ramp_eligible_.load(std::memory_order_relaxed);
+}
+
+void Engine::m_touched()
+{
+    if (pend_.active) finish_tail(false);
+    m_quiet_.store(false, std::memory_order_release);
 }
 
 void Engine::build_sw_chain(SwPlan &p, SwPlan::Chain &c, int m, int T, bool ramp)
@@ -1151,17 +1166,18 @@
         return (kind == 1 || kind == 3) && tk && (tk == 2 || gemm_tile_planned(m, d.d_model, kz, n)) && !gemm_fullk(m, d.d_model, kz, false, n, tk);
     };
     std::vector<RampStep> window;
-    if (ramp && m <= RAMP_MAX_M && T <= RAMP_MAX_T) {
+    if (ramp) {
         window = ramp_window(L, T, RAMP_R);
         for (const RampStep &s : window) if (needs_rows(1, s.own + (int)s.guests.size()) || needs_rows(3, s.own + (int)s.guests.size())) { window.clear(); break; }
-    }
-    if (ramp) p.hosts = !window.empty();
+        if (window.empty()) return;
+        p.pieces = ramp_pieces(L, T, RAMP_R);
+    }
     std::vector<GemmArgs> items;
     std::vector<RowArgs> rows;
     for (int W = 0; W <= T + L; ++W) {
-        const RampStep *host = nullptr; int wj = 0;
-        for (size_t j = 0; j < window.size(); ++j) if (window[j].macro == W) { host = &window[j]; wj = (int)j; }
-        if (host && wj == 0) { SwPlan::Batch b; b.off = c.host.size(); b.n = 0; b.macro = W; b.kind = 4; b.roff = c.rhost.size(); b.rn = 0; c.batches.push_back(b); }
+        const RampStep *host = nullptr;
+        for (size_t j = 0; j < window.size(); ++j) if (window[j].macro == W) host = &window[j];
+        if (ramp && !host) continue;
         for (int kind = 0; kind < 4; ++kind) {
             items.clear(); rows.clear();
             int n_act = 0;
@@ -1170,11 +1186,10 @@
             if (host) n_act += (int)host->guests.size();
             const int kz = kind == 1 ? kz_hr() : kz_ff2();
             const bool split = needs_rows(kind, n_act);
-            auto problem = [&](int l, int t, const int *run_flag) {
+            auto problem = [&](int l, int t) {
                 const size_t r0 = (size_t)t * m;
                 GemmArgs g = kind == 0 ? args_gates(l, r0, m, GATES_ALL) : kind == 1 ? args_whr(l, r0, m) : kind == 2 ? args_ff1(l, r0, m) : args_ff2(l, r0, m);
                 if (kind == 0 && cfg_.precision == 0) g.tile_ok = gates_tile_rows((long)m * n_act) ? 2 : 0;
-                if (run_flag) { g.run_flag = run_flag; g.run_gen = 1; }
                 if (split) {
                     float *ws = ws_ + r0 * d.d_model;
                     rows.push_back(row_form(g, ws, ws_mstride_, gemm_partials(m, d.d_model, kz, n_act, tk)));
@@ -1185,11 +1200,11 @@
             for (int l = 0; l < L; ++l) {
                 const int t = W - 1 - l;
                 if (t < 0 || t >= T) continue;
-                problem(l, t, ramp && W <= RAMP_R ? &ramp_d_->head_live[par] : nullptr);
+                problem(l, t);
             }
             if (host) {
                 select_parity(1 - par);
-                for (const auto &lt : host->guests) problem(lt.first, lt.second, &ramp_d_->guest_live[par][wj][lt.second]);
+                for (const auto &lt : host->guests) problem(lt.first, lt.second);
                 select_parity(par);
             }
             std::vector<int> groups;
@@ -1230,11 +1245,11 @@
 void Engine::free_sw_plans()
 {
     if (!sw_plans_.empty()) LOGI("engine: feed wavefront plans emptied (%zu plans)", sw_plans_.size());
-    for (auto &p : sw_plans_) for (SwPlan::Chain *c : {&p.second.one, &p.second.split}) { if (c->dev) (void)hipFree(c->dev); if (c->rdev) (void)hipFree(c->rdev); }
+    for (auto &p : sw_plans_) for (SwPlan::Chain *c : {&p.second.one, &p.second.merged}) { if (c->dev) (void)hipFree(c->dev); if (c->rdev) (void)hipFree(c->rdev); }
     sw_graphs_.clear(); sw_plans_.clear();
 }
 
-void Engine::run_sw_chain(int m, int T, bool dump_logits, const SwPlan &p, int part, hipStream_t st)
+void Engine::run_sw_chain(int m, int T, bool dump_logits, const SwPlan &p, int part, hipStream_t st, int piece)
 {
     const NetDims &d = L_.dims;
     const int MB = cfg_.max_batch;
@@ -1244,10 +1259,11 @@
     }
     if (part < 0 || part == 1) {
         static const int cls_of[4] = {T_GATES, T_GEMM_OTHER, T_GEMM_OTHER, T_GEMM_OTHER};
-        const SwPlan::Chain &c = p.layers(part == 1);
+        const SwPlan::Chain &c = piece == SW_MERGED ? p.merged : p.one;
+        const int *range = piece == SW_HEAD ? p.pieces.head : piece == SW_BODY ? p.pieces.body : piece ? p.pieces.tail : nullptr;
         for (size_t bi = 0; bi < c.batches.size(); ++bi) {
             const SwPlan::Batch &b = c.batches[bi];
-            if (b.kind == 4) { launch_ramp_latch(ramp_d_, flight_parity_, m, st); continue; }
+            if (range && (b.macro < range[0] || b.macro > range[1])) continue;
             timed_begin(cls_of[b.kind]); launch_gemm_z(c.host.data() + b.off, b.n, c.dev + b.off, st); timed_end(cls_of[b.kind]);
             if (b.rn > 0) { timed_begin(T_ROW); launch_row_z(c.rhost.data() + b.roff, b.rn, c.rdev + b.roff, st); timed_end(T_ROW); }
         }
@@ -1295,8 +1311,11 @@
     if (graphs && !sw_graphs_.find(sw_key(m, T, split ? 1 : 0)))
         capture_both_parities([&]() {
             const SwPlan &pl = sw_plan(m, T);
-            if (split) for (int part = 0; part < 3; ++part) cached_graph(sw_graphs_, sw_key(m, T, 1 + part), on[part], [&]() { run_sw_chain(m, T, false, pl, part, on[part]); });
-            else cached_graph(sw_graphs_, sw_key(m, T), stream_, [&]() { run_sw_chain(m, T, false, pl, -1, stream_); });
+            if (split) {
+                for (int part = 0; part < 3; ++part)
+                    if (part != 1 || !pl.pieces.ok) cached_graph(sw_graphs_, sw_key(m, T, 1 + part), on[part], [&]() { run_sw_chain(m, T, false, pl, part, on[part]); });
+                if (pl.pieces.ok) for (int piece = SW_HEAD; piece <= SW_MERGED; ++piece) cached_graph(sw_graphs_, sw_key(m, T, piece), stream_, [&]() { run_sw_chain(m, T, false, pl, 1, stream_, piece); });
+            } else cached_graph(sw_graphs_, sw_key(m, T), stream_, [&]() { run_sw_chain(m, T, false, pl, -1, stream_); });
         });
     if (split) { launch_split_feed(m, T, on[0]); return; }
     general_prologue();
@@ -1304,8 +1323,18 @@
     launch_count_ = 0; run_sw_chain(m, T, dump_logits, sw_plan(m, T), -1, stream_); kernels_per_step_ = (launch_count_ + 1 + T - 1) / T;
 }
 
+static void body_done_fn(void *flag) { static_cast<std::atomic<uint32_t> *>(flag)->store(1u, std::memory_order_release); }
+
 void Engine::launch_split_feed(int m, int T, hipStream_t fe)
 {
+    const SwPlan &pl = sw_plan(m, T);
+    const bool cut = pl.pieces.ok;
+    const int par = flight_parity_;
+    bool hosted = false;
+    if (pend_.active) {
+        hosted = cut && ramp_mode_ == 1 && fe == f_stream_ && pend_.closed && pend_.m == m && pend_.parity == 1 - par && m_quiet_.load(std::memory_order_acquire);
+        if (!hosted) m_touched();
+    }
     if (fe == f_stream_) {
         if (m_unseen_by_f_) { join(f_stream_, stream_); m_unseen_by_f_ = false; }
     } else if (f_unseen_by_m_) { join(stream_, f_stream_); f_unseen_by_m_ = false; }
@@ -1317,18 +1346,62 @@
         if (tr) HIP_CHECK(hipEventRecord(tr->ev[2 * i + 1], st));
     };
     part(0, fe);
-    if (ramp_mode_ != 0) {
-        const bool hostable = ramp_mode_ == 1 && fe == f_stream_ && m_quiet_.load(std::memory_order_acquire);
-        if (hostable) ramp_eligible_.fetch_add(1, std::memory_order_relaxed);
-        launch_ramp_ready(ramp_d_, flight_parity_, m, T, hostable ? 1 : 0, fe);
-    }
     if (fe == f_stream_) { join(stream_, f_stream_); f_unseen_by_m_ = false; }
-    part(1, stream_);
-    if (ramp_mode_ != 0) m_quiet_.store(true, std::memory_order_release);
-    join(s_stream_, stream_); part(2, s_stream_);
-    if (tr) { tr->m = m; tr->T = T; tr->used = true; }
-    s_unseen_by_m_ = true; flight_tail_s_ = true;
+    if (hosted) {
+        ramp_eligible_.fetch_add(1, std::memory_order_relaxed); ramp_hosted_.fetch_add(1, std::memory_order_relaxed);
+        finish_tail(true);
+    }
     if (fe != f_stream_) m_unseen_by_f_ = true;
+    if (tr) { tr->m = m; tr->T = T; }
+    if (!cut) {
+        part(1, stream_);
+        join(s_stream_, stream_); part(2, s_stream_);
+        if (tr) tr->used = true;
+        s_unseen_by_m_ = true; flight_tail_s_ = true;
+        return;
+    }
+    if (tr) HIP_CHECK(hipEventRecord(tr->ev[2], stream_));
+    if (!hosted) HIP_CHECK(hipGraphLaunch(sw_graphs_.find(sw_key(m, T, SW_HEAD)), stream_));
+    HIP_CHECK(hipGraphLaunch(sw_graphs_.find(sw_key(m, T, SW_BODY)), stream_));
+    if (tr) HIP_CHECK(hipEventRecord(tr->ev[6], stream_));
+    body_done_[par].store(0u, std::memory_order_release);
+    HIP_CHECK(hipEventRecord(body_ev_[par], stream_));
+    HIP_CHECK(hipStreamWaitEvent(s_stream_, body_ev_[par], 0));
+    HIP_CHECK(hipLaunchHostFunc(s_stream_, body_done_fn, &body_done_[par]));
+    pend_.active = true; pend_.closed = false; pend_.m = m; pend_.T = T; pend_.parity = par; pend_.tr = tr;
+    pend_parity_.store(par, std::memory_order_release);
+    m_quiet_.store(true, std::memory_order_release);
+}
+
+void Engine::finish_tail(bool merged)
+{
+    PendingTail &t = pend_;
+    const int q = t.parity;
+    auto graph = [&](int part) {
+        hipGraphExec_t g = sw_graphs_.find(GraphCache::Key{t.m, t.T, q * 8 + part});
+        if (!g) { LOGE("engine: the pending tail of a %d x %d feed has lost its graph (part %d)", t.m, t.T, part); abort(); }
+        return g;
+    };
+    StreamTrace *tr = t.tr;
+    if (tr) HIP_CHECK(hipEventRecord(tr->ev[7], stream_));
+    HIP_CHECK(hipGraphLaunch(graph(merged ? SW_MERGED : SW_TAIL), stream_));
+    if (tr) HIP_CHECK(hipEventRecord(tr->ev[3], stream_));
+    join(s_stream_, stream_);
+    if (tr) HIP_CHECK(hipEventRecord(tr->ev[4], s_stream_));
+    HIP_CHECK(hipGraphLaunch(graph(SW_SEARCH), s_stream_));
+    if (tr) { HIP_CHECK(hipEventRecord(tr->ev[5], s_stream_)); tr->tail = merged ? 2 : 1; tr->used = true; }
+    s_unseen_by_m_ = true;
+    if (t.closed) {
+        if (t.rec_n) HIP_CHECK(hipMemcpyAsync(rec_h_ + t.rec_base, rec_d_ + t.rec_base, t.rec_n * sizeof(StepRecord), hipMemcpyDeviceToHost, s_stream_));
+        for (const auto &sp : t.conf_spans) {
+            HIP_CHECK(hipMemcpyAsync(conf_h_ + sp.first, conf_d_ + sp.first, sp.second * sizeof(ConfRecord), hipMemcpyDeviceToHost, s_stream_));
+            conf_copied_.fetch_add(sp.second, std::memory_order_relaxed);
+        }
+        t.conf_spans.clear();
+        HIP_CHECK(hipEventRecord(flight_done_[q], s_stream_));
+    } else flight_tail_s_ = true;
+    t.active = false; t.tr = nullptr;
+    pend_parity_.store(-1, std::memory_order_release);
 }
 
 void Engine::run_layer_major(int m, int T, bool dump_logits)
@@ -1517,7 +1590,10 @@
 {
     HIP_CHECK(hipSetDevice(cfg_.device));
     const int p = flight_parity_ = next_parity_; next_parity_ ^= 1;
-    if (flight_open_[p]) { HIP_CHECK(hipEventSynchronize(flight_done_[p])); flight_open_[p] = false; }
+    if (flight_open_[p]) {
+        if (pend_parity_.load(std::memory_order_acquire) == p) { std::lock_guard<std::mutex> cg(capture_mu_); if (pend_.active && pend_.parity == p) finish_tail(false); }
+        HIP_CHECK(hipEventSynchronize(flight_done_[p])); flight_open_[p] = false;
+    }
     if (conf_has_pending_.load(std::memory_order_acquire)) apply_confidence_pending();
     if (bias_has_pending_.load(std::memory_order_acquire)) apply_bias_pending();
     if (opt_has_pending_.load(std::memory_order_acquire)) apply_search_options_pending();
@@ -1581,6 +1657,12 @@
 {
     HIP_CHECK(hipSetDevice(cfg_.device));
     std::lock_guard<std::mutex> cg(capture_mu_);
+    if (pend_.active && !pend_.closed) {
+        pend_.closed = true; pend_.rec_base = rec_base_; pend_.rec_n = rec_pos_ - rec_base_;
+        pend_.conf_spans.swap(conf_spans_); conf_spans_.clear();
+        flight_open_[flight_parity_] = true;
+        return flight_parity_;
+    }
     hipStream_t tail = s_stream_;
     if (!(flight_tail_s_ && s_unseen_by_m_)) {
         tail = stream_;
@@ -1600,6 +1682,12 @@
 
 bool Engine::flight_done(int parity)
 {
+    if (pend_parity_.load(std::memory_order_acquire) == parity) {
+        if (!body_done_[parity].load(std::memory_order_acquire)) return false;
+        std::lock_guard<std::mutex> cg(capture_mu_);
+        if (pend_.active && pend_.parity == parity) finish_tail(false);
+        return false;
+    }
     const hipError_t e = hipEventQuery(flight_done_[parity]);
     if (e == hipSuccess) return true;
     if (e != hipErrorNotReady) HIP_CHECK(e);
@@ -1610,6 +1698,10 @@
 void Engine::wait_flight(int parity)
 {
     HIP_CHECK(hipSetDevice(cfg_.device));
+    if (pend_parity_.load(std::memory_order_acquire) == parity) {
+        std::lock_guard<std::mutex> cg(capture_mu_);
+        if (pend_.active && pend_.parity == parity) finish_tail(false);
+    }
     HIP_CHECK(hipEventSynchronize(flight_done_[parity]));
     if (profiling_) sync();
 }
diff --git a/april_asr_amd/csrc/engine.h b/april_asr_amd/csrc/engine.h
--- a/april_asr_amd/csrc/engine.h
+++ b/april_asr_amd/csrc/engine.h
@@ -64,6 +64,8 @@
 
 struct RampStep { int macro = 0, own = 0; std::vector<std::pair<int, int>> guests; };
 std::vector<RampStep> ramp_window(int L, int T, int R, int max_problems = 3);
+struct RampPieces { bool ok = false; int head[2] = {0, -1}, body[2] = {0, -1}, tail[2] = {0, -1}; };
+RampPieces ramp_pieces(int L, int T, int R);
 
 class Engine {
 public:
@@ -221,22 +223,22 @@
         struct Batch { size_t off; int n, macro, kind; size_t roff; int rn; };
         struct Chain { std::vector<GemmArgs> host; GemmArgs *dev = nullptr; std::vector<Batch> batches; std::vector<RowArgs> rhost; RowArgs *rdev = nullptr; };
         Chain one;
-        Chain split;
-        bool hosts = false;
-        const Chain &layers(bool split_feed) const { return split_feed && !split.batches.empty() ? split : one; }
+        Chain merged;
+        RampPieces pieces;
         std::vector<std::pair<int, long>> stamp_slots; std::vector<int> stamp_n;
     };
-    GraphCache::Key graph_key(int m, int T = 0, int part = 0) const { return {m, T, flight_parity_ * 4 + part}; }
+    GraphCache::Key graph_key(int m, int T = 0, int part = 0) const { return {m, T, flight_parity_ * 8 + part}; }
     GraphCache::Key sw_key(int m, int T, int part = 0) const { return graph_key(gclk_ ? -m : m, T, part); }
+    enum { SW_FE = 1, SW_LAYERS = 2, SW_SEARCH = 3, SW_HEAD = 4, SW_BODY = 5, SW_TAIL = 6, SW_MERGED = 7 };
     SwPlan &sw_plan(int m, int T);
     void build_sw_chain(SwPlan &p, SwPlan::Chain &c, int m, int T, bool ramp);
     void free_sw_plans();
-    void run_sw_chain(int m, int T, bool dump_logits, const SwPlan &p, int part, hipStream_t st);
+    void run_sw_chain(int m, int T, bool dump_logits, const SwPlan &p, int part, hipStream_t st, int piece = 0);
     int stage_step(int m, int T, const int *slots, const int *ring_tails, const int *now_ms); void read_back_logits(int k, int rows, float *out);
     template <typename Chain> hipGraphExec_t cached_graph(GraphCache &cache, const GraphCache::Key &key, hipStream_t st, Chain &&chain);
     template <typename Capture> void capture_both_parities(Capture &&capture);
     void run_feed_wavefront(int m, int T, bool dump_logits); void run_layer_major(int m, int T, bool dump_logits); void launch_split_feed(int m, int T, hipStream_t fe);
-    struct StreamTrace { hipEvent_t ev[6] = {nullptr, nullptr, nullptr, nullptr, nullptr, nullptr}; int m = 0, T = 0; bool used = false; };
+    struct StreamTrace { hipEvent_t ev[8] = {nullptr, nullptr, nullptr, nullptr, nullptr, nullptr, nullptr, nullptr}; int m = 0, T = 0, tail = 0; bool used = false; };
     std::deque<StreamTrace> trace_; hipEvent_t trace_base_ = nullptr;
     StreamTrace *trace_slot();
     void dump_stream_trace();
@@ -318,10 +320,17 @@
     bool overlap_hint_ = false;
     int split_streams_ = 2;
     int ramp_mode_ = 1;
-    RampState *ramp_d_ = nullptr;
+    struct PendingTail {
+        bool active = false, closed = false; int m = 0, T = 0, parity = 0; StreamTrace *tr = nullptr;
+        size_t rec_base = 0, rec_n = 0; std::vector<std::pair<size_t, size_t>> conf_spans;
+    } pend_;
+    std::atomic<int> pend_parity_{-1};
+    std::atomic<uint32_t> body_done_[2] = {{0}, {0}};
+    hipEvent_t body_ev_[2] = {nullptr, nullptr};
+    void finish_tail(bool merged);
     std::atomic<bool> m_quiet_{false};
-    void m_touched() { m_quiet_.store(false, std::memory_order_release); }
-    std::atomic<uint64_t> ramp_eligible_{0};
+    void m_touched();
+    std::atomic<uint64_t> ramp_eligible_{0}, ramp_hosted_{0};
     float *xb_buf_[2] = {nullptr, nullptr}, *u_buf_[2] = {nullptr, nullptr}, *ff_buf_[2] = {nullptr, nullptr};
     uint16_t *xb16_buf_[2] = {nullptr, nullptr}, *u16_buf_[2] = {nullptr, nullptr}, *ff16_buf_[2] = {nullptr, nullptr};
     float *y_buf_[2] = {nullptr, nullptr}, *ssq_buf_[2] = {nullptr, nullptr}, *eout_lm_buf_[2] = {nullptr, nullptr}, *ws_fe_ = nullptr, *ws_sr_ = nullptr;
@@ -365,7 +374,7 @@
     GraphCache step_graphs_{"chunk step", 256};
     GraphCache lm_graphs_{"layer-major chain", 32};
     GraphCache lm_search_graphs_{"long-feed search", 64};
-    GraphCache sw_graphs_{"feed wavefront", 4 * 64};
+    GraphCache sw_graphs_{"feed wavefront", 8 * 64};
     size_t sw_plan_cap_ = 64;
     std::map<GraphCache::Key, SwPlan> sw_plans_;
     hipStream_t lm_stream_ = nullptr;
diff --git a/april_asr_amd/csrc/kernels.h b/april_asr_amd/csrc/kernels.h
--- a/april_asr_amd/csrc/kernels.h
+++ b/april_asr_amd/csrc/kernels.h
@@ -116,16 +116,6 @@
 void launch_row_z(const RowArgs *host_args, int n, const RowArgs *dev_args, hipStream_t s);
 
 constexpr int RAMP_R = 2;
-struct RampState {
-    unsigned long long ready[2];
-    int head_live[2];
-    int guest_live[2][RAMP_R][RAMP_R];
-    unsigned generation;
-    unsigned hosted;
-};
-constexpr int RAMP_MAX_M = 0xFFFFF, RAMP_MAX_T = 0xFF;
-void launch_ramp_ready(RampState *rs, int q, int m, int T, int hostable, hipStream_t s);
-void launch_ramp_latch(RampState *rs, int p, int m, hipStream_t s);
 
 struct StepRecord { int32_t idx; float max_val; float blank_val; uint32_t flags; };
 constexpr int kConfMaxAlt = 8;
diff --git a/april_asr_amd/csrc/kernels_misc.hip b/april_asr_amd/csrc/kernels_misc.hip
--- a/april_asr_amd/csrc/kernels_misc.hip
+++ b/april_asr_amd/csrc/kernels_misc.hip
@@ -86,44 +86,6 @@
     case ROW_RESID_SSQ: hipLaunchKernelGGL(row_zkernel<ROW_RESID_SSQ>, grid, block, 0, s, dev_args); break;
     default: hipLaunchKernelGGL(row_zkernel<ROW_SLOT_STORE>, grid, block, 0, s, dev_args); break;
     }
-}
-
-__global__ __launch_bounds__(64) void ramp_ready_kernel(RampState *rs, int q, int m, int T, int hostable)
-{
-    if (threadIdx.x != 0) return;
-    __hip_atomic_store(&rs->head_live[q], 1, __ATOMIC_RELAXED, __HIP_MEMORY_SCOPE_AGENT);
-    const unsigned g = __hip_atomic_load(&rs->generation, __ATOMIC_RELAXED, __HIP_MEMORY_SCOPE_AGENT) + 1u;
-    __hip_atomic_store(&rs->generation, g, __ATOMIC_RELAXED, __HIP_MEMORY_SCOPE_AGENT);
-    __builtin_amdgcn_fence(__ATOMIC_RELEASE, "agent");
-    asm volatile("s_waitcnt vmcnt(0)" ::: "memory");
-    const unsigned long long rec = ((unsigned long long)g << 32) | ((unsigned long long)(unsigned)m << 12) | ((unsigned long long)(unsigned)T << 4) | (unsigned long long)(hostable & 1);
-    __hip_atomic_store(&rs->ready[q], rec, __ATOMIC_RELAXED, __HIP_MEMORY_SCOPE_AGENT);
-}
-
-__global__ __launch_bounds__(64) void ramp_latch_kernel(RampState *rs, int p, int m)
-{
-    if (threadIdx.x != 0) return;
-    const unsigned long long mine = __hip_atomic_load(&rs->ready[p], __ATOMIC_RELAXED, __HIP_MEMORY_SCOPE_AGENT);
-    const unsigned long long next = __hip_atomic_load(&rs->ready[1 - p], __ATOMIC_RELAXED, __HIP_MEMORY_SCOPE_AGENT);
-    const unsigned g = (unsigned)(mine >> 32);
-    const int next_m = (int)((next >> 12) & RAMP_MAX_M), next_T = (int)((next >> 4) & RAMP_MAX_T);
-    const bool host = (unsigned)(next >> 32) == g + 1u && next_m == m && (int)((mine >> 12) & RAMP_MAX_M) == m && (next & 1ull) != 0;
-    if (host) {
-        __builtin_amdgcn_fence(__ATOMIC_ACQUIRE, "agent");
-        __hip_atomic_store(&rs->head_live[1 - p], 0, __ATOMIC_RELAXED, __HIP_MEMORY_SCOPE_AGENT);
-        rs->hosted += 1u;
-    }
-    for (int j = 1; j <= RAMP_R; ++j)
-        for (int t = 0; t < RAMP_R; ++t) rs->guest_live[p][j - 1][t] = (host && t < j && t < next_T) ? 1 : 0;
-}
-
-void launch_ramp_ready(RampState *rs, int q, int m, int T, int hostable, hipStream_t s)
-{
-    hipLaunchKernelGGL(ramp_ready_kernel, dim3(1), dim3(64), 0, s, rs, q, m, T, hostable);
-}
-void launch_ramp_latch(RampState *rs, int p, int m, hipStream_t s)
-{
-    hipLaunchKernelGGL(ramp_latch_kernel, dim3(1), dim3(64), 0, s, rs, p, m);
 }
 
 __device__ __forceinline__ void dec_embed_row(const DecEmbedParams &p, int tok0, int tok1, float *out)
diff --git a/april_asr_amd/csrc/ramp_api.cc b/april_asr_amd/csrc/ramp_api.cc
--- a/april_asr_amd/csrc/ramp_api.cc
+++ b/april_asr_amd/csrc/ramp_api.cc
@@ -24,6 +24,25 @@
     }
     return (int)w.size();
 }
+int aprilx_ramp_pieces(int L, int T, int R, int32_t *out, int cap)
+{
+    if (L <= 0 || T <= 0 || R <= 0 || !out) return -1;
+    const RampPieces p = ramp_pieces(L, T, R);
+    if (!p.ok) return 0;
+    const std::vector<RampStep> w = ramp_window(L, T, R);
+    int n = 0;
+    auto put = [&](int piece, int macro, int layer, int chunk, int guest) {
+        if ((n + 1) * 5 <= cap) { int32_t *o = out + (size_t)n * 5; o[0] = piece; o[1] = macro; o[2] = layer; o[3] = chunk; o[4] = guest; }
+        ++n;
+    };
+    const int *range[4] = {p.head, p.body, p.tail, p.tail};
+    for (int piece = 0; piece < 4; ++piece)
+        for (int W = range[piece][0]; W <= range[piece][1]; ++W) {
+            for (int l = 0; l < L; ++l) { const int t = W - 1 - l; if (t >= 0 && t < T) put(piece, W, l, t, 0); }
+            if (piece == 3) for (const RampStep &s : w) if (s.macro == W) for (const auto &g : s.guests) put(piece, W, g.first, g.second, 1);
+        }
+    return n * 5 <= cap ? n : -1;
+}
 int aprilx_model_ramp_stats(AprilASRModel model, int device_index, uint64_t *ramp_hosted, uint64_t *ramp_eligible)
 {
     if (!model || device_index < 0 || device_index >= (int)model->m.engines.size() || !ramp_hosted || !ramp_eligible) return -1;
diff --git a/include/aprilx_engine.h b/include/aprilx_engine.h
--- a/include/aprilx_engine.h
+++ b/include/aprilx_engine.h
@@ -50,6 +50,7 @@
 APRIL_EXPORT int aprilx_plan_gemm(int M, int N, int kz, int zcount, int tile_ok, int force, int32_t *out);
 
 APRIL_EXPORT int aprilx_ramp_window(int L, int T, int R, int32_t *out, int cap);
+APRIL_EXPORT int aprilx_ramp_pieces(int L, int T, int R, int32_t *out, int cap);
 
 APRIL_EXPORT int aprilx_stream_form(int kind, int M, int N, int K, int kz, int groups);
 
```
